# lucidrains/glom-pytorch

Hardware: AMD Instinct MI355X
Metric: images/sec (higher is better)
Workload: dtype bf16; 1 GPU; model=glom-512x6, global_batch=64, image_size=224, patch_size=14, iters=12, objective=denoising-mse fwd+bwd+adamw, decode_step=7, impl=native, parallelism=dp1

## Files before the change

### glom_pytorch_amd/ops/__init__.py

```python

from __future__ import annotations

import glob
import importlib
import os

import torch

_EXT = None
_EXT_ERR: Exception | None = None


def _load_extension():
    global _EXT, _EXT_ERR
    if _EXT is not None:
        return _EXT
    if _EXT_ERR is not None:
        raise _EXT_ERR
    try:
        from glom_pytorch_amd.ops import _glom_hip
        _EXT = _glom_hip
        return _EXT
    except ImportError as e:
        here = os.path.dirname(__file__)
        sos = glob.glob(os.path.join(here, "_glom_hip*.so"))
        _EXT_ERR = ImportError(
            f"glom_pytorch_amd HIP extension not importable ({e}). "
            f"Found candidate .so files: {sos or 'none'}. Build it in-tree with "
            f"`PYTORCH_ROCM_ARCH=gfx950 python setup.py build_ext --inplace` "
            f"from the repo root. The GPU path never falls back to eager.")
        raise _EXT_ERR


def available() -> bool:
    try:
        _load_extension()
        return True
    except ImportError:
        return False


def native_forward(model, img, iters, levels=None, return_all=False,
                   grad_iters=None, overlap_tail=False, loss_level_min=None):
    from glom_pytorch_amd.ops.functional import glom_forward
    return glom_forward(model, img, iters=iters, levels=levels,
                        return_all=return_all, grad_iters=grad_iters,
                        overlap_tail=overlap_tail,
                        loss_level_min=loss_level_min)


def set_token_hoist(on: bool) -> None:
    from glom_pytorch_amd.ops import functional
    functional.set_token_hoist(on)


def set_mix_fusion(on: bool) -> None:
    from glom_pytorch_amd.ops import functional
    functional.set_mix_fusion(on)


def set_check_level_cone(on: bool) -> None:
    from glom_pytorch_amd.ops import functional
    functional.set_check_level_cone(on)
```

### glom_pytorch_amd/ops/csrc/aux_kernels.h

```cpp
#pragma once
#include <hip/hip_runtime.h>

void launch_add_pos(const void* levels, const void* pos, void* out,
                    long total, int N, int L, int d, hipStream_t s);
void launch_rnorm(const void* levels, float* out, int B, int N, int L, int d,
                  hipStream_t s);
void launch_softmax_fwd(const void* scores, void* probs, const bool* mask,
                        int nprob, int N, int self_mask, hipStream_t s);
void launch_softmax_bwd(const void* P, const void* dP, const float* rnorm,
                        void* dS, void* dSr, const bool* mask, int nprob,
                        int N, int self_mask, float alpha, hipStream_t s,
                        int L = 1, int l_lo = 0);
void launch_knorm_combine(const void* dkhat, const void* lev,
                          const float* rnorm, const void* dv, const void* dq,
                          void* out, int B, int N, int L, int d,
                          hipStream_t s, int l_lo = 0);
void launch_mix_fwd(const void* prev, const void* bu, const void* td,
                    const void* cons, void* out, long total, int L, int d,
                    hipStream_t s, const void* bu0 = nullptr,
                    long bu0_ld = 0, const void* pos = nullptr,
                    void* td_next = nullptr, float* rn_next = nullptr,
                    int N = 1);
bool mix_fwd_can_emit_next(int L, int d);
void launch_mix_bwd(const void* dout, void* dmix, void* dtd, long total,
                    int L, int d, hipStream_t s);
void launch_add4(const void* a, const void* b, const void* c, const void* d,
                 void* out, long total, hipStream_t s);
void launch_gelu(const void* in, void* out, long total, hipStream_t s);
```

### glom_pytorch_amd/ops/csrc/aux_kernels.hip

```cpp

#include "common.h"
#include "aux_kernels.h"

#define NTHREADS 256
#define WPB (NTHREADS / WAVE)

__global__ __launch_bounds__(NTHREADS) void k_rnorm(
        const ushort_t* __restrict__ levels, float* __restrict__ out,
        int B, int N, int L, int d) {
    long row = (long)blockIdx.x * WPB + threadIdx.x / WAVE;
    long total = (long)B * N * L;
    if (row >= total) return;
    int lane = threadIdx.x % WAVE;
    int l = row % L;
    long n = (row / L) % N;
    long b = row / ((long)N * L);
    const ushort_t* x = levels + row * d;
    float ss = 0.f;
    if (d % 8 == 0) {
        for (int q0 = lane * 8; q0 < d; q0 += WAVE * 8) {
            union { uint4v v; ushort_t u[8]; } t;
            t.v = *(const uint4v*)(x + q0);
#pragma unroll
            for (int e = 0; e < 8; e++) {
                float v = bf2f(t.u[e]);
                ss += v * v;
            }
        }
    } else {
        for (int q = lane; q < d; q += WAVE) {
            float v = bf2f(x[q]);
            ss += v * v;
        }
    }
    ss = wave_reduce_sum(ss);
    if (lane == 0)
        out[(b * L + l) * N + n] = 1.0f / fmaxf(sqrtf(ss), 1e-12f);
}

__global__ __launch_bounds__(NTHREADS) void k_softmax_fwd(
        const ushort_t* __restrict__ scores, ushort_t* __restrict__ probs,
        const bool* __restrict__ nonlocal_mask, int nprob, int N,
        int self_mask) {
    long row = (long)blockIdx.x * WPB + threadIdx.x / WAVE;
    if (row >= (long)nprob * N) return;
    int lane = threadIdx.x % WAVE;
    int i = row % N;
    const ushort_t* s = scores + row * N;
    ushort_t* o = probs + row * N;
    const bool* m = nonlocal_mask ? nonlocal_mask + (long)i * N : nullptr;
    const float SELF = bf2f(f2bf(-5e-4f));
    const float NEG = -3.3895314e38f;

    if (N % 8 == 0) {
        float mx = -INFINITY, sum = 0.f;
#pragma unroll 1
        for (int j0 = lane * 8; j0 < N; j0 += WAVE * 8) {
            union { uint4v v; ushort_t u[8]; } t;
            t.v = *(const uint4v*)(s + j0);
#pragma unroll
            for (int e = 0; e < 8; e++) {
                float v = bf2f(t.u[e]);
                if (self_mask && j0 + e == i) v = SELF;
                if (m && m[j0 + e]) v = NEG;
                mx = fmaxf(mx, v);
            }
        }
        mx = wave_reduce_max(mx);
        mx = __shfl(mx, 0, WAVE);
#pragma unroll 1
        for (int j0 = lane * 8; j0 < N; j0 += WAVE * 8) {
            union { uint4v v; ushort_t u[8]; } t, ov;
            t.v = *(const uint4v*)(s + j0);
#pragma unroll
            for (int e = 0; e < 8; e++) {
                float v = bf2f(t.u[e]);
                if (self_mask && j0 + e == i) v = SELF;
                if (m && m[j0 + e]) v = NEG;
                float ex = __expf(v - mx);
                sum += ex;
                ov.u[e] = f2bf(ex);
            }
            *(uint4v*)(o + j0) = ov.v;
        }
        sum = wave_reduce_sum(sum);
        sum = __shfl(sum, 0, WAVE);
        float inv = 1.0f / sum;
#pragma unroll 1
        for (int j0 = lane * 8; j0 < N; j0 += WAVE * 8) {
            union { uint4v v; ushort_t u[8]; } t;
            t.v = *(const uint4v*)(o + j0);
#pragma unroll
            for (int e = 0; e < 8; e++) t.u[e] = f2bf(bf2f(t.u[e]) * inv);
            *(uint4v*)(o + j0) = t.v;
        }
        return;
    }
    float mx = -INFINITY;
    for (int j = lane; j < N; j += WAVE) {
        float v = bf2f(s[j]);
        if (self_mask && j == i) v = SELF;
        if (m && m[j]) v = NEG;
        mx = fmaxf(mx, v);
    }
    mx = wave_reduce_max(mx);
    mx = __shfl(mx, 0, WAVE);
    float sum = 0.f;
    for (int j = lane; j < N; j += WAVE) {
        float v = bf2f(s[j]);
        if (self_mask && j == i) v = SELF;
        if (m && m[j]) v = NEG;
        sum += expf(v - mx);
    }
    sum = wave_reduce_sum(sum);
    sum = __shfl(sum, 0, WAVE);
    float inv = 1.0f / sum;
    for (int j = lane; j < N; j += WAVE) {
        float v = bf2f(s[j]);
        if (self_mask && j == i) v = SELF;
        if (m && m[j]) v = NEG;
        o[j] = f2bf(expf(v - mx) * inv);
    }
}

__global__ __launch_bounds__(NTHREADS) void k_softmax_bwd(
        const ushort_t* __restrict__ P, const ushort_t* __restrict__ dP,
        const float* __restrict__ rnorm, ushort_t* __restrict__ dS,
        ushort_t* __restrict__ dSr, const bool* __restrict__ nonlocal_mask,
        int nprob, int N, int self_mask, float alpha, int L, int l_lo) {
    long row = (long)blockIdx.x * WPB + threadIdx.x / WAVE;
    if (row >= (long)nprob * N) return;
    int lane = threadIdx.x % WAVE;
    int i = row % N;
    long p = row / N;
    p = (p / (L - l_lo)) * L + l_lo + p % (L - l_lo);
    row = p * N + i;
    const ushort_t* pr = P + row * N;
    const ushort_t* dpr = dP + row * N;
    const float* rn = rnorm + p * N;
    const bool* m = nonlocal_mask ? nonlocal_mask + (long)i * N : nullptr;

    float t = 0.f;
    if (N % 8 == 0) {
#pragma unroll 1
        for (int j0 = lane * 8; j0 < N; j0 += WAVE * 8) {
            union { uint4v v; ushort_t u[8]; } a, bb;
            a.v = *(const uint4v*)(pr + j0);
            bb.v = *(const uint4v*)(dpr + j0);
#pragma unroll
            for (int e = 0; e < 8; e++) t += bf2f(a.u[e]) * bf2f(bb.u[e]);
        }
        t = wave_reduce_sum(t);
        t = __shfl(t, 0, WAVE);
#pragma unroll 1
        for (int j0 = lane * 8; j0 < N; j0 += WAVE * 8) {
            union { uint4v v; ushort_t u[8]; } a, bb, o1, o2;
            a.v = *(const uint4v*)(pr + j0);
            bb.v = *(const uint4v*)(dpr + j0);
#pragma unroll
            for (int e = 0; e < 8; e++) {
                float v = alpha * bf2f(a.u[e]) * (bf2f(bb.u[e]) - t);
                if (self_mask && j0 + e == i) v = 0.f;
                if (m && m[j0 + e]) v = 0.f;
                o1.u[e] = f2bf(v);
                o2.u[e] = f2bf(v * rn[j0 + e]);
            }
            *(uint4v*)(dS + row * N + j0) = o1.v;
            *(uint4v*)(dSr + row * N + j0) = o2.v;
        }
        return;
    }
    for (int j = lane; j < N; j += WAVE) t += bf2f(pr[j]) * bf2f(dpr[j]);
    t = wave_reduce_sum(t);
    t = __shfl(t, 0, WAVE);
    for (int j = lane; j < N; j += WAVE) {
        float v = alpha * bf2f(pr[j]) * (bf2f(dpr[j]) - t);
        if (self_mask && j == i) v = 0.f;
        if (m && m[j]) v = 0.f;
        dS[row * N + j] = f2bf(v);
        dSr[row * N + j] = f2bf(v * rn[j]);
    }
}

__global__ __launch_bounds__(NTHREADS) void k_knorm_combine(
        const ushort_t* __restrict__ dkhat, const ushort_t* __restrict__ lev,
        const float* __restrict__ rnorm, const ushort_t* __restrict__ dv,
        const ushort_t* __restrict__ dq, ushort_t* __restrict__ out,
        int B, int N, int L, int d, int l_lo) {
    long row = (long)blockIdx.x * WPB + threadIdx.x / WAVE;
    const int Ll = L - l_lo;
    long total = (long)B * N * Ll;
    if (row >= total) return;
    int lane = threadIdx.x % WAVE;
    int l = l_lo + row % Ll;
    long n = (row / Ll) % N;
    long b = row / ((long)N * Ll);
    row = (b * N + n) * L + l;
    const ushort_t* dkh = dkhat + ((b * L + l) * N + n) * (long)d;
    const ushort_t* x = lev + row * d;
    float r = rnorm[(b * L + l) * N + n];
    bool clamped = r >= 0.999e12f;

    const bool vec = (d % 8 == 0);
    float dot = 0.f;
    if (!clamped) {
        if (vec) {
            for (int q0 = lane * 8; q0 < d; q0 += WAVE * 8) {
                union { uint4v v; ushort_t u[8]; } a, b;
                a.v = *(const uint4v*)(dkh + q0);
                b.v = *(const uint4v*)(x + q0);
#pragma unroll
                for (int e = 0; e < 8; e++)
                    dot += bf2f(a.u[e]) * bf2f(b.u[e]);
            }
        } else {
            for (int q = lane; q < d; q += WAVE)
                dot += bf2f(dkh[q]) * bf2f(x[q]);
        }
        dot = wave_reduce_sum(dot);
        dot = __shfl(dot, 0, WAVE);
    }
    float c = clamped ? 0.f : r * r * dot;
    if (vec) {
        for (int q0 = lane * 8; q0 < d; q0 += WAVE * 8) {
            union { uint4v v; ushort_t u[8]; } a, b, dvv, dqv, o;
            a.v = *(const uint4v*)(dkh + q0);
            b.v = *(const uint4v*)(x + q0);
            dvv.v = *(const uint4v*)(dv + row * d + q0);
            dqv.v = *(const uint4v*)(dq + row * d + q0);
#pragma unroll
            for (int e = 0; e < 8; e++) {
                float dk = r * (bf2f(a.u[e]) - bf2f(b.u[e]) * c);
                o.u[e] = f2bf(dk + bf2f(dvv.u[e]) + bf2f(dqv.u[e]));
            }
            *(uint4v*)(out + row * d + q0) = o.v;
        }
    } else {
        for (int q = lane; q < d; q += WAVE) {
            float dk = r * (bf2f(dkh[q]) - bf2f(x[q]) * c);
            out[row * d + q] =
                f2bf(dk + bf2f(dv[row * d + q]) + bf2f(dq[row * d + q]));
        }
    }
}

template <bool NEXT>
__global__ __launch_bounds__(NTHREADS) void k_mix_fwd(
        const ushort_t* __restrict__ prev, const ushort_t* __restrict__ bu,
        const ushort_t* __restrict__ td, const ushort_t* __restrict__ cons,
        ushort_t* __restrict__ out, long total, int L, int d,
        const ushort_t* __restrict__ bu0, long bu0_ld,
        const ushort_t* __restrict__ pos, ushort_t* __restrict__ td_next,
        float* __restrict__ rn_next, int N) {
    long idx = ((long)blockIdx.x * NTHREADS + threadIdx.x) * 8;
    if (idx >= total) return;
    int q = idx % d;
    int l = (idx / d) % L;
    long bn = idx / ((long)d * L);
    union { uint4v v; ushort_t u[8]; } a, b, c4, t, o;
    a.v = *(const uint4v*)(prev + idx);
    b.v = *(const uint4v*)((bu0 && l == 0) ? bu0 + bn * bu0_ld + q
                                           : bu + idx);
    c4.v = *(const uint4v*)(cons + idx);
    bool has_td = l < L - 1;
    if (has_td) t.v = *(const uint4v*)(td + (bn * (L - 1) + l) * (long)d + q);
    float c = has_td ? 4.0f : 3.0f;
#pragma unroll
    for (int e = 0; e < 8; e++) {
        float v = bf2f(a.u[e]) + bf2f(b.u[e]) + bf2f(c4.u[e]);
        if (has_td) v += bf2f(t.u[e]);
        o.u[e] = f2bf(v / c);
    }
    *(uint4v*)(out + idx) = o.v;
    if (NEXT) {
        long n = bn % N;
        long bb = bn / N;
        float ss = 0.f;
#pragma unroll
        for (int e = 0; e < 8; e++) {
            float v = bf2f(o.u[e]);
            ss += v * v;
        }
        ss = wave_reduce_sum(ss);
        if (threadIdx.x % WAVE == 0)
            rn_next[(bb * L + l) * N + n] = 1.0f / fmaxf(sqrtf(ss), 1e-12f);
        if (l >= 1) {
            union { uint4v v; ushort_t u[8]; } p;
            p.v = *(const uint4v*)(pos + n * (long)d + q);
#pragma unroll
            for (int e = 0; e < 8; e++)
                p.u[e] = f2bf(bf2f(o.u[e]) + bf2f(p.u[e]));
            *(uint4v*)(td_next + (bn * (L - 1) + l - 1) * (long)d + q) = p.v;
        }
    }
}

__global__ __launch_bounds__(NTHREADS) void k_mix_bwd(
        const ushort_t* __restrict__ dout, ushort_t* __restrict__ dmix,
        ushort_t* __restrict__ dtd, long total, int L, int d) {
    long idx = ((long)blockIdx.x * NTHREADS + threadIdx.x) * 8;
    if (idx >= total) return;
    int q = idx % d;
    int l = (idx / d) % L;
    long bn = idx / ((long)d * L);
    union { uint4v v; ushort_t u[8]; } g, o;
    g.v = *(const uint4v*)(dout + idx);
    bool has_td = l < L - 1;
    float c = has_td ? 4.0f : 3.0f;
#pragma unroll
    for (int e = 0; e < 8; e++) o.u[e] = f2bf(bf2f(g.u[e]) / c);
    *(uint4v*)(dmix + idx) = o.v;
    if (has_td) *(uint4v*)(dtd + (bn * (L - 1) + l) * (long)d + q) = o.v;
}

__global__ __launch_bounds__(NTHREADS) void k_add_pos(
        const ushort_t* __restrict__ levels, const ushort_t* __restrict__ pos,
        ushort_t* __restrict__ out, long total, int N, int L, int d) {
    long i8 = ((long)blockIdx.x * NTHREADS + threadIdx.x) * 8;
    if (i8 >= total) return;
    int G = L - 1;
    int q = i8 % d;
    int g = (i8 / d) % G;
    long bn = i8 / ((long)d * G);
    long n = bn % N;
    const ushort_t* lv = levels + (bn * L + g + 1) * (long)d + q;
    const ushort_t* pp = pos + n * (long)d + q;
    union { uint4v v; ushort_t u[8]; } a, b;
    a.v = *(const uint4v*)lv;
    b.v = *(const uint4v*)pp;
#pragma unroll
    for (int e = 0; e < 8; e++) a.u[e] = f2bf(bf2f(a.u[e]) + bf2f(b.u[e]));
    *(uint4v*)(out + i8) = a.v;
}


static inline long cdiv(long a, long b) { return (a + b - 1) / b; }

void launch_add_pos(const void* levels, const void* pos, void* out,
                    long total, int N, int L, int d, hipStream_t s) {
    hipLaunchKernelGGL(k_add_pos, dim3(cdiv(total / 8, NTHREADS)),
                       dim3(NTHREADS), 0, s, (const ushort_t*)levels,
                       (const ushort_t*)pos, (ushort_t*)out, total, N, L, d);
}

void launch_rnorm(const void* levels, float* out, int B, int N, int L, int d,
                  hipStream_t s) {
    long rows = (long)B * N * L;
    hipLaunchKernelGGL(k_rnorm, dim3(cdiv(rows, WPB)), dim3(NTHREADS), 0, s,
                       (const ushort_t*)levels, out, B, N, L, d);
}

void launch_softmax_fwd(const void* scores, void* probs, const bool* mask,
                        int nprob, int N, int self_mask, hipStream_t s) {
    long rows = (long)nprob * N;
    hipLaunchKernelGGL(k_softmax_fwd, dim3(cdiv(rows, WPB)), dim3(NTHREADS),
                       0, s, (const ushort_t*)scores, (ushort_t*)probs, mask,
                       nprob, N, self_mask);
}

void launch_softmax_bwd(const void* P, const void* dP, const float* rnorm,
                        void* dS, void* dSr, const bool* mask, int nprob,
                        int N, int self_mask, float alpha, hipStream_t s,
                        int L, int l_lo) {
    long rows = (long)nprob * N;
    hipLaunchKernelGGL(k_softmax_bwd, dim3(cdiv(rows, WPB)), dim3(NTHREADS),
                       0, s, (const ushort_t*)P, (const ushort_t*)dP, rnorm,
                       (ushort_t*)dS, (ushort_t*)dSr, mask, nprob, N,
                       self_mask, alpha, L, l_lo);
}

void launch_knorm_combine(const void* dkhat, const void* lev,
                          const float* rnorm, const void* dv, const void* dq,
                          void* out, int B, int N, int L, int d,
                          hipStream_t s, int l_lo) {
    long rows = (long)B * N * (L - l_lo);
    if (rows <= 0) return;
    hipLaunchKernelGGL(k_knorm_combine, dim3(cdiv(rows, WPB)), dim3(NTHREADS),
                       0, s, (const ushort_t*)dkhat, (const ushort_t*)lev,
                       rnorm, (const ushort_t*)dv, (const ushort_t*)dq,
                       (ushort_t*)out, B, N, L, d, l_lo);
}

void launch_mix_fwd(const void* prev, const void* bu, const void* td,
                    const void* cons, void* out, long total, int L, int d,
                    hipStream_t s, const void* bu0, long bu0_ld,
                    const void* pos, void* td_next, float* rn_next, int N) {
    dim3 grid(cdiv(total / 8, NTHREADS)), block(NTHREADS);
    if (td_next)
        hipLaunchKernelGGL(k_mix_fwd<true>, grid, block, 0, s,
                           (const ushort_t*)prev, (const ushort_t*)bu,
                           (const ushort_t*)td, (const ushort_t*)cons,
                           (ushort_t*)out, total, L, d, (const ushort_t*)bu0,
                           bu0_ld, (const ushort_t*)pos, (ushort_t*)td_next,
                           rn_next, N);
    else
        hipLaunchKernelGGL(k_mix_fwd<false>, grid, block, 0, s,
                           (const ushort_t*)prev, (const ushort_t*)bu,
                           (const ushort_t*)td, (const ushort_t*)cons,
                           (ushort_t*)out, total, L, d, (const ushort_t*)bu0,
                           bu0_ld, (const ushort_t*)nullptr,
                           (ushort_t*)nullptr, (float*)nullptr, N);
}

bool mix_fwd_can_emit_next(int L, int d) { return d == WAVE * 8 && L >= 2; }

void launch_mix_bwd(const void* dout, void* dmix, void* dtd, long total,
                    int L, int d, hipStream_t s) {
    hipLaunchKernelGGL(k_mix_bwd, dim3(cdiv(total / 8, NTHREADS)), dim3(NTHREADS),
                       0, s, (const ushort_t*)dout, (ushort_t*)dmix,
                       (ushort_t*)dtd, total, L, d);
}

__global__ __launch_bounds__(NTHREADS) void k_add4(
        const ushort_t* __restrict__ a, const ushort_t* __restrict__ b,
        const ushort_t* __restrict__ c, const ushort_t* __restrict__ d,
        ushort_t* __restrict__ out, long total) {
    long i8 = ((long)blockIdx.x * NTHREADS + threadIdx.x) * 8;
    if (i8 >= total) return;
    union { uint4v v; ushort_t u[8]; } va, vb, vc, vd, o;
    va.v = *(const uint4v*)(a + i8);
    vb.v = *(const uint4v*)(b + i8);
    vc.v = *(const uint4v*)(c + i8);
    vd.v = *(const uint4v*)(d + i8);
#pragma unroll
    for (int e = 0; e < 8; e++)
        o.u[e] = f2bf(bf2f(va.u[e]) + bf2f(vb.u[e]) + bf2f(vc.u[e])
                      + bf2f(vd.u[e]));
    *(uint4v*)(out + i8) = o.v;
}

void launch_add4(const void* a, const void* b, const void* c, const void* d,
                 void* out, long total, hipStream_t s) {
    hipLaunchKernelGGL(k_add4, dim3(cdiv(total / 8, NTHREADS)),
                       dim3(NTHREADS), 0, s, (const ushort_t*)a,
                       (const ushort_t*)b, (const ushort_t*)c,
                       (const ushort_t*)d, (ushort_t*)out, total);
}

__global__ __launch_bounds__(NTHREADS) void k_gelu(
        const ushort_t* __restrict__ in, ushort_t* __restrict__ out,
        long total) {
    long i8 = ((long)blockIdx.x * NTHREADS + threadIdx.x) * 8;
    if (i8 >= total) return;
    union { uint4v v; ushort_t u[8]; } x, o;
    x.v = *(const uint4v*)(in + i8);
    float xin[8], yv[8];
#pragma unroll
    for (int e = 0; e < 8; e++) xin[e] = bf2f(x.u[e]);
    gelu_f_vec<8>(xin, yv);
#pragma unroll
    for (int e = 0; e < 8; e++) o.u[e] = f2bf(yv[e]);
    *(uint4v*)(out + i8) = o.v;
}

void launch_gelu(const void* in, void* out, long total, hipStream_t s) {
    hipLaunchKernelGGL(k_gelu, dim3(cdiv(total / 8, NTHREADS)),
                       dim3(NTHREADS), 0, s, (const ushort_t*)in,
                       (ushort_t*)out, total);
}
```

### glom_pytorch_amd/ops/csrc/bindings.cpp

```cpp

#include <torch/extension.h>
#include <c10/hip/HIPStream.h>
#include <hip/hip_runtime.h>

#include <cmath>
#include <cstring>
#include <vector>

#include "gemm.h"
#include "aux_kernels.h"
#include "native_ops.h"
#include "island_kernels.h"
#include "parse_kernels.h"
#include "contrast_kernels.h"

namespace {

torch::Tensor alias_slab_slice(const torch::Tensor& slab, int64_t idx,
                               c10::IntArrayRef sizes) {
    int64_t n = 1;
    for (auto s : sizes) n *= s;
    void* ptr = (char*)slab.data_ptr() + idx * n * slab.element_size();
    auto keep = slab;
    return torch::from_blob(
        ptr, sizes, [keep](void*) mutable {}, slab.options());
}

#define CHECK_IN(x)                                                        \
    TORCH_CHECK(x.is_cuda(), #x " must be on GPU");                        \
    TORCH_CHECK(x.is_contiguous(), #x " must be contiguous");              \
    TORCH_CHECK(x.scalar_type() == at::kBFloat16, #x " must be bf16")

hipStream_t cur_stream() {
    return c10::hip::getCurrentHIPStream().stream();
}

int g_nt8p_mode = []() {
    const char* e = getenv("GLOM_NT8P");
    return (e && e[0] == '0') ? 0 : 1;
}();

void set_nt8p(bool on) { g_nt8p_mode = on ? 1 : 0; }

int g_tn_tr = []() {
    const char* e = getenv("GLOM_TN_TR");
    return (e && e[0] >= '0' && e[0] <= '2') ? e[0] - '0' : 1;
}();
int g_tn_tr_variant = []() {
    const char* e = getenv("GLOM_TN_TR_VARIANT");
    return (e && e[0] >= '1' && e[0] <= '3') ? e[0] - '0' : 1;
}();
void set_tn_tr(bool on) { g_tn_tr = on ? 2 : 0; }
void set_tn_tr_mode(int64_t m) {
    TORCH_CHECK(m >= 0 && m <= 2, "tn_tr mode is 0..2");
    g_tn_tr = (int)m;
}
int64_t get_tn_tr_mode() { return g_tn_tr; }
void set_tn_tr_variant(int64_t v) {
    TORCH_CHECK(v >= 1 && v <= 3, "tn_tr variant is 1..3");
    g_tn_tr_variant = (int)v;
}
int64_t get_tn_tr_variant() { return g_tn_tr_variant; }
static bool tn_tr_auto(const GemmParams& p) {
    return p.splitk > 1 || p.K >= 4096;
}
int g_finish_wide = []() {
    const char* e = getenv("GLOM_FINISH_WIDE");
    return (e && e[0] == '0') ? 0 : 1;
}();
void set_finish_wide(bool on) { g_finish_wide = on ? 1 : 0; }

int g_gelu_pair = []() {
    const char* e = getenv("GLOM_GELU_PAIR");
    return (e && e[0] == '0') ? 0 : 1;
}();
void set_gelu_pair(bool on) { g_gelu_pair = on ? 1 : 0; }

int g_wide_epi = []() {
    const char* e = getenv("GLOM_WIDE_EPI");
    return (e && e[0] >= '0' && e[0] <= '3') ? e[0] - '0' : 1;
}();
int g_wide_epi_nt8p = []() {
    const char* e = getenv("GLOM_WIDE_EPI_NT8P");
    return (e && e[0] == '1') ? 1 : 0;
}();
void set_wide_epilogue(bool on) { g_wide_epi = on ? 2 : 0; }
void set_wide_epilogue_mode(int64_t m) {
    TORCH_CHECK(m >= 0 && m <= 3, "wide epilogue mode is 0..3");
    g_wide_epi = (int)m;
}
int64_t get_wide_epilogue_mode() { return g_wide_epi; }
static int wide_epi_auto(int epilogue) {
    return epilogue == EPI_GELUGRAD ? 3 : epilogue == EPI_GELU ? 1 : 0;
}
static int nt5p_wide_bits(int epilogue) {
    switch (g_wide_epi) {
    case 0: return 0;
    case 2: return 3;
    case 3: return 2;
    default: return wide_epi_auto(epilogue);
    }
}
void set_wide_epilogue_nt8p(bool on) { g_wide_epi_nt8p = on ? 1 : 0; }

static bool wide_epi_ok(const GemmParams& p) {
    auto al = [](const void* q) { return ((uintptr_t)q & 15) == 0; };
    bool ok = al(p.Cbase) && p.Cld % 8 == 0 && p.Csin % 8 == 0
              && p.Csout % 8 == 0;
    if (p.epilogue == EPI_GELU_PAIR)
        ok = ok && al(p.out2) && p.out2_ld % 8 == 0 && p.out2_sin % 8 == 0
             && p.out2_sout % 8 == 0;
    if (p.epilogue == EPI_GELUGRAD)
        ok = ok && al(p.aux_base) && p.aux_ld % 8 == 0 && p.aux_sin % 8 == 0
             && p.aux_sout % 8 == 0;
    return ok;
}

static bool nt5p_enabled() {
    static const bool on = []() {
        const char* e = getenv("GLOM_NT5P");
        return !e || e[0] != '0';
    }();
    return on;
}
static long nt5p_min_grid() {
    static const long g = []() {
        const char* e = getenv("GLOM_NT5P_MING");
        return e ? atol(e) : 96;
    }();
    return g;
}
static bool nt5p_takes_up_proj(int64_t M, int64_t N, int64_t K, int64_t G) {
    return nt5p_enabled() && M % 512 == 0 && N % 256 == 0 && N >= 1024
           && K % 64 == 0 && K >= 64
           && (N / 256) * (M / 512) * G >= nt5p_min_grid();
}

void check_launch() {
    hipError_t e = hipGetLastError();
    TORCH_CHECK(e == hipSuccess, "HIP launch failed: ", hipGetErrorString(e));
}

int64_t g_nce_launches[2] = {0, 0};
std::vector<int64_t> nce_launch_counts() {
    return {g_nce_launches[0], g_nce_launches[1]};
}
int g_nce_fast = []() {
    const char* e = getenv("GLOM_NCE_FAST");
    return (e && e[0] == '0') ? 0 : 1;
}();
void set_nce_fast(bool on) { g_nce_fast = on ? 1 : 0; }

void run_gemm(GemmParams& p, hipStream_t s, const torch::TensorOptions& opts,
              bool lds_ok, long gate_problems = 0) {
    const long gate_np = gate_problems > 0 ? gate_problems : p.nproblems;
    const bool no_xform = !(p.A.flags & (OP_GELU | OP_POS))
                          && !(p.B.flags & (OP_GELU | OP_POS));
    const bool nce_generic = !g_nce_fast && (p.epilogue == EPI_NCE_FWD
                                             || p.epilogue == EPI_NCE_BWD);
    const bool nt_fast = p.layout == LAYOUT_NT && lds_ok && no_xform
                         && p.M % 128 == 0 && p.N % 128 == 0
                         && p.K % 64 == 0 && p.K >= 64 && !nce_generic;
    const bool tn_fast = p.layout == LAYOUT_TN && lds_ok && no_xform
                         && p.M % 128 == 0 && p.N % 128 == 0 && p.K % 8 == 0;
    const bool nn_fast = p.layout == LAYOUT_NN && lds_ok && no_xform
                         && p.M % 128 == 0 && p.N % 128 == 0 && p.K % 8 == 0;

    p.splitk = 1;
    p.ws = nullptr;
    torch::Tensor ws;
    long blocks = ((p.N + 127) / 128) * ((p.M + 127) / 128) * gate_np;
    if (p.layout == LAYOUT_TN && p.epilogue == EPI_NONE && !p.has_bias
        && !p.has_colscale && blocks < 1024 && p.K >= 4096) {
        long sk = std::min<long>(16, std::max<long>(1, 2048 / blocks));
        sk = std::min<long>(sk, p.K / 64);
        if (sk > 1) {
            ws = torch::empty({sk * p.nproblems * (long)p.M * p.N},
                              opts.dtype(at::kFloat));
            p.splitk = (int)sk;
            p.ws = ws.data_ptr<float>();
        }
    }
    const bool nce = p.epilogue == EPI_NCE_FWD || p.epilogue == EPI_NCE_BWD;
    if (nce) {
        auto al = [](const void* q) { return ((uintptr_t)q & 15) == 0; };
        TORCH_CHECK(p.layout == LAYOUT_NT && p.nproblems == 1
                    && !((p.A.flags | p.B.flags | p.Cflags) & OP_TABLE)
                    && !p.has_bias && !p.has_colscale,
                    "EPI_NCE_* needs one plain NT problem");
        const NceArgs q = nce_get(p);
        TORCH_CHECK(q.rrow && q.rcol && q.part && q.group > 0,
                    "EPI_NCE_* parameters not set (nce_set)");
        TORCH_CHECK(p.epilogue == EPI_NCE_FWD ? q.pos != nullptr
                                              : (q.lse && p.Cbase),
                    "EPI_NCE_* outputs not set");
        TORCH_CHECK(!nt_fast
                    || (al(p.A.base) && al(p.B.base)
                        && (p.epilogue == EPI_NCE_FWD
                            || (al(p.Cbase) && p.Cld % 8 == 0))),
                    "EPI_NCE_* full-tile path needs 16-byte aligned operands");
    }
    const bool nt3 = nt_fast && p.N % 256 == 0 && p.N >= 1024 && !nce;
    const bool nt5p_on = nt5p_enabled();
    const bool nt5p = nt5p_on && nt3 && p.M % 512 == 0
                      && (long)(p.N / 256) * (p.M / 512) * gate_np
                         >= nt5p_min_grid()
                      && !(p.Cflags & OP_TABLE)
                      && (p.epilogue == EPI_NONE
                          || p.epilogue == EPI_GELUGRAD
                          || p.epilogue == EPI_GELU_PAIR
                          || p.epilogue == EPI_GELU);
    TORCH_CHECK(p.epilogue != EPI_GELU || nt5p,
                "EPI_GELU needs an nt5p-eligible shape");
    static const bool disp_dbg = []() {
        const char* e = getenv("GLOM_DISPATCH_DEBUG");
        return e && e[0] == '1';
    }();
    const bool nt8p_on = g_nt8p_mode == 1;
    static const long nt8p_mink = []() {
        const char* e = getenv("GLOM_NT8P_MINK");
        return e ? atol(e) : 2048;
    }();
    const bool nt8p = nt8p_on && p.layout == LAYOUT_NT && lds_ok && no_xform
                      && p.M % 256 == 0 && p.N % 256 == 0 && p.K % 64 == 0
                      && p.K >= nt8p_mink
                      && !(p.Cflags & OP_TABLE)
                      && (p.epilogue == EPI_NONE
                          || p.epilogue == EPI_GELUGRAD)
                      && (long)(p.N / 256) * (p.M / 256) * gate_np >= 256;
    auto al16 = [](const void* q) { return ((uintptr_t)q & 15) == 0; };
    bool tn_al = al16(p.A.base) && al16(p.B.base);
    if (p.A.flags & OP_TABLE)
        for (int g = 0; g < p.nproblems; g++) tn_al = tn_al && al16(p.Atab[g]);
    if (p.B.flags & OP_TABLE)
        for (int g = 0; g < p.nproblems; g++) tn_al = tn_al && al16(p.Btab[g]);
    const bool tn_tr = (g_tn_tr == 2 || (g_tn_tr == 1 && tn_tr_auto(p)))
                       && tn_fast && p.K % 64 == 0 && p.K >= 64
                       && tn_al && p.A.sin % 8 == 0 && p.A.sout % 8 == 0
                       && p.B.sin % 8 == 0 && p.B.sout % 8 == 0;
    p.wide_epi = !wide_epi_ok(p) ? 0
                 : nt8p ? g_wide_epi_nt8p : nt5p_wide_bits(p.epilogue);
    if (disp_dbg)
        fprintf(stderr,
                "[dispatch] L%d M%ld N%ld K%ld epi%d nt3=%d nt5p=%d on=%d "
                "nt8p=%d ctabflag=%d m512=%d tn_tr=%d sk=%d finw=%d "
                "kern=%s\n",
                p.layout, (long)p.M, (long)p.N, (long)p.K, p.epilogue,
                (int)nt3, (int)nt5p, (int)nt5p_on, (int)nt8p,
                (int)(p.Cflags & OP_TABLE), (int)(p.M % 512 == 0),
                tn_tr ? (p.splitk > 1 ? g_tn_tr_variant : 1) : 0,
                p.splitk, g_finish_wide,
                nt8p ? "nt8p" : nt5p ? "nt5p" : nt3 ? "nt4"
                : nt_fast ? "nt_fast" : tn_tr ? "tn_tr"
                : tn_fast ? (p.splitk > 1 ? "tn_sk" : "tn_fast")
                : nn_fast ? "nn_fast" : "generic");
    if (nt8p)
        launch_gemm_nt_fast8p(p, s);
    else if (nt5p)
        launch_gemm_nt_fast5p(p, s);
    else if (nt3)
        launch_gemm_nt_fast4(p, s);
    else if (nt_fast) {
        launch_gemm_nt_fast(p, s);
        if (nce) g_nce_launches[0]++;
    }
    else if (tn_tr)
        launch_gemm_tn_tr(p, g_tn_tr_variant, s);
    else if (tn_fast && p.splitk > 1)
        launch_gemm_tn_sk(p, s);
    else if (tn_fast)
        launch_gemm_tn_fast(p, s);
    else if (nn_fast)
        launch_gemm_nn_fast(p, s);
    else {
        launch_gemm(p, s);
        if (nce) g_nce_launches[1]++;
    }
    check_launch();
    if (p.splitk > 1) {
        launch_gemm_finish(p, s, g_finish_wide == 1);
        check_launch();
    }
}

GemmParams base_params(int64_t M, int64_t N, int64_t K, int layout,
                       int64_t nproblems, int64_t nInner, float alpha) {
    GemmParams p;
    std::memset(&p, 0, sizeof(p));
    p.M = (int)M; p.N = (int)N; p.K = (int)K;
    p.layout = layout;
    p.nproblems = (int)nproblems;
    p.nInner = (int)nInner;
    p.alpha = alpha;
    p.epilogue = EPI_NONE;
    return p;
}


void* u16_at(const torch::Tensor& t, int64_t off) {
    return (void*)((uint16_t*)t.data_ptr() + off);
}

void zero_fill(void* ptr, int64_t bytes, hipStream_t s) {
    if (bytes <= 0) return;
    hipError_t e = hipMemsetAsync(ptr, 0, (size_t)bytes, s);
    TORCH_CHECK(e == hipSuccess, "zero fill failed: ", hipGetErrorString(e));
}

void zero_unwritten_dx(void* dLevels, int64_t BN, int64_t L, int64_t d,
                       int64_t mode, int64_t g_lo, hipStream_t s) {
    if (mode == 0) {
        launch_zero_slices(dLevels, BN, (int)L, (int)d, 0,
                           (int)std::max<int64_t>(g_lo, 1) - 1, s);
        check_launch();
        launch_zero_slice(dLevels, BN, (int)L, (int)d, (int)L - 1, s);
        check_launch();
    } else {
        launch_zero_slices(dLevels, BN, (int)L, (int)d, 0,
                           (int)std::min<int64_t>(g_lo + 1, L), s);
        check_launch();
    }
}


std::vector<torch::Tensor> grouped_ff_fwd(
        c10::optional<torch::Tensor> tokens_opt, torch::Tensor levels,
        c10::optional<torch::Tensor> pos_opt, torch::Tensor w1,
        torch::Tensor b1, torch::Tensor w2, torch::Tensor b2, int64_t mode,
        bool save_for_bwd = true, bool group0_done = false,
        c10::optional<torch::Tensor> td_in_ready = c10::nullopt) {
    CHECK_IN(levels); CHECK_IN(w1); CHECK_IN(b1); CHECK_IN(w2); CHECK_IN(b2);
    const int64_t B = levels.size(0), N = levels.size(1),
                  L = levels.size(2), d = levels.size(3);
    const int64_t G = (mode == 0) ? L : L - 1;
    TORCH_CHECK(G <= GEMM_MAX_TABLE, "levels > 16 unsupported by table mode");
    TORCH_CHECK(!group0_done || (mode == 0 && G >= 2),
                "group0_done needs the bottom-up mode and levels >= 2");
    const int64_t g0 = group0_done ? 1 : 0;
    const int64_t Ga = G - g0;
    const int64_t m4 = w1.size(0) / G;
    const int64_t M = B * N;
    TORCH_CHECK(d % 8 == 0 && m4 % 8 == 0, "dim and mult*dim must be /8");
    TORCH_CHECK(w1.size(0) == G * m4 && w1.size(1) == d);
    TORCH_CHECK(w2.size(0) == G * d && w2.size(1) == m4);

    auto opts = levels.options();
    const bool pair = g_gelu_pair
                      && (M % 512 == 0) && (m4 % 256 == 0)
                      && m4 >= 1024;
    const bool gelu_only = !save_for_bwd && pair
                           && nt5p_takes_up_proj(M, m4, d, G);
    auto Hpre = gelu_only ? torch::empty({0}, opts)
                          : torch::empty({G, M, m4}, opts);
    auto Hact = torch::empty({G, M, m4}, opts);
    auto Y = torch::empty({B, N, G, d}, opts);
    hipStream_t s = cur_stream();

    torch::Tensor td_in;
    if (mode == 1) {
        TORCH_CHECK(pos_opt.has_value(), "top-down needs pos");
        auto pos = pos_opt.value();
        CHECK_IN(pos);
        if (td_in_ready.has_value()) {
            td_in = td_in_ready.value();
            CHECK_IN(td_in);
            TORCH_CHECK(td_in.dim() == 4 && td_in.size(0) == B
                        && td_in.size(1) == N && td_in.size(2) == G
                        && td_in.size(3) == d, "td_in must be (B,N,L-1,d)");
        } else {
            td_in = torch::empty({B, N, G, d}, opts);
            launch_add_pos(levels.data_ptr(), pos.data_ptr(),
                           td_in.data_ptr(), td_in.numel(), (int)N, (int)L,
                           (int)d, s);
            check_launch();
        }
    }

    {
        GemmParams p = base_params(M, m4, d, LAYOUT_NT, Ga, Ga, 1.0f);
        if (mode == 0) {
            TORCH_CHECK(tokens_opt.has_value(), "bottom-up needs tokens");
            auto tokens = tokens_opt.value();
            CHECK_IN(tokens);
            TORCH_CHECK(tokens.numel() == M * d, "tokens must be (B,N,d)");
            p.A.flags = OP_TABLE;
            if (g0 == 0) {
                p.Atab[0] = tokens.data_ptr();
                p.Atabld[0] = d;
            }
            for (int64_t g = 1; g < G; g++) {
                p.Atab[g - g0] = (const char*)levels.data_ptr()
                                 + (g - 1) * d * 2;
                p.Atabld[g - g0] = L * d;
            }
        } else {
            p.A.base = td_in.data_ptr();
            p.A.sin = d; p.A.ld = G * d;
        }
        p.B.base = u16_at(w1, g0 * m4 * d); p.B.sin = m4 * d; p.B.ld = d;
        p.Csin = M * m4; p.Cld = m4;
        p.bias_base = u16_at(b1, g0 * m4); p.bias_sin = m4; p.has_bias = 1;
        if (gelu_only) {
            p.epilogue = EPI_GELU;
            p.Cbase = u16_at(Hact, g0 * M * m4);
        } else {
            p.Cbase = u16_at(Hpre, g0 * M * m4);
            if (pair) {
                p.epilogue = EPI_GELU_PAIR;
                p.out2 = u16_at(Hact, g0 * M * m4);
                p.out2_sin = M * m4; p.out2_ld = m4;
            }
        }
        run_gemm(p, s, opts, true, G);
        if (!pair) {
            launch_gelu(u16_at(Hpre, g0 * M * m4), u16_at(Hact, g0 * M * m4),
                        Ga * M * m4, s);
            check_launch();
        }
    }
    {
        GemmParams p = base_params(M, d, m4, LAYOUT_NT, Ga, Ga, 1.0f);
        p.A.base = u16_at(Hact, g0 * M * m4); p.A.sin = M * m4; p.A.ld = m4;
        p.B.base = u16_at(w2, g0 * d * m4); p.B.sin = d * m4; p.B.ld = m4;
        p.Cbase = u16_at(Y, g0 * d); p.Csin = d; p.Cld = G * d;
        p.bias_base = u16_at(b2, g0 * d); p.bias_sin = d; p.has_bias = 1;
        run_gemm(p, s, opts, true, G);
    }
    if (mode != 1) td_in = torch::empty({0}, opts);
    if (!save_for_bwd) Hpre = torch::empty({0}, opts);
    return {Y, Hpre, Hact, td_in};
}

std::vector<torch::Tensor> grouped_ff_bwd(
        torch::Tensor dY, c10::optional<torch::Tensor> tokens_opt,
        torch::Tensor levels, c10::optional<torch::Tensor> pos_opt,
        torch::Tensor w1, torch::Tensor w2, torch::Tensor Hpre,
        torch::Tensor Hact, int64_t mode,
        c10::optional<torch::Tensor> w1t_opt = c10::nullopt,
        c10::optional<torch::Tensor> w2t_opt = c10::nullopt,
        c10::optional<torch::Tensor> td_in_opt = c10::nullopt,
        int64_t g_lo = 0) {
    CHECK_IN(dY); CHECK_IN(levels); CHECK_IN(w1); CHECK_IN(w2); CHECK_IN(Hpre);
    CHECK_IN(Hact);
    const int64_t B = levels.size(0), N = levels.size(1),
                  L = levels.size(2), d = levels.size(3);
    const int64_t G = (mode == 0) ? L : L - 1;
    const int64_t m4 = w1.size(0) / G;
    const int64_t M = B * N;
    TORCH_CHECK(g_lo >= 0 && g_lo <= G, "g_lo out of range");
    const int64_t Ga = G - g_lo;
    auto opts = levels.options();
    hipStream_t s = cur_stream();

    auto dLevels = torch::empty({B, N, L, d}, opts);
    zero_unwritten_dx(dLevels.data_ptr(), B * N, L, d, mode, g_lo, s);
    torch::Tensor dTokens;
    auto dW1 = torch::empty({G * m4, d}, opts);
    auto dW2 = torch::empty({G * d, m4}, opts);
    auto dB1 = torch::empty({G * m4}, opts);
    auto dB2 = torch::empty({G * d}, opts);
    zero_fill(dW1.data_ptr(), g_lo * m4 * d * 2, s);
    zero_fill(dW2.data_ptr(), g_lo * d * m4 * 2, s);
    zero_fill(dB1.data_ptr(), g_lo * m4 * 2, s);
    if (mode == 0) {
        dTokens = torch::empty({B, N, d}, opts);
        if (g_lo > 0) zero_fill(dTokens.data_ptr(), M * d * 2, s);
    } else {
        dTokens = torch::empty({0}, opts);
    }
    if (Ga == 0) {
        zero_fill(dB2.data_ptr(), G * d * 2, s);
        return {dTokens, dLevels, dW1, dB1, dW2, dB2};
    }
    TORCH_CHECK(Hpre.numel() == G * M * m4 && Hact.numel() == G * M * m4,
                "Hpre / Hact must be (G, M, m4)");
    auto dHpre = torch::empty({G, M, m4}, opts);

    auto w1t = w1t_opt.has_value()
        ? w1t_opt.value()
        : w1.view({G, m4, d}).transpose(1, 2).contiguous();
    auto w2t = w2t_opt.has_value()
        ? w2t_opt.value()
        : w2.view({G, d, m4}).transpose(1, 2).contiguous();

    torch::Tensor td_in;
    if (mode == 1) {
        if (td_in_opt.has_value() && td_in_opt->numel() > 0) {
            td_in = td_in_opt.value();
        } else {
            auto pos = pos_opt.value();
            CHECK_IN(pos);
            td_in = torch::empty({B, N, G, d}, opts);
            launch_add_pos(levels.data_ptr(), pos.data_ptr(),
                           td_in.data_ptr(), td_in.numel(), (int)N, (int)L,
                           (int)d, s);
            check_launch();
        }
    }

    const bool dh_nt3 = (M % 128 == 0) && (m4 % 256 == 0) && (m4 >= 1024)
                        && (d % 64 == 0);
    torch::Tensor db1f;
    {
        GemmParams p = base_params(M, m4, d, LAYOUT_NT, Ga, Ga, 1.0f);
        p.A.base = u16_at(dY, g_lo * d); p.A.sin = d; p.A.ld = G * d;
        p.B.base = u16_at(w2t, g_lo * m4 * d); p.B.sin = m4 * d; p.B.ld = d;
        p.Cbase = u16_at(dHpre, g_lo * M * m4); p.Csin = M * m4; p.Cld = m4;
        p.epilogue = EPI_GELUGRAD;
        p.aux_base = u16_at(Hpre, g_lo * M * m4);
        p.aux_sin = M * m4; p.aux_ld = m4;
        if (dh_nt3) {
            db1f = torch::empty({Ga, M / 64, m4}, opts.dtype(at::kFloat));
            p.colsum_out = db1f.data_ptr<float>();
            p.colsum_sin = (M / 64) * m4;
        }
        run_gemm(p, s, opts, true, G);
    }
    {
        GemmParams p = base_params(M, d, m4, LAYOUT_NT, Ga, Ga, 1.0f);
        p.A.base = u16_at(dHpre, g_lo * M * m4); p.A.sin = M * m4; p.A.ld = m4;
        p.B.base = u16_at(w1t, g_lo * d * m4); p.B.sin = d * m4; p.B.ld = m4;
        if (mode == 0) {
            p.Cflags = OP_TABLE;
            for (int64_t g = g_lo; g < G; g++) {
                p.Ctab[g - g_lo] = g == 0 ? dTokens.data_ptr()
                                          : u16_at(dLevels, (g - 1) * d);
                p.Ctabld[g - g_lo] = g == 0 ? d : L * d;
            }
        } else {
            p.Cbase = u16_at(dLevels, (g_lo + 1) * d);
            p.Csin = d; p.Cld = L * d;
        }
        run_gemm(p, s, opts, true, G);
    }
    {
        GemmParams p = base_params(m4, d, M, LAYOUT_TN, Ga, Ga, 1.0f);
        p.A.base = u16_at(dHpre, g_lo * M * m4); p.A.sin = M * m4; p.A.ld = m4;
        if (mode == 0) {
            auto tokens = tokens_opt.value();
            CHECK_IN(tokens);
            p.B.flags = OP_TABLE;
            for (int64_t g = g_lo; g < G; g++) {
                p.Btab[g - g_lo] = g == 0 ? tokens.data_ptr()
                                          : u16_at(levels, (g - 1) * d);
                p.Btabld[g - g_lo] = g == 0 ? d : L * d;
            }
        } else {
            p.B.base = u16_at(td_in, g_lo * d);
            p.B.sin = d; p.B.ld = G * d;
        }
        p.Cbase = u16_at(dW1, g_lo * m4 * d); p.Csin = m4 * d; p.Cld = d;
        run_gemm(p, s, opts, true, G);
    }
    {
        GemmParams p = base_params(d, m4, M, LAYOUT_TN, Ga, Ga, 1.0f);
        p.A.base = u16_at(dY, g_lo * d); p.A.sin = d; p.A.ld = G * d;
        p.B.base = u16_at(Hact, g_lo * M * m4); p.B.sin = M * m4; p.B.ld = m4;
        p.Cbase = u16_at(dW2, g_lo * d * m4); p.Csin = d * m4; p.Cld = m4;
        run_gemm(p, s, opts, true, G);
    }
    if (dh_nt3) {
        launch_colsum_fin(db1f.data_ptr<float>(), u16_at(dB1, g_lo * m4),
                          (int)Ga, m4, (int)(M / 64), s);
        check_launch();
    } else {
        auto ws = torch::empty({(long)Ga * colsum_rb(M) * m4},
                               opts.dtype(at::kFloat));
        launch_colsum(u16_at(dHpre, g_lo * M * m4), ws.data_ptr<float>(),
                      u16_at(dB1, g_lo * m4), (int)Ga, M, m4, s);
        check_launch();
    }
    {
        auto ws = torch::empty({(long)colsum_rb(M) * G * d},
                               opts.dtype(at::kFloat));
        launch_colsum(dY.data_ptr(), ws.data_ptr<float>(), dB2.data_ptr(),
                      1, M, G * d, s);
        check_launch();
    }
    return {dTokens, dLevels, dW1, dB1, dW2, dB2};
}


std::vector<torch::Tensor> consensus_fwd(
        torch::Tensor levels, bool attend_self,
        c10::optional<torch::Tensor> mask_opt,
        c10::optional<torch::Tensor> rnorm_ready = c10::nullopt) {
    CHECK_IN(levels);
    const int64_t B = levels.size(0), N = levels.size(1),
                  L = levels.size(2), d = levels.size(3);
    const int64_t P = B * L;
    auto opts = levels.options();
    hipStream_t s = cur_stream();
    const bool* mask = nullptr;
    if (mask_opt.has_value()) {
        auto m = mask_opt.value();
        TORCH_CHECK(m.is_cuda() && m.is_contiguous()
                    && m.scalar_type() == at::kBool);
        mask = m.data_ptr<bool>();
    }

    const bool lds_ok = (N % 8 == 0) && (d % 8 == 0);
    torch::Tensor rnorm;
    if (rnorm_ready.has_value()) {
        rnorm = rnorm_ready.value();
        TORCH_CHECK(rnorm.is_cuda() && rnorm.is_contiguous()
                    && rnorm.scalar_type() == at::kFloat
                    && rnorm.dim() == 3 && rnorm.size(0) == B
                    && rnorm.size(1) == L && rnorm.size(2) == N,
                    "rnorm must be f32 (B,L,N)");
    } else {
        rnorm = torch::empty({B, L, N}, opts.dtype(at::kFloat));
        launch_rnorm(levels.data_ptr(), rnorm.data_ptr<float>(),
                     (int)B, (int)N, (int)L, (int)d, s);
        check_launch();
    }

    auto probs = torch::empty({B, L, N, N}, opts);
    const bool fused_sm = (N == 256) && (d % 64 == 0) && lds_ok;
    const bool fuse_av = fused_sm && !getenv("GLOM_NO_FUSE_AV");
    torch::Tensor out_av;
    if (fuse_av) out_av = torch::empty({B, N, L, d}, opts);
    {
        GemmParams p = base_params(N, N, d, LAYOUT_NT, P, L,
                                   (float)std::pow((double)d, -0.5));
        p.A.base = levels.data_ptr(); p.A.sin = d; p.A.sout = N * L * d;
        p.A.ld = L * d;
        p.B = p.A;
        p.Cbase = probs.data_ptr(); p.Csin = N * N; p.Csout = L * N * N;
        p.Cld = N;
        p.colscale_base = rnorm.data_ptr<float>();
        p.cs_sin = N; p.cs_sout = L * N; p.has_colscale = 1;
        if (fused_sm) {
            p.epilogue = EPI_SOFTMAX;
            p.self_mask = attend_self ? 0 : 1;
            p.nlmask = mask;
            p.splitk = 1;
            if (fuse_av) {
                p.out2 = out_av.data_ptr();
                p.out2_sin = d; p.out2_sout = N * L * d; p.out2_ld = L * d;
                p.aux_base = levels.data_ptr();
                p.aux_sin = d; p.aux_sout = N * L * d; p.aux_ld = L * d;
                p.npatch = (int)d;
            }
            launch_gemm_nt_fast4(p, s);
            check_launch();
        } else {
            run_gemm(p, s, opts, lds_ok);
            launch_softmax_fwd(probs.data_ptr(), probs.data_ptr(), mask,
                               (int)P, (int)N, attend_self ? 0 : 1, s);
            check_launch();
        }
    }
    if (fuse_av)
        return {out_av, probs, rnorm};
    auto out = torch::empty({B, N, L, d}, opts);
    {
        GemmParams p = base_params(N, d, N, LAYOUT_NN, P, L, 1.0f);
        p.A.base = probs.data_ptr(); p.A.sin = N * N; p.A.sout = L * N * N;
        p.A.ld = N;
        p.B.base = levels.data_ptr(); p.B.sin = d; p.B.sout = N * L * d;
        p.B.ld = L * d;
        p.Cbase = out.data_ptr(); p.Csin = d; p.Csout = N * L * d;
        p.Cld = L * d;
        run_gemm(p, s, opts, lds_ok);
    }
    return {out, probs, rnorm};
}

torch::Tensor consensus_bwd(torch::Tensor dOut, torch::Tensor levels,
                            torch::Tensor probs, torch::Tensor rnorm,
                            bool attend_self,
                            c10::optional<torch::Tensor> mask_opt,
                            int64_t l_lo = 0) {
    CHECK_IN(dOut); CHECK_IN(levels); CHECK_IN(probs);
    const int64_t B = levels.size(0), N = levels.size(1),
                  L = levels.size(2), d = levels.size(3);
    TORCH_CHECK(l_lo >= 0 && l_lo <= L, "l_lo out of range");
    const int64_t Ll = L - l_lo;
    const int64_t P = B * Ll;
    const int64_t Pfull = B * L;
    const bool lds_ok = (N % 8 == 0) && (d % 8 == 0);
    auto opts = levels.options();
    hipStream_t s = cur_stream();
    const bool* mask = nullptr;
    if (mask_opt.has_value()) mask = mask_opt.value().data_ptr<bool>();

    auto dLevels = torch::empty({B, N, L, d}, opts);
    launch_zero_slices(dLevels.data_ptr(), B * N, (int)L, (int)d, 0,
                       (int)l_lo, s);
    check_launch();
    if (Ll == 0) return dLevels;
    TORCH_CHECK(l_lo == 0 || d % 8 == 0, "l_lo needs dim % 8 == 0");
    const float* rn = rnorm.data_ptr<float>();
    auto lv = [&](const torch::Tensor& t) { return u16_at(t, l_lo * d); };
    auto nn = [&](const torch::Tensor& t) { return u16_at(t, l_lo * N * N); };

    const bool fused_sm = (N == 256) && (d % 64 == 0) && lds_ok;
    auto dS = torch::empty({B, L, N, N}, opts);
    auto dSr = torch::empty({B, L, N, N}, opts);
    torch::Tensor dP;
    if (fused_sm) {
        GemmParams p = base_params(N, N, d, LAYOUT_NT, P, Ll, 1.0f);
        p.A.base = lv(dOut); p.A.sin = d; p.A.sout = N * L * d;
        p.A.ld = L * d;
        p.B.base = lv(levels); p.B.sin = d; p.B.sout = N * L * d;
        p.B.ld = L * d;
        p.Cbase = nn(dS); p.Csin = N * N; p.Csout = L * N * N;
        p.Cld = N;
        p.epilogue = EPI_SMBWD;
        p.aux_base = nn(probs);
        p.aux_sin = N * N; p.aux_sout = L * N * N; p.aux_ld = N;
        p.out2 = nn(dSr);
        p.out2_sin = N * N; p.out2_sout = L * N * N; p.out2_ld = N;
        p.colscale_base = rn + l_lo * N;
        p.cs_sin = N; p.cs_sout = L * N; p.has_colscale = 1;
        p.self_mask = attend_self ? 0 : 1;
        p.nlmask = mask;
        p.alpha2 = (float)std::pow((double)d, -0.5);
        p.splitk = 1;
        launch_gemm_nt_fast4(p, s);
        check_launch();
    } else {
        dP = torch::empty({B, L, N, N}, opts);
        GemmParams p = base_params(N, N, d, LAYOUT_NT, P, Ll, 1.0f);
        p.A.base = lv(dOut); p.A.sin = d; p.A.sout = N * L * d;
        p.A.ld = L * d;
        p.B.base = lv(levels); p.B.sin = d; p.B.sout = N * L * d;
        p.B.ld = L * d;
        p.Cbase = nn(dP); p.Csin = N * N; p.Csout = L * N * N;
        p.Cld = N;
        run_gemm(p, s, opts, lds_ok, Pfull);
        launch_softmax_bwd(probs.data_ptr(), dP.data_ptr(), rn,
                           dS.data_ptr(), dSr.data_ptr(), mask, (int)P,
                           (int)N, attend_self ? 0 : 1,
                           (float)std::pow((double)d, -0.5), s, (int)L,
                           (int)l_lo);
        check_launch();
    }

    auto dv = torch::empty({B, N, L, d}, opts);
    {
        GemmParams p = base_params(N, d, N, LAYOUT_TN, P, Ll, 1.0f);
        p.A.base = nn(probs); p.A.sin = N * N; p.A.sout = L * N * N;
        p.A.ld = N;
        p.B.base = lv(dOut); p.B.sin = d; p.B.sout = N * L * d;
        p.B.ld = L * d;
        p.Cbase = lv(dv); p.Csin = d; p.Csout = N * L * d;
        p.Cld = L * d;
        run_gemm(p, s, opts, lds_ok, Pfull);
    }
    auto dq = torch::empty({B, N, L, d}, opts);
    {
        GemmParams p = base_params(N, d, N, LAYOUT_NN, P, Ll, 1.0f);
        p.A.base = nn(dSr); p.A.sin = N * N; p.A.sout = L * N * N;
        p.A.ld = N;
        p.B.base = lv(levels); p.B.sin = d; p.B.sout = N * L * d;
        p.B.ld = L * d;
        p.Cbase = lv(dq); p.Csin = d; p.Csout = N * L * d;
        p.Cld = L * d;
        run_gemm(p, s, opts, lds_ok, Pfull);
    }
    auto dkhat = torch::empty({B, L, N, d}, opts);
    {
        GemmParams p = base_params(N, d, N, LAYOUT_TN, P, Ll, 1.0f);
        p.A.base = nn(dS); p.A.sin = N * N; p.A.sout = L * N * N;
        p.A.ld = N;
        p.B.base = lv(levels); p.B.sin = d; p.B.sout = N * L * d;
        p.B.ld = L * d;
        p.Cbase = u16_at(dkhat, l_lo * N * d);
        p.Csin = N * d; p.Csout = L * N * d;
        p.Cld = d;
        run_gemm(p, s, opts, lds_ok, Pfull);
    }
    launch_knorm_combine(dkhat.data_ptr(), levels.data_ptr(), rn,
                         dv.data_ptr(), dq.data_ptr(), dLevels.data_ptr(),
                         (int)B, (int)N, (int)L, (int)d, s, (int)l_lo);
    check_launch();
    return dLevels;
}


std::vector<torch::Tensor> level_mix_fwd_next(
        torch::Tensor levels, torch::Tensor bu, torch::Tensor td,
        torch::Tensor cons, c10::optional<torch::Tensor> slab = c10::nullopt,
        int64_t slab_idx = 0, c10::optional<torch::Tensor> bu0 = c10::nullopt,
        c10::optional<torch::Tensor> pos = c10::nullopt) {
    CHECK_IN(levels); CHECK_IN(bu); CHECK_IN(td); CHECK_IN(cons);
    const int64_t B = levels.size(0), N = levels.size(1),
                  L = levels.size(2), d = levels.size(3);
    TORCH_CHECK(d % 8 == 0, "dim must be a multiple of 8");
    TORCH_CHECK(bu.numel() == levels.numel() && cons.numel() == levels.numel()
                && td.numel() == B * N * (L - 1) * d,
                "level mix operands do not match levels");
    const void* bu0_ptr = nullptr;
    int64_t bu0_ld = 0;
    if (bu0.has_value()) {
        const auto& t = bu0.value();
        TORCH_CHECK(t.is_cuda() && t.scalar_type() == at::kBFloat16
                    && t.dim() == 3 && t.size(0) == B && t.size(1) == N
                    && t.size(2) == d && t.stride(2) == 1
                    && t.stride(1) >= d && t.stride(1) % 8 == 0
                    && t.stride(0) == N * t.stride(1)
                    && ((uintptr_t)t.data_ptr() & 15) == 0,
                    "bu0 must be an evenly strided (B,N,d) bf16 view");
        bu0_ptr = t.data_ptr();
        bu0_ld = t.stride(1);
    }
    const bool emit = pos.has_value() && mix_fwd_can_emit_next((int)L, (int)d);
    auto td_next = torch::empty({0}, levels.options());
    auto rn_next = torch::empty({0}, levels.options().dtype(at::kFloat));
    if (emit) {
        CHECK_IN(pos.value());
        TORCH_CHECK(pos->numel() == N * d, "pos must be (N,d)");
        td_next = torch::empty({B, N, L - 1, d}, levels.options());
        rn_next = torch::empty({B, L, N}, levels.options().dtype(at::kFloat));
    }
    torch::Tensor out;
    if (slab.has_value()) {
        TORCH_CHECK(slab->is_contiguous()
                    && slab->scalar_type() == at::kBFloat16
                    && slab->numel() >= (slab_idx + 1) * levels.numel(),
                    "bad trajectory slab");
        out = alias_slab_slice(slab.value(), slab_idx, levels.sizes());
    } else {
        out = torch::empty_like(levels);
    }
    launch_mix_fwd(levels.data_ptr(), bu.data_ptr(), td.data_ptr(),
                   cons.data_ptr(), out.data_ptr(), levels.numel(), (int)L,
                   (int)d, cur_stream(), bu0_ptr, bu0_ld,
                   emit ? pos->data_ptr() : nullptr,
                   emit ? td_next.data_ptr() : nullptr,
                   emit ? rn_next.data_ptr<float>() : nullptr, (int)N);
    check_launch();
    return {out, td_next, rn_next};
}

torch::Tensor level_mix_fwd(torch::Tensor levels, torch::Tensor bu,
                            torch::Tensor td, torch::Tensor cons,
                            c10::optional<torch::Tensor> slab = c10::nullopt,
                            int64_t slab_idx = 0,
                            c10::optional<torch::Tensor> bu0 = c10::nullopt) {
    return level_mix_fwd_next(levels, bu, td, cons, slab, slab_idx, bu0,
                              c10::nullopt)[0];
}

std::vector<torch::Tensor> level_mix_bwd(torch::Tensor dout) {
    CHECK_IN(dout);
    const int64_t B = dout.size(0), N = dout.size(1), L = dout.size(2),
                  d = dout.size(3);
    TORCH_CHECK(d % 8 == 0, "dim must be a multiple of 8");
    auto dmix = torch::empty_like(dout);
    auto dtd = torch::empty({B, N, L - 1, d}, dout.options());
    launch_mix_bwd(dout.data_ptr(), dmix.data_ptr(), dtd.data_ptr(),
                   dout.numel(), (int)L, (int)d, cur_stream());
    check_launch();
    return {dmix, dtd};
}




std::vector<torch::Tensor> glom_step_fwd(
        torch::Tensor tokens, torch::Tensor levels, torch::Tensor pos,
        torch::Tensor bw1, torch::Tensor bb1, torch::Tensor bw2,
        torch::Tensor bb2, torch::Tensor tw1, torch::Tensor tb1,
        torch::Tensor tw2, torch::Tensor tb2, bool attend_self,
        c10::optional<torch::Tensor> mask,
        c10::optional<torch::Tensor> slab = c10::nullopt,
        int64_t slab_idx = 0, bool save_for_bwd = true,
        c10::optional<torch::Tensor> bu0 = c10::nullopt,
        c10::optional<torch::Tensor> td_in_ready = c10::nullopt,
        c10::optional<torch::Tensor> rnorm_ready = c10::nullopt,
        bool emit_next = false) {
    auto bu = grouped_ff_fwd(tokens, levels, c10::nullopt, bw1, bb1, bw2,
                             bb2, 0, save_for_bwd, bu0.has_value());
    auto td = grouped_ff_fwd(c10::nullopt, levels, pos, tw1, tb1, tw2,
                             tb2, 1, save_for_bwd, false, td_in_ready);
    auto at = consensus_fwd(levels, attend_self, mask, rnorm_ready);
    auto mx = level_mix_fwd_next(
        levels, bu[0], td[0], at[0], slab, slab_idx, bu0,
        emit_next ? c10::optional<torch::Tensor>(pos) : c10::nullopt);
    std::vector<torch::Tensor> r = {mx[0], bu[1], bu[2], td[1], td[2],
                                    at[1], at[2], td[3]};
    if (emit_next) { r.push_back(mx[1]); r.push_back(mx[2]); }
    return r;
}

std::vector<torch::Tensor> glom_step_bwd(
        torch::Tensor dnew, torch::Tensor tokens, torch::Tensor levels,
        torch::Tensor pos, torch::Tensor bw1, torch::Tensor bw2,
        torch::Tensor tw1, torch::Tensor tw2, torch::Tensor buHpre,
        torch::Tensor buHact, torch::Tensor tdHpre, torch::Tensor tdHact,
        torch::Tensor probs, torch::Tensor rnorm, bool attend_self,
        c10::optional<torch::Tensor> mask,
        c10::optional<torch::Tensor> bw1t, c10::optional<torch::Tensor> bw2t,
        c10::optional<torch::Tensor> tw1t,
        c10::optional<torch::Tensor> tw2t,
        c10::optional<torch::Tensor> td_in = c10::nullopt,
        int64_t lo = 0) {
    const int64_t L = levels.size(2);
    TORCH_CHECK(lo >= 0 && lo < L, "lo out of range");
    auto mix = level_mix_bwd(dnew);
    auto bu = grouped_ff_bwd(mix[0], tokens, levels, c10::nullopt, bw1,
                             bw2, buHpre, buHact, 0, bw1t, bw2t,
                             c10::nullopt, lo);
    auto td = grouped_ff_bwd(mix[1], c10::nullopt, levels, pos, tw1, tw2,
                             tdHpre, tdHact, 1, tw1t, tw2t, td_in,
                             std::min<int64_t>(lo, L - 1));
    auto dAttn = consensus_bwd(mix[0], levels, probs, rnorm, attend_self,
                               mask, lo);
    auto dLevels = torch::empty_like(levels);
    launch_add4(mix[0].data_ptr(), bu[1].data_ptr(), td[1].data_ptr(),
                dAttn.data_ptr(), dLevels.data_ptr(), levels.numel(),
                cur_stream());
    check_launch();
    const int64_t B = levels.size(0), N = levels.size(1),
                  d = levels.size(3);
    auto dPos = torch::empty({N, d}, levels.options());
    const int BCH = (int)std::min<int64_t>(B, 8);
    auto ws = torch::empty({BCH * N * d}, levels.options().dtype(at::kFloat));
    launch_dpos(td[1].data_ptr(), dPos.data_ptr(), ws.data_ptr<float>(),
                BCH, (int)B, (int)N, (int)L, (int)d, cur_stream());
    check_launch();
    return {bu[0], dLevels, dPos, bu[2], bu[3], bu[4], bu[5],
            td[2], td[3], td[4], td[5]};
}

double bench_gemm(int64_t M, int64_t N, int64_t K, int64_t layout,
                  int64_t nproblems, int64_t epilogue, int64_t reps) {
    auto opts = torch::TensorOptions().dtype(at::kBFloat16)
                    .device(at::kCUDA);
    torch::Tensor A, Bt;
    if (layout == LAYOUT_TN)
        A = torch::randn({nproblems, K, M}, opts) * 0.05;
    else
        A = torch::randn({nproblems, M, K}, opts) * 0.05;
    if (layout == LAYOUT_NT)
        Bt = torch::randn({nproblems, N, K}, opts) * 0.05;
    else
        Bt = torch::randn({nproblems, K, N}, opts) * 0.05;
    auto C = torch::empty({nproblems, M, N}, opts);
    auto bias = torch::randn({nproblems, N}, opts);
    auto aux = torch::randn({nproblems, M, N}, opts);
    auto out2 = torch::empty({nproblems, M, N}, opts);
    hipStream_t s = cur_stream();

    auto run = [&]() {
        GemmParams p = base_params(M, N, K, (int)layout, nproblems,
                                   nproblems, 1.0f);
        p.A.base = A.data_ptr();
        p.A.sin = A.size(1) * A.size(2); p.A.ld = A.size(2);
        p.B.base = Bt.data_ptr();
        p.B.sin = Bt.size(1) * Bt.size(2); p.B.ld = Bt.size(2);
        p.Cbase = C.data_ptr(); p.Csin = M * N; p.Cld = N;
        p.epilogue = (int)epilogue;
        if (epilogue == EPI_GELUGRAD) {
            p.aux_base = aux.data_ptr(); p.aux_sin = M * N; p.aux_ld = N;
        }
        if (epilogue == EPI_GELU_PAIR || epilogue == EPI_GELU
            || epilogue == 10 || epilogue == 12) {
            p.bias_base = bias.data_ptr(); p.bias_sin = N; p.has_bias = 1;
            p.out2 = out2.data_ptr(); p.out2_sin = M * N; p.out2_ld = N;
        }
        run_gemm(p, s, opts, true);
    };
    for (int i = 0; i < 3; i++) run();
    hipEvent_t e0, e1;
    hipEventCreate(&e0); hipEventCreate(&e1);
    hipEventRecord(e0, s);
    for (int64_t i = 0; i < reps; i++) run();
    hipEventRecord(e1, s);
    hipEventSynchronize(e1);
    float ms = 0;
    hipEventElapsedTime(&ms, e0, e1);
    hipEventDestroy(e0); hipEventDestroy(e1);
    return ms / reps;
}

torch::Tensor gemm_tn(torch::Tensor A, torch::Tensor B) {
    CHECK_IN(A); CHECK_IN(B);
    TORCH_CHECK(A.dim() == 3 && B.dim() == 3 && A.size(0) == B.size(0)
                && A.size(1) == B.size(1), "A (G,K,M), B (G,K,N)");
    const int64_t G = A.size(0), K = A.size(1), M = A.size(2),
                  N = B.size(2);
    TORCH_CHECK(M % 8 == 0 && N % 8 == 0, "M and N must be /8");
    auto C = torch::empty({G, M, N}, A.options());
    GemmParams p = base_params(M, N, K, LAYOUT_TN, G, G, 1.0f);
    p.A.base = A.data_ptr(); p.A.sin = K * M; p.A.ld = M;
    p.B.base = B.data_ptr(); p.B.sin = K * N; p.B.ld = N;
    p.Cbase = C.data_ptr(); p.Csin = M * N; p.Cld = N;
    run_gemm(p, cur_stream(), A.options(), true);
    return C;
}

torch::Tensor gemm_nt(torch::Tensor A, torch::Tensor B,
                      c10::optional<torch::Tensor> bias_opt = c10::nullopt) {
    CHECK_IN(A); CHECK_IN(B);
    TORCH_CHECK(A.dim() == 3 && B.dim() == 3 && A.size(0) == B.size(0)
                && A.size(2) == B.size(2), "A (G,M,K), B (G,N,K)");
    const int64_t G = A.size(0), M = A.size(1), K = A.size(2),
                  N = B.size(1);
    TORCH_CHECK(K % 8 == 0 && N % 8 == 0, "K and N must be /8");
    auto C = torch::empty({G, M, N}, A.options());
    GemmParams p = base_params(M, N, K, LAYOUT_NT, G, G, 1.0f);
    p.A.base = A.data_ptr(); p.A.sin = M * K; p.A.ld = K;
    p.B.base = B.data_ptr(); p.B.sin = N * K; p.B.ld = K;
    p.Cbase = C.data_ptr(); p.Csin = M * N; p.Cld = N;
    if (bias_opt.has_value()) {
        auto bias = bias_opt.value();
        CHECK_IN(bias);
        TORCH_CHECK(bias.dim() == 2 && bias.size(0) == G
                    && bias.size(1) == N, "bias (G,N)");
        p.bias_base = bias.data_ptr(); p.bias_sin = N; p.has_bias = 1;
    }
    run_gemm(p, cur_stream(), A.options(), true);
    return C;
}

torch::Tensor gemm_nn(torch::Tensor A, torch::Tensor B) {
    CHECK_IN(A); CHECK_IN(B);
    TORCH_CHECK(A.dim() == 3 && B.dim() == 3 && A.size(0) == B.size(0)
                && A.size(2) == B.size(1), "A (G,M,K), B (G,K,N)");
    const int64_t G = A.size(0), M = A.size(1), K = A.size(2),
                  N = B.size(2);
    TORCH_CHECK(K % 8 == 0 && N % 8 == 0, "K and N must be /8");
    auto C = torch::empty({G, M, N}, A.options());
    GemmParams p = base_params(M, N, K, LAYOUT_NN, G, G, 1.0f);
    p.A.base = A.data_ptr(); p.A.sin = M * K; p.A.ld = K;
    p.B.base = B.data_ptr(); p.B.sin = K * N; p.B.ld = N;
    p.Cbase = C.data_ptr(); p.Csin = M * N; p.Cld = N;
    run_gemm(p, cur_stream(), A.options(), true);
    return C;
}

void add4_into(torch::Tensor a, torch::Tensor b, torch::Tensor c,
               torch::Tensor d, torch::Tensor out) {
    CHECK_IN(a); CHECK_IN(b); CHECK_IN(c); CHECK_IN(d); CHECK_IN(out);
    launch_add4(a.data_ptr(), b.data_ptr(), c.data_ptr(), d.data_ptr(),
                out.data_ptr(), out.numel(), cur_stream());
    check_launch();
}



std::vector<torch::Tensor> ff_bwd_dh(torch::Tensor dY, torch::Tensor w2t,
                                     torch::Tensor Hpre, int64_t g_lo = 0) {
    CHECK_IN(dY); CHECK_IN(w2t); CHECK_IN(Hpre);
    TORCH_CHECK(Hpre.dim() == 3, "Hpre must be (G, M, m4)");
    const int64_t G = Hpre.size(0), M = Hpre.size(1), m4 = Hpre.size(2);
    const int64_t d = dY.size(3);
    TORCH_CHECK(g_lo >= 0 && g_lo <= G, "g_lo out of range");
    const int64_t Ga = G - g_lo;
    auto opts = dY.options();
    hipStream_t s = cur_stream();
    auto dHpre = torch::empty({G, M, m4}, opts);
    auto dB1 = torch::empty({G * m4}, opts);
    zero_fill(dB1.data_ptr(), g_lo * m4 * 2, s);
    if (Ga == 0) return {dHpre, dB1};
    const bool fused = (M % 128 == 0) && (m4 % 256 == 0) && (m4 >= 1024)
                       && (d % 64 == 0);
    torch::Tensor db1f;
    GemmParams p = base_params(M, m4, d, LAYOUT_NT, Ga, Ga, 1.0f);
    p.A.base = u16_at(dY, g_lo * d); p.A.sin = d; p.A.ld = G * d;
    p.B.base = u16_at(w2t, g_lo * m4 * d); p.B.sin = m4 * d; p.B.ld = d;
    p.Cbase = u16_at(dHpre, g_lo * M * m4); p.Csin = M * m4; p.Cld = m4;
    p.epilogue = EPI_GELUGRAD;
    p.aux_base = u16_at(Hpre, g_lo * M * m4);
    p.aux_sin = M * m4; p.aux_ld = m4;
    if (fused) {
        db1f = torch::empty({Ga, M / 64, m4}, opts.dtype(at::kFloat));
        p.colsum_out = db1f.data_ptr<float>();
        p.colsum_sin = (M / 64) * m4;
    }
    run_gemm(p, s, opts, true, G);
    if (fused) {
        launch_colsum_fin(db1f.data_ptr<float>(), u16_at(dB1, g_lo * m4),
                          (int)Ga, m4, (int)(M / 64), s);
        check_launch();
    } else {
        auto cws = torch::empty({(long)Ga * colsum_rb(M) * m4},
                                opts.dtype(at::kFloat));
        launch_colsum(u16_at(dHpre, g_lo * M * m4), cws.data_ptr<float>(),
                      u16_at(dB1, g_lo * m4), (int)Ga, M, m4, s);
        check_launch();
    }
    return {dHpre, dB1};
}

std::vector<torch::Tensor> ff_bwd_dx(torch::Tensor dHpre, torch::Tensor w1t,
                                     c10::optional<torch::Tensor> tokens_opt,
                                     int64_t B, int64_t N, int64_t L,
                                     int64_t mode, int64_t g_lo = 0) {
    CHECK_IN(dHpre); CHECK_IN(w1t);
    const int64_t G = dHpre.size(0), M = dHpre.size(1), m4 = dHpre.size(2);
    const int64_t d = w1t.numel() / (G * m4);
    TORCH_CHECK(g_lo >= 0 && g_lo <= G, "g_lo out of range");
    TORCH_CHECK(G == (mode == 0 ? L : L - 1) && M == B * N,
                "dHpre does not match (B, N, L)");
    const int64_t Ga = G - g_lo;
    auto opts = dHpre.options();
    hipStream_t s = cur_stream();
    torch::Tensor dTokens;
    auto dLevels = torch::empty({B, N, L, d}, opts);
    zero_unwritten_dx(dLevels.data_ptr(), B * N, L, d, mode, g_lo, s);
    if (mode == 0) {
        auto tokens = tokens_opt.value();
        CHECK_IN(tokens);
        dTokens = torch::empty({B, N, d}, opts);
        if (g_lo > 0) zero_fill(dTokens.data_ptr(), M * d * 2, s);
    } else {
        dTokens = torch::empty({0}, opts);
    }
    if (Ga == 0) return {dTokens, dLevels};
    GemmParams p = base_params(M, d, m4, LAYOUT_NT, Ga, Ga, 1.0f);
    p.A.base = u16_at(dHpre, g_lo * M * m4); p.A.sin = M * m4; p.A.ld = m4;
    p.B.base = u16_at(w1t, g_lo * d * m4); p.B.sin = d * m4; p.B.ld = m4;
    if (mode == 0) {
        p.Cflags = OP_TABLE;
        for (int64_t g = g_lo; g < G; g++) {
            p.Ctab[g - g_lo] = g == 0 ? dTokens.data_ptr()
                                      : u16_at(dLevels, (g - 1) * d);
            p.Ctabld[g - g_lo] = g == 0 ? d : L * d;
        }
    } else {
        p.Cbase = u16_at(dLevels, (g_lo + 1) * d);
        p.Csin = d; p.Cld = L * d;
    }
    run_gemm(p, s, opts, true, G);
    return {dTokens, dLevels};
}

std::vector<torch::Tensor> ff_bwd_dw(
        torch::Tensor dY, torch::Tensor dHpre,
        c10::optional<torch::Tensor> tokens_opt, torch::Tensor levels,
        c10::optional<torch::Tensor> pos_opt, torch::Tensor Hact,
        int64_t mode,
        c10::optional<torch::Tensor> td_in_opt = c10::nullopt,
        int64_t g_lo = 0) {
    CHECK_IN(dY); CHECK_IN(dHpre); CHECK_IN(levels); CHECK_IN(Hact);
    const int64_t B = levels.size(0), N = levels.size(1),
                  L = levels.size(2), d = levels.size(3);
    const int64_t G = dHpre.size(0), M = dHpre.size(1), m4 = dHpre.size(2);
    TORCH_CHECK(g_lo >= 0 && g_lo <= G, "g_lo out of range");
    TORCH_CHECK(G == (mode == 0 ? L : L - 1) && M == B * N,
                "dHpre does not match levels");
    const int64_t Ga = G - g_lo;
    auto opts = levels.options();
    hipStream_t s = cur_stream();
    auto dW1 = torch::empty({G * m4, d}, opts);
    auto dW2 = torch::empty({G * d, m4}, opts);
    auto dB2 = torch::empty({G * d}, opts);
    zero_fill(dW1.data_ptr(), g_lo * m4 * d * 2, s);
    zero_fill(dW2.data_ptr(), g_lo * d * m4 * 2, s);
    if (Ga == 0) {
        zero_fill(dB2.data_ptr(), G * d * 2, s);
        return {dW1, dW2, dB2};
    }
    torch::Tensor td_in;
    if (mode == 1) {
        if (td_in_opt.has_value() && td_in_opt->numel() > 0) {
            td_in = td_in_opt.value();
        } else {
            auto pos = pos_opt.value();
            CHECK_IN(pos);
            td_in = torch::empty({B, N, G, d}, opts);
            launch_add_pos(levels.data_ptr(), pos.data_ptr(),
                           td_in.data_ptr(), td_in.numel(), (int)N, (int)L,
                           (int)d, s);
            check_launch();
        }
    }
    {
        GemmParams p = base_params(m4, d, M, LAYOUT_TN, Ga, Ga, 1.0f);
        p.A.base = u16_at(dHpre, g_lo * M * m4);
        p.A.sin = M * m4; p.A.ld = m4;
        if (mode == 0) {
            auto tokens = tokens_opt.value();
            CHECK_IN(tokens);
            p.B.flags = OP_TABLE;
            for (int64_t g = g_lo; g < G; g++) {
                p.Btab[g - g_lo] = g == 0 ? tokens.data_ptr()
                                          : u16_at(levels, (g - 1) * d);
                p.Btabld[g - g_lo] = g == 0 ? d : L * d;
            }
        } else {
            p.B.base = u16_at(td_in, g_lo * d);
            p.B.sin = d; p.B.ld = G * d;
        }
        p.Cbase = u16_at(dW1, g_lo * m4 * d); p.Csin = m4 * d; p.Cld = d;
        run_gemm(p, s, opts, true, G);
    }
    {
        GemmParams p = base_params(d, m4, M, LAYOUT_TN, Ga, Ga, 1.0f);
        p.A.base = u16_at(dY, g_lo * d); p.A.sin = d; p.A.ld = G * d;
        p.B.base = u16_at(Hact, g_lo * M * m4);
        p.B.sin = M * m4; p.B.ld = m4;
        p.Cbase = u16_at(dW2, g_lo * d * m4); p.Csin = d * m4; p.Cld = m4;
        run_gemm(p, s, opts, true, G);
    }
    {
        auto cws = torch::empty({(long)colsum_rb(M) * G * d},
                                opts.dtype(at::kFloat));
        launch_colsum(dY.data_ptr(), cws.data_ptr<float>(), dB2.data_ptr(),
                      1, M, G * d, s);
        check_launch();
    }
    return {dW1, dW2, dB2};
}


static int64_t pad_k(int64_t k) { return (k + 63) / 64 * 64; }

std::vector<torch::Tensor> patch_embed_fwd(torch::Tensor img,
                                           torch::Tensor w, torch::Tensor b,
                                           int64_t P) {
    CHECK_IN(img); CHECK_IN(w); CHECK_IN(b);
    const int64_t B = img.size(0), C = img.size(1), H = img.size(2),
                  W = img.size(3);
    const int64_t S = W / P, N = (H / P) * S;
    const int64_t K0 = P * P * C, Kp = pad_k(K0), dout = w.size(0);
    TORCH_CHECK(w.size(1) == K0, "embed weight/patch mismatch");
    auto opts = img.options();
    hipStream_t s = cur_stream();

    auto X = torch::empty({B, N, Kp}, opts);
    launch_patchify(img.data_ptr(), X.data_ptr(), (int)B, (int)C, (int)H,
                    (int)W, (int)P, (int)Kp, s);
    check_launch();
    auto Wp = torch::empty({dout, Kp}, opts);
    launch_pad_cols(w.data_ptr(), Wp.data_ptr(), dout, (int)K0, (int)Kp, s);
    check_launch();

    auto tokens = torch::empty({B, N, dout}, opts);
    GemmParams p = base_params(B * N, dout, Kp, LAYOUT_NT, 1, 1, 1.0f);
    p.A.base = X.data_ptr(); p.A.sin = 0; p.A.ld = Kp;
    p.B.base = Wp.data_ptr(); p.B.sin = 0; p.B.ld = Kp;
    p.Cbase = tokens.data_ptr(); p.Csin = 0; p.Cld = dout;
    p.bias_base = b.data_ptr(); p.bias_sin = 0; p.has_bias = 1;
    run_gemm(p, s, opts, true);
    return {tokens, X};
}

std::vector<torch::Tensor> patch_embed_bwd(torch::Tensor dTokens,
                                           torch::Tensor X, torch::Tensor w,
                                           int64_t P, int64_t imgH,
                                           int64_t imgW, bool need_dimg) {
    CHECK_IN(dTokens); CHECK_IN(X); CHECK_IN(w);
    const int64_t B = dTokens.size(0), N = dTokens.size(1),
                  dout = dTokens.size(2);
    const int64_t Kp = X.size(2), K0 = w.size(1), C = K0 / (P * P);
    const int64_t M = B * N;
    auto opts = dTokens.options();
    hipStream_t s = cur_stream();

    auto dWp = torch::empty({dout, Kp}, opts);
    {
        GemmParams p = base_params(dout, Kp, M, LAYOUT_TN, 1, 1, 1.0f);
        p.A.base = dTokens.data_ptr(); p.A.sin = 0; p.A.ld = dout;
        p.B.base = X.data_ptr(); p.B.sin = 0; p.B.ld = Kp;
        p.Cbase = dWp.data_ptr(); p.Csin = 0; p.Cld = Kp;
        run_gemm(p, s, opts, true);
    }
    auto dW = torch::empty({dout, K0}, opts);
    launch_slice_cols(dWp.data_ptr(), dW.data_ptr(), dout, (int)Kp,
                      (int)K0, s);
    check_launch();

    auto dB = torch::empty({dout}, opts);
    {
        auto cws = torch::empty({(long)colsum_rb(M) * dout},
                                opts.dtype(at::kFloat));
        launch_colsum(dTokens.data_ptr(), cws.data_ptr<float>(),
                      dB.data_ptr(), 1, M, dout, s);
        check_launch();
    }

    torch::Tensor dImg = torch::empty({0}, opts);
    if (need_dimg) {
        auto Wp = torch::empty({dout, Kp}, opts);
        launch_pad_cols(w.data_ptr(), Wp.data_ptr(), dout, (int)K0,
                        (int)Kp, s);
        check_launch();
        auto dX = torch::empty({B, N, Kp}, opts);
        GemmParams p = base_params(M, Kp, dout, LAYOUT_NN, 1, 1, 1.0f);
        p.A.base = dTokens.data_ptr(); p.A.sin = 0; p.A.ld = dout;
        p.B.base = Wp.data_ptr(); p.B.sin = 0; p.B.ld = Kp;
        p.Cbase = dX.data_ptr(); p.Csin = 0; p.Cld = Kp;
        run_gemm(p, s, opts, true);
        dImg = torch::empty({B, C, imgH, imgW}, opts);
        launch_unpatchify(dX.data_ptr(), dImg.data_ptr(), (int)B, (int)C,
                          (int)imgH, (int)imgW, (int)P, (int)Kp, s);
        check_launch();
    }
    return {dW, dB, dImg};
}

torch::Tensor dpos(torch::Tensor dLevels) {
    CHECK_IN(dLevels);
    const int64_t B = dLevels.size(0), N = dLevels.size(1),
                  L = dLevels.size(2), d = dLevels.size(3);
    auto out = torch::empty({N, d}, dLevels.options());
    const int BCH = (int)std::min<int64_t>(B, 8);
    auto ws = torch::empty({BCH * N * d},
                           dLevels.options().dtype(at::kFloat));
    launch_dpos(dLevels.data_ptr(), out.data_ptr(),
                d % 8 == 0 ? ws.data_ptr<float>() : nullptr, BCH,
                (int)B, (int)N, (int)L, (int)d, cur_stream());
    check_launch();
    return out;
}

torch::Tensor colsum(torch::Tensor x) {
    CHECK_IN(x);
    TORCH_CHECK(x.dim() == 2, "colsum expects (M, C)");
    const int64_t M = x.size(0), C = x.size(1);
    auto out = torch::empty({C}, x.options());
    auto ws = torch::empty({(long)colsum_rb(M) * C},
                           x.options().dtype(at::kFloat));
    launch_colsum(x.data_ptr(), ws.data_ptr<float>(), out.data_ptr(), 1, M,
                  C, cur_stream());
    check_launch();
    return out;
}


static OptTable opt_table(const std::vector<torch::Tensor>& grads,
                          const std::vector<torch::Tensor>& masters,
                          const std::vector<torch::Tensor>& m1s,
                          const std::vector<torch::Tensor>& m2s,
                          const std::vector<torch::Tensor>& params,
                          const torch::Tensor& partials,
                          const torch::Tensor& norm,
                          const torch::Tensor& step_dev) {
    const size_t nt = grads.size();
    TORCH_CHECK(nt > 0 && nt <= OPT_MAX_T, "fused_adamw: 1..", OPT_MAX_T,
                " tensors supported, got ", nt);
    TORCH_CHECK(masters.size() == nt && m1s.size() == nt
                && m2s.size() == nt && params.size() == nt);
    TORCH_CHECK(partials.numel() >= OPT_NPART
                && partials.scalar_type() == at::kFloat);
    TORCH_CHECK(norm.numel() >= 1 && norm.scalar_type() == at::kFloat);
    TORCH_CHECK(step_dev.numel() >= 1
                && step_dev.scalar_type() == at::kFloat);
    OptTable t;
    std::memset(&t, 0, sizeof(t));
    t.nt = (int)nt;
    long cum = 0;
    for (size_t i = 0; i < nt; i++) {
        CHECK_IN(grads[i]); CHECK_IN(params[i]);
        TORCH_CHECK(masters[i].is_contiguous()
                    && masters[i].scalar_type() == at::kFloat);
        TORCH_CHECK(m1s[i].is_contiguous() && m2s[i].is_contiguous());
        const long n = grads[i].numel();
        TORCH_CHECK(masters[i].numel() == n && m1s[i].numel() == n
                    && m2s[i].numel() == n && params[i].numel() == n);
        t.g[i] = (const unsigned short*)grads[i].data_ptr();
        t.mw[i] = masters[i].data_ptr<float>();
        t.m1[i] = m1s[i].data_ptr<float>();
        t.m2[i] = m2s[i].data_ptr<float>();
        t.pw[i] = (unsigned short*)params[i].data_ptr();
        t.cum[i] = cum;
        cum += n;
    }
    t.cum[nt] = cum;
    return t;
}

void fused_adamw(std::vector<torch::Tensor> grads,
                 std::vector<torch::Tensor> masters,
                 std::vector<torch::Tensor> m1s,
                 std::vector<torch::Tensor> m2s,
                 std::vector<torch::Tensor> params,
                 double lr, double b1, double b2, double eps, double wd,
                 double max_norm, torch::Tensor partials, torch::Tensor norm,
                 torch::Tensor step_dev) {
    OptTable t = opt_table(grads, masters, m1s, m2s, params, partials, norm,
                           step_dev);
    hipStream_t s = cur_stream();
    launch_grad_norm(t, partials.data_ptr<float>(), norm.data_ptr<float>(),
                     step_dev.data_ptr<float>(), s);
    check_launch();
    launch_adamw(t, (float)lr, (float)b1, (float)b2, (float)eps, (float)wd,
                 (float)max_norm, norm.data_ptr<float>(),
                 step_dev.data_ptr<float>(), s);
    check_launch();
}

void fused_adamw_sched(std::vector<torch::Tensor> grads,
                       std::vector<torch::Tensor> masters,
                       std::vector<torch::Tensor> m1s,
                       std::vector<torch::Tensor> m2s,
                       std::vector<torch::Tensor> params,
                       std::vector<double> lr_scales,
                       std::vector<double> wds, double b1, double b2,
                       double eps, double max_norm, torch::Tensor partials,
                       torch::Tensor norm, torch::Tensor step_dev,
                       torch::Tensor hyper) {
    OptTable t = opt_table(grads, masters, m1s, m2s, params, partials, norm,
                           step_dev);
    const size_t nt = grads.size();
    TORCH_CHECK(lr_scales.size() == nt && wds.size() == nt,
                "fused_adamw_sched: one lr_scale and weight_decay per tensor");
    TORCH_CHECK(hyper.is_cuda() && hyper.is_contiguous()
                && hyper.numel() >= OPT_H_SIZE
                && hyper.scalar_type() == at::kFloat
                && hyper.device() == step_dev.device(),
                "fused_adamw_sched: hyper must be ", OPT_H_SIZE,
                " contiguous fp32 values on the optimizer's device");
    OptGroups h;
    std::memset(&h, 0, sizeof(h));
    for (size_t i = 0; i < nt; i++) {
        h.lr_scale[i] = (float)lr_scales[i];
        h.wd[i] = (float)wds[i];
    }
    hipStream_t s = cur_stream();
    launch_grad_norm_sched(t, partials.data_ptr<float>(),
                           norm.data_ptr<float>(),
                           step_dev.data_ptr<float>(),
                           hyper.data_ptr<float>(), s);
    check_launch();
    launch_adamw_sched(t, h, (float)b1, (float)b2, (float)eps,
                       (float)max_norm, norm.data_ptr<float>(),
                       step_dev.data_ptr<float>(), hyper.data_ptr<float>(),
                       s);
    check_launch();
}


torch::Tensor island_agreement(torch::Tensor levels, int64_t H, int64_t W,
                               int64_t connectivity) {
    CHECK_IN(levels);
    TORCH_CHECK(levels.dim() >= 3, "levels must be (*lead, N, L, D)");
    TORCH_CHECK(connectivity == 4 || connectivity == 8,
                "connectivity must be 4 or 8");
    const int64_t nd = levels.dim();
    const int64_t N = levels.size(nd - 3), L = levels.size(nd - 2),
                  D = levels.size(nd - 1);
    TORCH_CHECK(H > 0 && W > 0 && H * W == N, "grid does not match N");
    TORCH_CHECK(D % 8 == 0, "dim must be a multiple of 8");
    const int64_t C = connectivity == 4 ? 2 : 4;
    TORCH_CHECK(N * L * C < (1LL << 30), "grid too large (32-bit indices)");
    const int64_t P = N * L * D ? levels.numel() / (N * L * D) : 0;
    TORCH_CHECK((P * N * L + 3) / 4 <= INT32_MAX
                && (P * L * C * N + 255) / 256 <= INT32_MAX,
                "too many rows for one launch");
    std::vector<int64_t> shape(levels.sizes().begin(),
                               levels.sizes().end() - 3);
    shape.insert(shape.end(), {L, C, H, W});
    auto fopts = levels.options().dtype(at::kFloat);
    auto out = torch::empty(shape, fopts);
    auto norm = torch::empty({P * L, N}, fopts);
    hipStream_t s = cur_stream();
    launch_island_dots(levels.data_ptr(), norm.data_ptr<float>(),
                       out.data_ptr<float>(), P, (int)H, (int)W, (int)L,
                       (int)D, (int)C, s);
    check_launch();
    launch_island_finish(norm.data_ptr<float>(), out.data_ptr<float>(),
                         P * L, (int)H, (int)W, (int)C, s);
    check_launch();
    return out;
}

torch::Tensor island_labels(torch::Tensor agreement, double threshold) {
    TORCH_CHECK(agreement.is_cuda() && agreement.is_contiguous()
                && agreement.scalar_type() == at::kFloat,
                "agreement must be a contiguous f32 GPU tensor");
    TORCH_CHECK(agreement.dim() >= 4,
                "agreement must be (*lead, L, C, H, W)");
    const int64_t nd = agreement.dim();
    const int64_t C = agreement.size(nd - 3), H = agreement.size(nd - 2),
                  W = agreement.size(nd - 1);
    TORCH_CHECK(C == 2 || C == 4, "agreement must have 2 or 4 channels");
    TORCH_CHECK(H * W <= ISLAND_MAX_CELLS, "native labelling needs N <= ",
                ISLAND_MAX_CELLS);
    const int64_t cell = C * H * W;
    const int64_t PL = cell ? agreement.numel() / cell : 0;
    TORCH_CHECK(PL <= INT32_MAX, "too many (lead, level) problems");
    std::vector<int64_t> shape(agreement.sizes().begin(),
                               agreement.sizes().end() - 3);
    shape.insert(shape.end(), {H, W});
    auto labels = torch::empty(shape, agreement.options().dtype(at::kInt));
    launch_island_labels(agreement.data_ptr<float>(),
                         labels.data_ptr<int>(), PL, (int)H, (int)W, (int)C,
                         (float)threshold, cur_stream());
    check_launch();
    return labels;
}

std::vector<torch::Tensor> island_sizes(torch::Tensor labels,
                                        bool want_sizes, bool want_count) {
    TORCH_CHECK(labels.is_cuda() && labels.is_contiguous()
                && labels.scalar_type() == at::kInt,
                "labels must be a contiguous i32 GPU tensor");
    TORCH_CHECK(labels.dim() >= 2, "labels must be (*lead, H, W)");
    const int64_t nd = labels.dim();
    const int64_t N = labels.size(nd - 2) * labels.size(nd - 1);
    TORCH_CHECK(N <= ISLAND_MAX_CELLS, "native island sizes need N <= ",
                ISLAND_MAX_CELLS);
    TORCH_CHECK(N > 0, "empty grid");
    const int64_t PL = labels.numel() / N;
    TORCH_CHECK(PL <= INT32_MAX, "too many (lead, level) problems");
    std::vector<int64_t> cshape(labels.sizes().begin(),
                                labels.sizes().end() - 2);
    auto sizes = want_sizes ? torch::empty_like(labels)
                            : torch::empty({0}, labels.options());
    auto count = want_count ? torch::empty(cshape, labels.options())
                            : torch::empty({0}, labels.options());
    if (want_sizes || want_count) {
        launch_island_sizes(labels.data_ptr<int>(),
                            want_sizes ? sizes.data_ptr<int>() : nullptr,
                            want_count ? count.data_ptr<int>() : nullptr,
                            PL, (int)N, cur_stream());
        check_launch();
    }
    return {sizes, count};
}


std::vector<torch::Tensor> island_parents(torch::Tensor labels) {
    TORCH_CHECK(labels.is_cuda() && labels.is_contiguous()
                && labels.scalar_type() == at::kInt,
                "labels must be a contiguous i32 GPU tensor");
    TORCH_CHECK(labels.dim() >= 3, "labels must be (*lead, L, H, W)");
    const int64_t nd = labels.dim();
    const int64_t L = labels.size(nd - 3);
    const int64_t N = labels.size(nd - 2) * labels.size(nd - 1);
    TORCH_CHECK(N <= PARSE_MAX_CELLS, "native island parents need N <= ",
                PARSE_MAX_CELLS);
    TORCH_CHECK(N > 0 && L > 0, "empty grid");
    const int64_t PL = labels.numel() / N;
    TORCH_CHECK(PL <= INT32_MAX && L <= INT32_MAX,
                "too many (lead, level) problems");
    auto parents = torch::empty_like(labels);
    auto overlap = torch::empty_like(labels);
    launch_island_parents(labels.data_ptr<int>(), parents.data_ptr<int>(),
                          overlap.data_ptr<int>(), PL, (int)L, (int)N,
                          cur_stream());
    check_launch();
    return {parents, overlap};
}

torch::Tensor island_means(torch::Tensor levels, torch::Tensor labels,
                           bool broadcast, bool out_bf16) {
    CHECK_IN(levels);
    TORCH_CHECK(labels.is_cuda() && labels.is_contiguous()
                && labels.scalar_type() == at::kInt,
                "labels must be a contiguous i32 GPU tensor");
    TORCH_CHECK(labels.device() == levels.device(),
                "levels and labels must be on the same device");
    TORCH_CHECK(levels.dim() >= 3, "levels must be (*lead, N, L, D)");
    TORCH_CHECK(labels.dim() == levels.dim(),
                "labels must be (*lead, L, H, W) with the lead of levels");
    const int64_t nd = levels.dim();
    const int64_t N = levels.size(nd - 3), L = levels.size(nd - 2),
                  D = levels.size(nd - 1);
    for (int64_t i = 0; i < nd - 3; i++)
        TORCH_CHECK(labels.size(i) == levels.size(i),
                    "levels and labels must have equal lead dimensions");
    TORCH_CHECK(labels.size(nd - 3) == L
                && labels.size(nd - 2) * labels.size(nd - 1) == N,
                "labels do not match the N and L of levels");
    TORCH_CHECK(N > 0 && L > 0 && D > 0, "empty levels");
    TORCH_CHECK(N <= PARSE_MAX_CELLS, "native island means need N <= ",
                PARSE_MAX_CELLS);
    TORCH_CHECK(D % 8 == 0, "dim must be a multiple of 8");
    TORCH_CHECK((uintptr_t)levels.data_ptr() % 16 == 0,
                "levels must be 16-byte aligned");
    const int64_t P = levels.numel() / (N * L * D);
    TORCH_CHECK(P * L <= INT32_MAX && L * D <= INT32_MAX,
                "too many (lead, level) problems");
    auto out = torch::empty(
        levels.sizes(),
        levels.options().dtype(out_bf16 ? at::kBFloat16 : at::kFloat));
    launch_island_means(levels.data_ptr(), labels.data_ptr<int>(),
                        out.data_ptr(), P, (int)N, (int)L, (int)D, broadcast,
                        out_bf16, cur_stream());
    check_launch();
    return out;
}


static void check_nce_in(const torch::Tensor& x, const char* name) {
    TORCH_CHECK(x.is_cuda() && x.scalar_type() == at::kBFloat16
                && x.dim() == 2, name, " must be a 2-D bf16 GPU tensor");
    TORCH_CHECK(x.stride(1) == 1 && x.stride(0) % 8 == 0
                && x.size(1) % 8 == 0
                && ((uintptr_t)x.data_ptr() & 15) == 0,
                name, " needs unit column stride, dim and row stride "
                "multiples of 8 and a 16-byte aligned base");
}

static float* fptr(const torch::Tensor& t) { return t.data_ptr<float>(); }

static NceArgs nce_common(int64_t group, double temperature, bool all,
                          int64_t M) {
    NceArgs q;
    std::memset(&q, 0, sizeof(q));
    q.invt = (float)(1.0 / temperature);
    q.invm = (float)(1.0 / (double)M);
    q.group = (int)group;
    q.all = all ? 1 : 0;
    return q;
}

std::vector<torch::Tensor> nce_fwd(torch::Tensor a, torch::Tensor b,
                                   int64_t group, double temperature,
                                   bool all) {
    check_nce_in(a, "a"); check_nce_in(b, "b");
    TORCH_CHECK(a.sizes() == b.sizes(), "a and b must have equal shapes");
    const int64_t M = a.size(0), D = a.size(1);
    TORCH_CHECK(M > 0 && group > 0 && M % group == 0, "bad group size");
    TORCH_CHECK(temperature >= 0.03, "native path needs temperature >= 0.03");
    TORCH_CHECK(M <= (1LL << 30), "too many rows");
    auto fo = a.options().dtype(at::kFloat);
    hipStream_t s = cur_stream();
    const int64_t ntn = (M + 127) / 128;
    auto ra = torch::empty({M}, fo), rb = torch::empty({M}, fo);
    auto lse = torch::empty({M}, fo), pos = torch::empty({M}, fo);
    auto part = torch::empty({M, ntn}, fo);
    auto bpart = torch::empty({NCE_MAX_PARTS}, fo);
    auto loss = torch::empty({}, fo);
    launch_nce_rnorm(a.data_ptr(), a.stride(0), fptr(ra), M, (int)D, s);
    check_launch();
    launch_nce_rnorm(b.data_ptr(), b.stride(0), fptr(rb), M, (int)D, s);
    check_launch();
    GemmParams p = base_params(M, M, D, LAYOUT_NT, 1, 1, 1.0f);
    p.A.base = a.data_ptr(); p.A.ld = a.stride(0);
    p.B.base = b.data_ptr(); p.B.ld = b.stride(0);
    p.epilogue = EPI_NCE_FWD;
    NceArgs q = nce_common(group, temperature, all, M);
    q.rrow = fptr(ra); q.rcol = fptr(rb);
    q.part = fptr(part); q.pos = fptr(pos);
    nce_set(p, q);
    run_gemm(p, s, a.options(), true);
    launch_nce_loss(fptr(part), fptr(pos), fptr(lse), fptr(bpart),
                    fptr(loss), M, (int)ntn, q.invt, s);
    check_launch();
    return {loss, lse, ra, rb};
}

static torch::Tensor nce_bwd_side(const torch::Tensor& go,
                                  const torch::Tensor& x,
                                  const torch::Tensor& y,
                                  const torch::Tensor& rx,
                                  const torch::Tensor& ry,
                                  const torch::Tensor& lse, bool lse_by_col,
                                  int64_t group, double temperature, bool all,
                                  hipStream_t s) {
    const int64_t M = x.size(0), D = x.size(1);
    const int64_t ntn = (M + 127) / 128;
    int64_t Rc = (32LL << 20) / M;
    if (Rc >= 128) Rc -= Rc % 128;
    Rc = std::max<int64_t>(1, std::min(Rc, M));
    auto opts = x.options();
    auto ws = torch::empty({Rc, M}, opts);
    auto part = torch::empty({Rc, ntn}, opts.dtype(at::kFloat));
    auto dx = torch::empty({M, D}, opts);
    const int64_t tiles = ((Rc + 127) / 128) * ((D + 127) / 128);
    const int64_t sk = std::max<int64_t>(
        2, std::min<int64_t>({16, (512 + tiles - 1) / tiles, (M + 63) / 64}));
    auto acc = torch::empty({sk, Rc, D}, opts.dtype(at::kFloat));
    for (int64_t r0 = 0; r0 < M; r0 += Rc) {
        const int64_t rows = std::min(Rc, M - r0);
        {
            GemmParams p = base_params(rows, M, D, LAYOUT_NT, 1, 1, 1.0f);
            p.A.base = (const uint16_t*)x.data_ptr() + r0 * x.stride(0);
            p.A.ld = x.stride(0);
            p.B.base = y.data_ptr(); p.B.ld = y.stride(0);
            p.Cbase = ws.data_ptr(); p.Cld = M;
            p.epilogue = EPI_NCE_BWD;
            NceArgs q = nce_common(group, temperature, all, M);
            q.rrow = fptr(rx); q.rcol = fptr(ry);
            q.lse = fptr(lse); q.lse_col = lse_by_col ? 1 : 0;
            q.part = fptr(part);
            q.row0 = (int)r0;
            nce_set(p, q);
            run_gemm(p, s, opts, true);
        }
        {
            GemmParams p = base_params(rows, D, M, LAYOUT_NN, 1, 1, 1.0f);
            p.A.base = ws.data_ptr(); p.A.ld = M;
            p.B.base = y.data_ptr(); p.B.ld = y.stride(0);
            p.splitk = (int)sk; p.ws = fptr(acc);
            if (rows % 128 == 0 && D % 128 == 0 && M % 8 == 0)
                launch_gemm_nn_sk(p, s);
            else
                launch_gemm(p, s);
            check_launch();
        }
        launch_nce_grad_rows((uint16_t*)dx.data_ptr() + r0 * D, fptr(acc),
                             (int)sk,
                             (const uint16_t*)x.data_ptr() + r0 * x.stride(0),
                             x.stride(0), fptr(part), (int)ntn,
                             fptr(rx) + r0, fptr(go), rows, (int)D, s);
        check_launch();
    }
    return dx;
}

std::vector<torch::Tensor> nce_bwd(torch::Tensor go, torch::Tensor a,
                                   torch::Tensor b, torch::Tensor lse,
                                   torch::Tensor ra, torch::Tensor rb,
                                   int64_t group, double temperature,
                                   bool all, bool need_a, bool need_b) {
    check_nce_in(a, "a"); check_nce_in(b, "b");
    TORCH_CHECK(a.sizes() == b.sizes(), "a and b must have equal shapes");
    const int64_t M = a.size(0);
    TORCH_CHECK(M > 0 && group > 0 && M % group == 0, "bad group size");
    TORCH_CHECK(temperature >= 0.03, "native path needs temperature >= 0.03");
    auto isf = [&](const torch::Tensor& t, int64_t n) {
        return t.is_cuda() && t.is_contiguous()
               && t.scalar_type() == at::kFloat && t.numel() == n;
    };
    TORCH_CHECK(isf(go, 1) && isf(lse, M) && isf(ra, M) && isf(rb, M),
                "go / lse / ra / rb must be contiguous f32 GPU tensors");
    hipStream_t s = cur_stream();
    auto none = torch::empty({0}, a.options());
    auto dA = need_a ? nce_bwd_side(go, a, b, ra, rb, lse, false, group,
                                    temperature, all, s) : none;
    auto dB = need_b ? nce_bwd_side(go, b, a, rb, ra, lse, true, group,
                                    temperature, all, s) : none;
    return {dA, dB};
}

std::string build_info() {
    return "glom_pytorch_amd HIP extension (gfx950, bf16 MFMA 16x16x32)";
}

}

PYBIND11_MODULE(TORCH_EXTENSION_NAME, m) {
    m.def("grouped_ff_fwd", &grouped_ff_fwd, "grouped FF forward",
          py::arg("tokens"), py::arg("levels"), py::arg("pos"),
          py::arg("w1"), py::arg("b1"), py::arg("w2"), py::arg("b2"),
          py::arg("mode"), py::arg("save_for_bwd") = true,
          py::arg("group0_done") = false,
          py::arg("td_in") = c10::nullopt);
    m.def("grouped_ff_bwd", &grouped_ff_bwd, "grouped FF backward",
          py::arg("dY"), py::arg("tokens"), py::arg("levels"),
          py::arg("pos"), py::arg("w1"), py::arg("w2"),
          py::arg("Hpre"), py::arg("Hact"), py::arg("mode"),
          py::arg("w1t") = c10::nullopt,
          py::arg("w2t") = c10::nullopt,
          py::arg("td_in") = c10::nullopt, py::arg("g_lo") = 0);
    m.def("consensus_fwd", &consensus_fwd, "consensus attention forward",
          py::arg("levels"), py::arg("attend_self"), py::arg("mask"),
          py::arg("rnorm") = c10::nullopt);
    m.def("consensus_bwd", &consensus_bwd, "consensus attention backward",
          py::arg("dOut"), py::arg("levels"), py::arg("probs"),
          py::arg("rnorm"), py::arg("attend_self"), py::arg("mask"),
          py::arg("l_lo") = 0);
    m.def("level_mix_fwd", &level_mix_fwd, "level mix forward",
          py::arg("levels"), py::arg("bu"), py::arg("td"), py::arg("cons"),
          py::arg("slab") = c10::nullopt, py::arg("slab_idx") = 0,
          py::arg("bu0") = c10::nullopt);
    m.def("level_mix_fwd_next", &level_mix_fwd_next,
          "level mix forward, also emitting the next td_in / rnorm",
          py::arg("levels"), py::arg("bu"), py::arg("td"), py::arg("cons"),
          py::arg("slab") = c10::nullopt, py::arg("slab_idx") = 0,
          py::arg("bu0") = c10::nullopt, py::arg("pos") = c10::nullopt);
    m.def("level_mix_bwd", &level_mix_bwd, "level mix backward");
    m.def("glom_step_fwd", &glom_step_fwd, "full GLOM iteration forward",
          py::arg("tokens"), py::arg("levels"), py::arg("pos"),
          py::arg("bw1"), py::arg("bb1"), py::arg("bw2"), py::arg("bb2"),
          py::arg("tw1"), py::arg("tb1"), py::arg("tw2"), py::arg("tb2"),
          py::arg("attend_self"), py::arg("mask"),
          py::arg("slab") = c10::nullopt, py::arg("slab_idx") = 0,
          py::arg("save_for_bwd") = true, py::arg("bu0") = c10::nullopt,
          py::arg("td_in") = c10::nullopt, py::arg("rnorm") = c10::nullopt,
          py::arg("emit_next") = false);
    m.def("glom_step_bwd", &glom_step_bwd, "full GLOM iteration backward",
          py::arg("dnew"), py::arg("tokens"), py::arg("levels"),
          py::arg("pos"), py::arg("bw1"), py::arg("bw2"), py::arg("tw1"),
          py::arg("tw2"), py::arg("buHpre"), py::arg("buHact"),
          py::arg("tdHpre"), py::arg("tdHact"), py::arg("probs"),
          py::arg("rnorm"), py::arg("attend_self"), py::arg("mask"),
          py::arg("bw1t") = c10::nullopt, py::arg("bw2t") = c10::nullopt,
          py::arg("tw1t") = c10::nullopt, py::arg("tw2t") = c10::nullopt,
          py::arg("td_in") = c10::nullopt, py::arg("lo") = 0);
    m.def("patch_embed_fwd", &patch_embed_fwd,
          "patchify + embed GEMM (K1)");
    m.def("patch_embed_bwd", &patch_embed_bwd, "patch embed backward");
    m.def("dpos", &dpos, "positional embedding gradient reduction");
    m.def("colsum", &colsum, "fixed-order column sum (M,C) -> (C,)");
    m.def("fused_adamw", &fused_adamw,
          "fused AdamW + global-norm grad clip (torch semantics)");
    m.def("fused_adamw_sched", &fused_adamw_sched,
          "fused AdamW with device-resident lr schedule and per-tensor "
          "lr scale / weight decay");
    m.def("add4_into", &add4_into, "fused 4-way elementwise sum");
    m.def("ff_bwd_dh", &ff_bwd_dh, py::arg("dY"), py::arg("w2t"),
          py::arg("Hpre"), py::arg("g_lo") = 0);
    m.def("ff_bwd_dx", &ff_bwd_dx, py::arg("dHpre"), py::arg("w1t"),
          py::arg("tokens"), py::arg("B"), py::arg("N"), py::arg("L"),
          py::arg("mode"), py::arg("g_lo") = 0);
    m.def("ff_bwd_dw", &ff_bwd_dw, py::arg("dY"), py::arg("dHpre"),
          py::arg("tokens"), py::arg("levels"), py::arg("pos"),
          py::arg("Hact"), py::arg("mode"),
          py::arg("td_in") = c10::nullopt, py::arg("g_lo") = 0);
    m.def("set_nt8p", &set_nt8p, "toggle the 8-phase NT kernel (A/B)");
    m.def("set_tn_tr", &set_tn_tr,
          "toggle the transposed-read TN kernel (A/B, same bits)");
    m.def("set_tn_tr_mode", &set_tn_tr_mode,
          "0 never, 1 default policy, 2 every eligible TN call");
    m.def("get_tn_tr_mode", &get_tn_tr_mode);
    m.def("get_tn_tr_variant", &get_tn_tr_variant);
    m.def("set_tn_tr_variant", &set_tn_tr_variant,
          "split-K pipeline point of the transposed-read TN kernel (1..3)");
    m.def("set_finish_wide", &set_finish_wide,
          "toggle the re-blocked split-K finish (A/B, same bits)");
    m.def("gemm_tn", &gemm_tn, "C = A^T B per group (tests / tuning only)");
    m.def("gemm_nt", &gemm_nt, "C = A B^T + bias per group (tests only)",
          py::arg("A"), py::arg("B"), py::arg("bias") = c10::nullopt);
    m.def("gemm_nn", &gemm_nn, "C = A B per group (tests only)");
    m.def("set_wide_epilogue", &set_wide_epilogue,
          "toggle the 16-byte register epilogue of nt5p (A/B)");
    m.def("set_wide_epilogue_mode", &set_wide_epilogue_mode,
          "0 narrow, 1 per-epilogue default, 2 all wide, 3 wide aux only");
    m.def("get_wide_epilogue_mode", &get_wide_epilogue_mode);
    m.def("set_wide_epilogue_nt8p", &set_wide_epilogue_nt8p,
          "toggle the 16-byte register epilogue of nt8p (A/B)");
    m.def("set_gelu_pair", &set_gelu_pair,
          "toggle fused GELU-pair up-projection epilogue (A/B)");
    m.def("island_agreement", &island_agreement,
          "neighbour cosine agreement on the patch grid",
          py::arg("levels"), py::arg("H"), py::arg("W"),
          py::arg("connectivity"));
    m.def("island_labels", &island_labels,
          "connected components of the kept-edge graph (min-index labels)");
    m.def("island_sizes", &island_sizes,
          "island size at each root cell and/or island count",
          py::arg("labels"), py::arg("want_sizes") = true,
          py::arg("want_count") = true);
    m.def("island_parents", &island_parents,
          "parent label and overlap of every island one level up");
    m.def("island_means", &island_means,
          "mean level-state vector of every island",
          py::arg("levels"), py::arg("labels"), py::arg("broadcast"),
          py::arg("out_bf16"));
    m.def("nce_fwd", &nce_fwd,
          "column-contrastive loss forward: (M,D) bf16 a, b -> "
          "{loss, lse, ra, rb}");
    m.def("nce_bwd", &nce_bwd, "column-contrastive loss backward");
    m.def("set_nce_fast", &set_nce_fast,
          "A/B: host the EPI_NCE_* epilogues on gemm_nt_fast where eligible");
    m.def("nce_launch_counts", &nce_launch_counts,
          "EPI_NCE_* launches so far: {gemm_nt_fast, generic}");
    m.def("build_info", &build_info);
    m.def("bench_gemm", &bench_gemm, "raw GEMM microbench (tuning only)");
}
```

### glom_pytorch_amd/ops/csrc/native_ops.h

```cpp
#pragma once
#include <hip/hip_runtime.h>

void launch_patchify(const void* img, void* X, int B, int C, int H, int W,
                     int P, int Kp, hipStream_t s);
void launch_unpatchify(const void* dX, void* dImg, int B, int C, int H,
                       int W, int P, int Kp, hipStream_t s);
void launch_pad_cols(const void* src, void* dst, long rows, int Kin, int Kp,
                     hipStream_t s);
void launch_slice_cols(const void* src, void* dst, long rows, int Kp,
                       int Kin, hipStream_t s);
int colsum_rb(long M);
void launch_colsum(const void* in, float* partials, void* out, int nprob,
                   long M, long C, hipStream_t s);
void launch_colsum_fin(const float* partials, void* out, int nprob, long C,
                       int RB, hipStream_t s);
void launch_dpos(const void* dlev, void* out, float* partials, int BCH,
                 int B, int N, int L, int d, hipStream_t s);
void launch_zero_slice(void* out, long BN, int L, int d, int l0,
                       hipStream_t s);
void launch_zero_slices(void* out, long BN, int L, int d, int l0, int nl,
                        hipStream_t s);

#define OPT_MAX_T 24

struct OptTable {
    int nt;
    const unsigned short* g[OPT_MAX_T];
    float* mw[OPT_MAX_T];
    float* m1[OPT_MAX_T];
    float* m2[OPT_MAX_T];
    unsigned short* pw[OPT_MAX_T];
    long cum[OPT_MAX_T + 1];
};

#define OPT_NPART 1024

void launch_grad_norm(const OptTable& t, float* partials, float* norm,
                      float* step_dev, hipStream_t s);
void launch_adamw(const OptTable& t, float lr, float b1, float b2, float eps,
                  float wd, float max_norm, const float* norm,
                  const float* step_dev, hipStream_t s);

#define OPT_H_BASE_LR 0
#define OPT_H_KIND 1
#define OPT_H_WARMUP 2
#define OPT_H_TOTAL 3
#define OPT_H_MIN_RATIO 4
#define OPT_H_LR_T 5
#define OPT_H_SIZE 8

struct OptGroups {
    float lr_scale[OPT_MAX_T];
    float wd[OPT_MAX_T];
};

void launch_grad_norm_sched(const OptTable& t, float* partials, float* norm,
                            float* step_dev, float* hyper, hipStream_t s);
void launch_adamw_sched(const OptTable& t, const OptGroups& h, float b1,
                        float b2, float eps, float max_norm,
                        const float* norm, const float* step_dev,
                        const float* hyper, hipStream_t s);
```

### glom_pytorch_amd/ops/csrc/native_ops.hip

```cpp

#include "common.h"
#include "native_ops.h"

#define NT256 256

__host__ __device__ static inline long cdivl(long a, long b) {
    return (a + b - 1) / b;
}


__global__ __launch_bounds__(NT256) void k_patchify(
        const ushort_t* __restrict__ img, ushort_t* __restrict__ X,
        int B, int C, int H, int W, int P, int Kp) {
    const int S = W / P;
    const int K0 = P * P * C;
    long idx = (long)blockIdx.x * NT256 + threadIdx.x;
    long total = (long)B * (H / P) * S * Kp;
    if (idx >= total) return;
    int k = idx % Kp;
    long n = (idx / Kp) % ((long)(H / P) * S);
    long b = idx / ((long)Kp * (H / P) * S);
    ushort_t v = 0;
    if (k < K0) {
        int c = k % C;
        int p2 = (k / C) % P;
        int p1 = k / (C * P);
        int h = n / S, w = n % S;
        v = img[((b * C + c) * (long)H + h * P + p1) * W + w * P + p2];
    }
    X[idx] = v;
}

__global__ __launch_bounds__(NT256) void k_unpatchify(
        const ushort_t* __restrict__ dX, ushort_t* __restrict__ dImg,
        int B, int C, int H, int W, int P, int Kp) {
    const int S = W / P;
    long idx = (long)blockIdx.x * NT256 + threadIdx.x;
    long total = (long)B * C * H * W;
    if (idx >= total) return;
    int x = idx % W;
    int y = (idx / W) % H;
    int c = (idx / ((long)W * H)) % C;
    long b = idx / ((long)W * H * C);
    long n = (long)(y / P) * S + x / P;
    int k = ((y % P) * P + x % P) * C + c;
    dImg[idx] = dX[(b * ((long)(H / P) * S) + n) * Kp + k];
}

__global__ __launch_bounds__(NT256) void k_pad_cols(
        const ushort_t* __restrict__ src, ushort_t* __restrict__ dst,
        long rows, int Kin, int Kp) {
    long idx = (long)blockIdx.x * NT256 + threadIdx.x;
    if (idx >= rows * Kp) return;
    int k = idx % Kp;
    long r = idx / Kp;
    dst[idx] = (k < Kin) ? src[r * Kin + k] : (ushort_t)0;
}

__global__ __launch_bounds__(NT256) void k_slice_cols(
        const ushort_t* __restrict__ src, ushort_t* __restrict__ dst,
        long rows, int Kp, int Kin) {
    long idx = (long)blockIdx.x * NT256 + threadIdx.x;
    if (idx >= rows * Kin) return;
    int k = idx % Kin;
    long r = idx / Kin;
    dst[idx] = src[r * Kp + k];
}

void launch_patchify(const void* img, void* X, int B, int C, int H, int W,
                     int P, int Kp, hipStream_t s) {
    long total = (long)B * (H / P) * (W / P) * Kp;
    hipLaunchKernelGGL(k_patchify, dim3(cdivl(total, NT256)), dim3(NT256),
                       0, s, (const ushort_t*)img, (ushort_t*)X, B, C, H, W,
                       P, Kp);
}

void launch_unpatchify(const void* dX, void* dImg, int B, int C, int H,
                       int W, int P, int Kp, hipStream_t s) {
    long total = (long)B * C * H * W;
    hipLaunchKernelGGL(k_unpatchify, dim3(cdivl(total, NT256)), dim3(NT256),
                       0, s, (const ushort_t*)dX, (ushort_t*)dImg, B, C, H,
                       W, P, Kp);
}

void launch_pad_cols(const void* src, void* dst, long rows, int Kin, int Kp,
                     hipStream_t s) {
    hipLaunchKernelGGL(k_pad_cols, dim3(cdivl(rows * Kp, NT256)),
                       dim3(NT256), 0, s, (const ushort_t*)src,
                       (ushort_t*)dst, rows, Kin, Kp);
}

void launch_slice_cols(const void* src, void* dst, long rows, int Kp,
                       int Kin, hipStream_t s) {
    hipLaunchKernelGGL(k_slice_cols, dim3(cdivl(rows * Kin, NT256)),
                       dim3(NT256), 0, s, (const ushort_t*)src,
                       (ushort_t*)dst, rows, Kp, Kin);
}


int colsum_rb(long M) {
    long rb = cdivl(M, 64);
    return (int)(rb < 256 ? rb : 256);
}

__global__ __launch_bounds__(NT256) void k_colsum_part(
        const ushort_t* __restrict__ in, float* __restrict__ partials,
        long M, long C, int RB) {
    int rc = blockIdx.y;
    int p = blockIdx.z;
    long chunk = cdivl(M, RB);
    long r0 = rc * chunk, r1 = min((long)M, r0 + chunk);
    const ushort_t* base = in + (long)p * M * C;
    float* pout = partials + ((long)p * RB + rc) * C;
    if (C % 8 == 0) {
        long c8 = ((long)blockIdx.x * NT256 + threadIdx.x) * 8;
        if (c8 >= C) return;
        float acc[8] = {};
        for (long r = r0; r < r1; r++) {
            union { uint4v v; ushort_t u[8]; } t;
            t.v = *(const uint4v*)(base + r * C + c8);
#pragma unroll
            for (int e = 0; e < 8; e++) acc[e] += bf2f(t.u[e]);
        }
#pragma unroll
        for (int e = 0; e < 8; e++) pout[c8 + e] = acc[e];
        return;
    }
    long c = (long)blockIdx.x * NT256 + threadIdx.x;
    if (c >= C) return;
    float acc = 0.f;
    for (long r = r0; r < r1; r++) acc += bf2f(base[r * C + c]);
    pout[c] = acc;
}

#define CSF_NT 64
#define CSF_UNROLL 16
__global__ __launch_bounds__(CSF_NT) void k_colsum_fin(
        const float* __restrict__ partials, ushort_t* __restrict__ out,
        long C, int RB) {
    long c = (long)blockIdx.x * CSF_NT + threadIdx.x;
    int p = blockIdx.y;
    if (c >= C) return;
    const float* base = partials + (long)p * RB * C + c;
    float acc = 0.f;
    int rc = 0;
    for (; rc + CSF_UNROLL <= RB; rc += CSF_UNROLL) {
        float v[CSF_UNROLL];
#pragma unroll
        for (int u = 0; u < CSF_UNROLL; u++) v[u] = base[(long)(rc + u) * C];
#pragma unroll
        for (int u = 0; u < CSF_UNROLL; u++) acc += v[u];
    }
    for (; rc < RB; rc++) acc += base[(long)rc * C];
    out[(long)p * C + c] = f2bf(acc);
}

void launch_colsum(const void* in, float* partials, void* out, int nprob,
                   long M, long C, hipStream_t s) {
    int RB = colsum_rb(M);
    long ctiles = (C % 8 == 0) ? cdivl(C / 8, NT256) : cdivl(C, NT256);
    hipLaunchKernelGGL(k_colsum_part,
                       dim3(ctiles, RB, nprob), dim3(NT256), 0, s,
                       (const ushort_t*)in, partials, M, C, RB);
    hipLaunchKernelGGL(k_colsum_fin, dim3(cdivl(C, CSF_NT), nprob),
                       dim3(CSF_NT), 0, s, partials, (ushort_t*)out, C, RB);
}

void launch_colsum_fin(const float* partials, void* out, int nprob, long C,
                       int RB, hipStream_t s) {
    hipLaunchKernelGGL(k_colsum_fin, dim3(cdivl(C, CSF_NT), nprob),
                       dim3(CSF_NT), 0, s, partials, (ushort_t*)out, C, RB);
}


__global__ __launch_bounds__(NT256) void k_dpos_part(
        const ushort_t* __restrict__ dlev, float* __restrict__ partials,
        int B, int N, int L, int d, int BCH) {
    long q8 = ((long)blockIdx.x * NT256 + threadIdx.x) * 8;
    int n = blockIdx.y;
    int bc = blockIdx.z;
    if (q8 >= d) return;
    int bchunk = (B + BCH - 1) / BCH;
    int b0 = bc * bchunk, b1 = min(B, b0 + bchunk);
    float acc[8] = {};
    const long bstride = (long)N * L * d;
    const ushort_t* base = dlev + ((long)n * L + 1) * d + q8;
    for (int b = b0; b < b1; b++) {
        const ushort_t* p = base + b * bstride;
        for (int l = 0; l < L - 1; l++) {
            union { uint4v v; ushort_t u[8]; } t;
            t.v = *(const uint4v*)(p + (long)l * d);
#pragma unroll
            for (int e = 0; e < 8; e++) acc[e] += bf2f(t.u[e]);
        }
    }
    float* pout = partials + ((long)bc * N + n) * d + q8;
#pragma unroll
    for (int e = 0; e < 8; e++) pout[e] = acc[e];
}

__global__ __launch_bounds__(NT256) void k_dpos_fin(
        const float* __restrict__ partials, ushort_t* __restrict__ out,
        long Nd, int BCH) {
    long i = (long)blockIdx.x * NT256 + threadIdx.x;
    if (i >= Nd) return;
    float acc = 0.f;
    for (int bc = 0; bc < BCH; bc++) acc += partials[(long)bc * Nd + i];
    out[i] = f2bf(acc);
}

__global__ __launch_bounds__(NT256) void k_dpos(
        const ushort_t* __restrict__ dlev, ushort_t* __restrict__ out,
        int B, int N, int L, int d) {
    int q = blockIdx.x * NT256 + threadIdx.x;
    int n = blockIdx.y;
    if (q >= d) return;
    float acc = 0.f;
    const long bstride = (long)N * L * d;
    const ushort_t* base = dlev + ((long)n * L + 1) * d + q;
    for (int b = 0; b < B; b++) {
        const ushort_t* p = base + b * bstride;
        for (int l = 0; l < L - 1; l++) acc += bf2f(p[(long)l * d]);
    }
    out[(long)n * d + q] = f2bf(acc);
}

void launch_dpos(const void* dlev, void* out, float* partials, int BCH,
                 int B, int N, int L, int d, hipStream_t s) {
    if (d % 8 == 0 && partials != nullptr && BCH > 0) {
        hipLaunchKernelGGL(k_dpos_part,
                           dim3(cdivl(d / 8, NT256), N, BCH), dim3(NT256),
                           0, s, (const ushort_t*)dlev, partials, B, N, L,
                           d, BCH);
        hipLaunchKernelGGL(k_dpos_fin,
                           dim3(cdivl((long)N * d, NT256)), dim3(NT256), 0,
                           s, partials, (ushort_t*)out, (long)N * d, BCH);
        return;
    }
    hipLaunchKernelGGL(k_dpos, dim3(cdivl(d, NT256), N), dim3(NT256), 0, s,
                       (const ushort_t*)dlev, (ushort_t*)out, B, N, L, d);
}


__global__ __launch_bounds__(NT256) void k_zero_slice(
        ushort_t* __restrict__ out, long BN, int L, int d, int l0) {
    long i8 = ((long)blockIdx.x * NT256 + threadIdx.x) * 8;
    if (i8 >= BN * d) return;
    int q = i8 % d;
    long bn = i8 / d;
    uint4v z = {0, 0, 0, 0};
    *(uint4v*)(out + (bn * L + l0) * (long)d + q) = z;
}

void launch_zero_slice(void* out, long BN, int L, int d, int l0,
                       hipStream_t s) {
    hipLaunchKernelGGL(k_zero_slice, dim3(cdivl(BN * d / 8, NT256)),
                       dim3(NT256), 0, s, (ushort_t*)out, BN, L, d, l0);
}

__global__ __launch_bounds__(NT256) void k_zero_slices(
        ushort_t* __restrict__ out, long BN, long Ld, long w, long off) {
    long i8 = ((long)blockIdx.x * NT256 + threadIdx.x) * 8;
    if (i8 >= BN * w) return;
    long q = i8 % w;
    long bn = i8 / w;
    uint4v z = {0, 0, 0, 0};
    *(uint4v*)(out + bn * Ld + off + q) = z;
}

void launch_zero_slices(void* out, long BN, int L, int d, int l0, int nl,
                        hipStream_t s) {
    if (nl <= 0 || BN <= 0) return;
    const long w = (long)nl * d;
    hipLaunchKernelGGL(k_zero_slices, dim3(cdivl(BN * w / 8, NT256)),
                       dim3(NT256), 0, s, (ushort_t*)out, BN, (long)L * d, w,
                       (long)l0 * d);
}


__global__ __launch_bounds__(NT256) void k_grad_norm_part(
        OptTable t, float* __restrict__ partials) {
    long gid = (long)blockIdx.x * NT256 + threadIdx.x;
    const long gstride = (long)OPT_NPART * NT256;
    float acc = 0.f;
    for (int ti = 0; ti < t.nt; ti++) {
        const ushort_t* g = t.g[ti];
        long n = t.cum[ti + 1] - t.cum[ti];
        for (long i = gid; i < n; i += gstride) {
            float v = bf2f(g[i]);
            acc = fmaf(v, v, acc);
        }
    }
    __shared__ float red[NT256 / WAVE];
    acc = wave_reduce_sum(acc);
    if (threadIdx.x % WAVE == 0) red[threadIdx.x / WAVE] = acc;
    __syncthreads();
    if (threadIdx.x == 0) {
        float s = 0.f;
        for (int w = 0; w < NT256 / WAVE; w++) s += red[w];
        partials[blockIdx.x] = s;
    }
}

__global__ __launch_bounds__(NT256) void k_grad_norm_fin(
        const float* __restrict__ partials, float* __restrict__ norm,
        float* __restrict__ step_dev) {
    __shared__ float red[NT256 / WAVE];
    float acc = 0.f;
    for (int i = threadIdx.x; i < OPT_NPART; i += NT256) acc += partials[i];
    acc = wave_reduce_sum(acc);
    if (threadIdx.x % WAVE == 0) red[threadIdx.x / WAVE] = acc;
    __syncthreads();
    if (threadIdx.x == 0) {
        float s = 0.f;
        for (int w = 0; w < NT256 / WAVE; w++) s += red[w];
        norm[0] = sqrtf(s);
        step_dev[0] += 1.0f;
    }
}

__global__ __launch_bounds__(NT256) void k_adamw(
        OptTable t, float lr, float b1, float b2, float eps, float wd,
        float max_norm, const float* __restrict__ norm,
        const float* __restrict__ step_dev) {
    const float tstep = step_dev[0];
    float scale = 1.0f;
    if (max_norm > 0.f) {
        float c = max_norm / (norm[0] + 1e-6f);
        scale = fminf(1.0f, c);
    }
    const float bc1 = 1.0f - __powf(b1, tstep);
    const float bc2 = 1.0f - __powf(b2, tstep);
    const float step_size = lr / bc1;
    const float inv_bc2 = 1.0f / bc2;
    const float decay = 1.0f - lr * wd;

    long gid = (long)blockIdx.x * NT256 + threadIdx.x;
    const long gstride = (long)gridDim.x * NT256;
    for (int ti = 0; ti < t.nt; ti++) {
        const ushort_t* gp = t.g[ti];
        float* mw = t.mw[ti];
        float* m1 = t.m1[ti];
        float* m2 = t.m2[ti];
        ushort_t* pw = t.pw[ti];
        long n = t.cum[ti + 1] - t.cum[ti];
        for (long i = gid; i < n; i += gstride) {
            float g = bf2f(gp[i]) * scale;
            float m = fmaf(b1, m1[i], (1.0f - b1) * g);
            float v = fmaf(b2, m2[i], (1.0f - b2) * g * g);
            m1[i] = m;
            m2[i] = v;
            float p = mw[i] * decay;
            p -= step_size * m / (sqrtf(v * inv_bc2) + eps);
            mw[i] = p;
            pw[i] = f2bf(p);
        }
    }
}

__global__ __launch_bounds__(NT256) void k_grad_norm_fin_sched(
        const float* __restrict__ partials, float* __restrict__ norm,
        float* __restrict__ step_dev, float* __restrict__ hyper) {
    __shared__ float red[NT256 / WAVE];
    float acc = 0.f;
    for (int i = threadIdx.x; i < OPT_NPART; i += NT256) acc += partials[i];
    acc = wave_reduce_sum(acc);
    if (threadIdx.x % WAVE == 0) red[threadIdx.x / WAVE] = acc;
    __syncthreads();
    if (threadIdx.x == 0) {
        float s = 0.f;
        for (int w = 0; w < NT256 / WAVE; w++) s += red[w];
        norm[0] = sqrtf(s);
        const float tstep = step_dev[0] + 1.0f;
        step_dev[0] = tstep;

        const float si = tstep - 1.0f;
        const int kind = (int)hyper[OPT_H_KIND];
        const float W = hyper[OPT_H_WARMUP];
        const float T = hyper[OPT_H_TOTAL];
        const float mr = hyper[OPT_H_MIN_RATIO];
        float f;
        if (si < W) {
            f = (si + 1.0f) / W;
        } else if (kind == 0) {
            f = 1.0f;
        } else if (si >= T) {
            f = mr;
        } else {
            const float x = (si - W) / (T - W);
            const float shape = kind == 1
                ? 1.0f - x
                : 0.5f * (1.0f + cosf(3.14159265358979323846f * x));
            f = mr + (1.0f - mr) * shape;
        }
        hyper[OPT_H_LR_T] = hyper[OPT_H_BASE_LR] * f;
    }
}

__global__ __launch_bounds__(NT256) void k_adamw_sched(
        OptTable t, OptGroups h, float b1, float b2, float eps,
        float max_norm, const float* __restrict__ norm,
        const float* __restrict__ step_dev,
        const float* __restrict__ hyper) {
#pragma clang fp contract(off)
    const float tstep = step_dev[0];
    const float lr_t = hyper[OPT_H_LR_T];
    float scale = 1.0f;
    if (max_norm > 0.f) {
        float c = max_norm / (norm[0] + 1e-6f);
        scale = fminf(1.0f, c);
    }
    const float bc1 = 1.0f - __powf(b1, tstep);
    const float bc2 = 1.0f - __powf(b2, tstep);
    const float inv_bc2 = 1.0f / bc2;

    long gid = (long)blockIdx.x * NT256 + threadIdx.x;
    const long gstride = (long)gridDim.x * NT256;
    for (int ti = 0; ti < t.nt; ti++) {
        const float lr = lr_t * h.lr_scale[ti];
        const float wd = h.wd[ti];
        const float step_size = lr / bc1;
        const float decay = fmaf(-lr, wd, 1.0f);
        const ushort_t* gp = t.g[ti];
        float* mw = t.mw[ti];
        float* m1 = t.m1[ti];
        float* m2 = t.m2[ti];
        ushort_t* pw = t.pw[ti];
        long n = t.cum[ti + 1] - t.cum[ti];
        for (long i = gid; i < n; i += gstride) {
            float g = bf2f(gp[i]) * scale;
            float m = fmaf(b1, m1[i], (1.0f - b1) * g);
            float v = fmaf(b2, m2[i], (1.0f - b2) * g * g);
            m1[i] = m;
            m2[i] = v;
            float p = mw[i] * decay;
            p -= step_size * m / (sqrtf(v * inv_bc2) + eps);
            mw[i] = p;
            pw[i] = f2bf(p);
        }
    }
}

void launch_grad_norm_sched(const OptTable& t, float* partials, float* norm,
                            float* step_dev, float* hyper, hipStream_t s) {
    hipLaunchKernelGGL(k_grad_norm_part, dim3(OPT_NPART), dim3(NT256), 0, s,
                       t, partials);
    hipLaunchKernelGGL(k_grad_norm_fin_sched, dim3(1), dim3(NT256), 0, s,
                       partials, norm, step_dev, hyper);
}

void launch_adamw_sched(const OptTable& t, const OptGroups& h, float b1,
                        float b2, float eps, float max_norm,
                        const float* norm, const float* step_dev,
                        const float* hyper, hipStream_t s) {
    hipLaunchKernelGGL(k_adamw_sched, dim3(2048), dim3(NT256), 0, s, t, h,
                       b1, b2, eps, max_norm, norm, step_dev, hyper);
}

void launch_grad_norm(const OptTable& t, float* partials, float* norm,
                      float* step_dev, hipStream_t s) {
    hipLaunchKernelGGL(k_grad_norm_part, dim3(OPT_NPART), dim3(NT256), 0, s,
                       t, partials);
    hipLaunchKernelGGL(k_grad_norm_fin, dim3(1), dim3(NT256), 0, s,
                       partials, norm, step_dev);
}

void launch_adamw(const OptTable& t, float lr, float b1, float b2, float eps,
                  float wd, float max_norm, const float* norm,
                  const float* step_dev, hipStream_t s) {
    hipLaunchKernelGGL(k_adamw, dim3(2048), dim3(NT256), 0, s, t, lr, b1,
                       b2, eps, wd, max_norm, norm, step_dev);
}
```

### glom_pytorch_amd/ops/functional.py

```python

from __future__ import annotations

import os

import torch

from glom_pytorch_amd.ops import _load_extension


class PatchEmbedFn(torch.autograd.Function):

    @staticmethod
    def forward(ctx, img, w, b, patch_size):
        ext = _load_extension()
        tokens, X = ext.patch_embed_fwd(img.contiguous(), w, b, patch_size)
        ctx.save_for_backward(X, w)
        ctx.patch = patch_size
        ctx.img_hw = (img.shape[2], img.shape[3])
        return tokens

    @staticmethod
    def backward(ctx, dTokens):
        ext = _load_extension()
        X, w = ctx.saved_tensors
        need_dimg = ctx.needs_input_grad[0]
        dW, dB, dImg = ext.patch_embed_bwd(
            dTokens.contiguous(), X, w, ctx.patch, ctx.img_hw[0],
            ctx.img_hw[1], need_dimg)
        return (dImg if need_dimg else None), dW, dB, None


class LinearFixedBiasGradFn(torch.autograd.Function):

    @staticmethod
    def forward(ctx, x, w, b):
        ctx.save_for_backward(x, w)
        return torch.nn.functional.linear(x, w, b)

    @staticmethod
    def backward(ctx, g):
        ext = _load_extension()
        x, w = ctx.saved_tensors
        g2 = g.reshape(-1, g.shape[-1]).contiguous()
        x2 = x.reshape(-1, x.shape[-1])
        dx = g2.mm(w).view_as(x) if ctx.needs_input_grad[0] else None
        dw = g2.t().mm(x2) if ctx.needs_input_grad[1] else None
        db = ext.colsum(g2) if ctx.needs_input_grad[2] else None
        return dx, dw, db


class ContrastFn(torch.autograd.Function):

    @staticmethod
    def forward(ctx, a, b, group, temperature, all_negatives):
        ext = _load_extension()
        loss, lse, ra, rb = ext.nce_fwd(a, b, group, temperature,
                                        all_negatives)
        ctx.save_for_backward(a, b, lse, ra, rb)
        ctx.cfg = (group, temperature, all_negatives)
        return loss

    @staticmethod
    def backward(ctx, go):
        ext = _load_extension()
        a, b, lse, ra, rb = ctx.saved_tensors
        need_a, need_b = ctx.needs_input_grad[0], ctx.needs_input_grad[1]
        go = go.to(torch.float32).reshape(1).contiguous()
        dA, dB = ext.nce_bwd(go, a, b, lse, ra, rb, *ctx.cfg, need_a,
                             need_b)
        return (dA if need_a else None), (dB if need_b else None), \
            None, None, None


class TrajectoryFn(torch.autograd.Function):

    @staticmethod
    def forward(ctx, slab, *steps):
        return slab

    @staticmethod
    def backward(ctx, dtraj):
        return (None,) + tuple(dtraj[t] for t in range(dtraj.shape[0]))


class GroupedFFFn(torch.autograd.Function):

    @staticmethod
    def forward(ctx, tokens, levels, pos, w1, b1, w2, b2, mode):
        ext = _load_extension()
        Y, Hpre, Hact, td_in = ext.grouped_ff_fwd(tokens, levels, pos, w1,
                                                  b1, w2, b2, mode)
        ctx.save_for_backward(tokens, levels, pos, w1, w2, Hpre, Hact,
                              td_in)
        ctx.mode = mode
        return Y

    @staticmethod
    def backward(ctx, dY):
        ext = _load_extension()
        tokens, levels, pos, w1, w2, Hpre, Hact, td_in = ctx.saved_tensors
        dTokens, dLevels, dW1, dB1, dW2, dB2 = ext.grouped_ff_bwd(
            dY.contiguous(), tokens, levels, pos, w1, w2, Hpre, Hact,
            ctx.mode, None, None, td_in)
        dPos = None
        if ctx.mode == 1 and pos is not None and ctx.needs_input_grad[2]:
            dPos = ext.dpos(dLevels)
        if ctx.mode == 0:
            return dTokens, dLevels, None, dW1, dB1, dW2, dB2, None
        return None, dLevels, dPos, dW1, dB1, dW2, dB2, None


class ConsensusFn(torch.autograd.Function):

    @staticmethod
    def forward(ctx, levels, attend_self, mask):
        ext = _load_extension()
        out, probs, rnorm = ext.consensus_fwd(levels, attend_self, mask)
        ctx.save_for_backward(levels, probs, rnorm, mask)
        ctx.attend_self = attend_self
        return out

    @staticmethod
    def backward(ctx, dOut):
        ext = _load_extension()
        levels, probs, rnorm, mask = ctx.saved_tensors
        dLevels = ext.consensus_bwd(dOut.contiguous(), levels, probs, rnorm,
                                    ctx.attend_self, mask)
        return dLevels, None, None


class LevelMixFn(torch.autograd.Function):

    @staticmethod
    def forward(ctx, levels, bu, td, cons):
        ext = _load_extension()
        return ext.level_mix_fwd(levels, bu, td, cons)

    @staticmethod
    def backward(ctx, dout):
        ext = _load_extension()
        dmix, dtd = ext.level_mix_bwd(dout.contiguous())
        return dmix, dmix.view_as(dmix), dtd, dmix.view_as(dmix)


class GlomStepFn(torch.autograd.Function):

    _streams = None

    @staticmethod
    def _side_streams():
        if GlomStepFn._streams is None:
            GlomStepFn._streams = (torch.cuda.Stream(), torch.cuda.Stream(),
                                   torch.cuda.Stream())
        return GlomStepFn._streams

    @staticmethod
    def forward(ctx, tokens, levels, pos, bw1, bb1, bw2, bb2,
                tw1, tb1, tw2, tb2, attend_self, mask,
                bw1t, bw2t, tw1t, tw2t, slab_ref=None,
                save_for_bwd=True, cone=None, carry=None):
        ext = _load_extension()
        bu0 = carry.bu0 if carry is not None and carry.skip0 else None
        td_ready = carry.td_in if carry is not None else None
        rn_ready = carry.rnorm if carry is not None else None
        emit = carry is not None and carry.emit
        slab, sidx = slab_ref if slab_ref is not None else (None, 0)
        lo = cone[0] if cone is not None else 0
        save_td = save_for_bwd and (lo < levels.size(2) - 1
                                    or FORCE_SAVE_FOR_BWD)
        if (torch.is_grad_enabled()
                and os.environ.get("GLOM_FWD_STREAMS", "0") != "1"):
            (out, bhp, bha, thp, tha, probs, rnorm,
             tdin) = ext.glom_step_fwd(
                tokens, levels, pos, bw1, bb1, bw2, bb2, tw1, tb1, tw2,
                tb2, attend_self, mask, slab, sidx, save_for_bwd)
            if carry is not None:
                carry.set_next(None, None)
        else:
            cur = torch.cuda.current_stream()
            s_td, s_at, _ = GlomStepFn._side_streams()
            ev = torch.cuda.Event()
            ev.record(cur)
            buY, bhp, bha, _ = ext.grouped_ff_fwd(tokens, levels, None,
                                                  bw1, bb1, bw2, bb2, 0,
                                                  save_for_bwd,
                                                  bu0 is not None)
            with torch.cuda.stream(s_td):
                s_td.wait_event(ev)
                tdY, thp, tha, tdin = ext.grouped_ff_fwd(None, levels, pos,
                                                         tw1, tb1, tw2,
                                                         tb2, 1,
                                                         save_td, False,
                                                         td_ready)
            with torch.cuda.stream(s_at):
                s_at.wait_event(ev)
                cons, probs, rnorm = ext.consensus_fwd(levels, attend_self,
                                                       mask, rn_ready)
            cur.wait_stream(s_td)
            cur.wait_stream(s_at)
            for t in (tdY, thp, tha, tdin, cons, probs, rnorm):
                if t.numel():
                    t.record_stream(cur)
            if emit:
                out, td_next, rn_next = ext.level_mix_fwd_next(
                    levels, buY, tdY, cons, slab, sidx, bu0, pos)
                carry.set_next(td_next, rn_next)
            else:
                out = ext.level_mix_fwd(levels, buY, tdY, cons, slab, sidx,
                                        bu0)
                if carry is not None:
                    carry.set_next(None, None)
            if carry is not None and carry.hoist and carry.bu0 is None:
                carry.bu0 = buY[:, :, 0, :]
        ctx.save_for_backward(tokens, levels, pos, bw1, bw2, tw1, tw2,
                              bhp, bha, thp, tha, probs, rnorm, mask,
                              bw1t, bw2t, tw1t, tw2t, tdin)
        ctx.attend_self = attend_self
        ctx.cone = cone
        return out

    @staticmethod
    def backward(ctx, dnew):
        ext = _load_extension()
        (tokens, levels, pos, bw1, bw2, tw1, tw2, bhp, bha, thp, tha,
         probs, rnorm, mask, bw1t, bw2t, tw1t, tw2t,
         tdin) = ctx.saved_tensors
        L = levels.size(2)
        lo = ctx.cone[0] if ctx.cone is not None else 0
        if lo > 0 and CHECK_LEVEL_CONE:
            _check_cone(dnew, lo, ctx.cone[1])
        td_lo = min(lo, L - 1)
        td_live = td_lo < L - 1
        if os.environ.get("GLOM_NO_BWD_STREAMS", "0") == "1":
            (dTokens, dLevels, dPos, dbw1, dbb1, dbw2, dbb2,
             dtw1, dtb1, dtw2, dtb2) = ext.glom_step_bwd(
                dnew.contiguous(), tokens, levels, pos, bw1, bw2, tw1, tw2,
                bhp, bha, thp, tha, probs, rnorm, ctx.attend_self, mask,
                bw1t, bw2t, tw1t, tw2t, tdin, lo)
            return (dTokens, dLevels, dPos, dbw1, dbb1, dbw2, dbb2,
                    dtw1, dtb1, dtw2, dtb2, None, None, None, None, None,
                    None, None, None, None, None)
        if os.environ.get("GLOM_BWD_FORK", "3") == "3":
            cur = torch.cuda.current_stream()
            s_td, s_at, _ = GlomStepFn._side_streams()
            dmix, dtd = ext.level_mix_bwd(dnew.contiguous())
            ev = torch.cuda.Event()
            ev.record(cur)
            bu = ext.grouped_ff_bwd(dmix, tokens, levels, None, bw1, bw2,
                                    bhp, bha, 0, bw1t, bw2t, None, lo)
            if td_live:
                with torch.cuda.stream(s_td):
                    s_td.wait_event(ev)
                    td = ext.grouped_ff_bwd(dtd, None, levels, pos, tw1,
                                            tw2, thp, tha, 1, tw1t, tw2t,
                                            tdin, td_lo)
                dtd.record_stream(s_td)
            else:
                td = ext.grouped_ff_bwd(dtd, None, levels, pos, tw1, tw2,
                                        thp, tha, 1, tw1t, tw2t, tdin,
                                        td_lo)
            with torch.cuda.stream(s_at):
                s_at.wait_event(ev)
                dAttn = ext.consensus_bwd(dmix, levels, probs, rnorm,
                                          ctx.attend_self, mask, lo)
            dmix.record_stream(s_at)
            if td_live:
                cur.wait_stream(s_td)
            cur.wait_stream(s_at)
            for t in (list(td) if td_live else []) + [dAttn]:
                if t is not None and t.numel():
                    t.record_stream(cur)
            dLevels = torch.empty_like(levels)
            ext.add4_into(dmix, bu[1], td[1], dAttn, dLevels)
            dPos = ext.dpos(td[1])
            return (bu[0], dLevels, dPos, bu[2], bu[3], bu[4], bu[5],
                    td[2], td[3], td[4], td[5], None, None, None, None,
                    None, None, None, None, None, None)
        B, N = levels.size(0), levels.size(1)
        cur = torch.cuda.current_stream()
        s_td, s_at, s_w = GlomStepFn._side_streams()
        dmix, dtd = ext.level_mix_bwd(dnew.contiguous())
        ev0 = torch.cuda.Event()
        ev0.record(cur)
        bu_dh, bu_db1 = ext.ff_bwd_dh(dmix, bw2t, bhp, lo)
        ev_bu = torch.cuda.Event()
        ev_bu.record(cur)
        if td_live:
            with torch.cuda.stream(s_td):
                s_td.wait_event(ev0)
                td_dh, td_db1 = ext.ff_bwd_dh(dtd, tw2t, thp, td_lo)
                ev_td = torch.cuda.Event()
                ev_td.record(s_td)
        else:
            (_, td_dl, td_w1, td_db1, td_w2, td_b2) = ext.grouped_ff_bwd(
                dtd, None, levels, pos, tw1, tw2, thp, tha, 1, tw1t, tw2t,
                tdin, td_lo)
        with torch.cuda.stream(s_at):
            s_at.wait_event(ev0)
            dAttn = ext.consensus_bwd(dmix, levels, probs, rnorm,
                                      ctx.attend_self, mask, lo)
        with torch.cuda.stream(s_w):
            s_w.wait_event(ev_bu)
            bu_w1, bu_w2, bu_b2 = ext.ff_bwd_dw(dmix, bu_dh, tokens,
                                                levels, None, bha, 0, None,
                                                lo)
            if td_live:
                s_w.wait_event(ev_td)
                td_w1, td_w2, td_b2 = ext.ff_bwd_dw(dtd, td_dh, None,
                                                    levels, pos, tha, 1,
                                                    tdin, td_lo)
        bu_dt, bu_dl = ext.ff_bwd_dx(bu_dh, bw1t, tokens, B, N, L, 0, lo)
        if td_live:
            with torch.cuda.stream(s_td):
                _, td_dl = ext.ff_bwd_dx(td_dh, tw1t, None, B, N, L, 1,
                                         td_lo)
        pins = [(dmix, s_at), (dmix, s_w), (bu_dh, s_w)]
        if td_live:
            pins += [(dtd, s_td), (dtd, s_w), (td_dh, s_w)]
        for t, st in pins:
            t.record_stream(st)
        if td_live:
            cur.wait_stream(s_td)
        cur.wait_stream(s_at)
        cur.wait_stream(s_w)
        back = [dAttn, bu_w1, bu_w2, bu_b2]
        if td_live:
            back += [td_db1, td_dl, td_w1, td_w2, td_b2]
        for t in back:
            t.record_stream(cur)
        dLevels = torch.empty_like(levels)
        ext.add4_into(dmix, bu_dl, td_dl, dAttn, dLevels)
        dPos = ext.dpos(td_dl)
        return (bu_dt, dLevels, dPos, bu_w1, bu_db1, bu_w2, bu_b2,
                td_w1, td_db1, td_w2, td_b2, None, None, None, None, None,
                None, None, None, None, None)


def _transposed_weights(model):
    with torch.no_grad():
        L, d = model.levels, model.dim
        bw1 = model.bottom_up.net[1].weight[..., 0]
        bw2 = model.bottom_up.net[3].weight[..., 0]
        tw1 = model.top_down.net[1].weight[..., 0]
        tw2 = model.top_down.net[3].weight[..., 0]
        m4 = bw1.shape[0] // L
        return (
            bw1.view(L, m4, d).transpose(1, 2).contiguous(),
            bw2.view(L, d, m4).transpose(1, 2).contiguous(),
            tw1.view(L - 1, m4, d).transpose(1, 2).contiguous(),
            tw2.view(L - 1, d, m4).transpose(1, 2).contiguous(),
        )


FORCE_SAVE_FOR_BWD = os.environ.get("GLOM_SAVE_HPRE", "0") == "1"


CHECK_LEVEL_CONE = os.environ.get("GLOM_CHECK_LEVEL_CONE", "0") == "1"


def set_check_level_cone(on: bool) -> None:
    global CHECK_LEVEL_CONE
    CHECK_LEVEL_CONE = bool(on)


TOKEN_HOIST = True
MIX_FUSION = True


def set_token_hoist(on: bool) -> None:
    global TOKEN_HOIST
    TOKEN_HOIST = bool(on)


def set_mix_fusion(on: bool) -> None:
    global MIX_FUSION
    MIX_FUSION = bool(on)


class _LoopCarry:

    def __init__(self, levels):
        two = levels.size(2) >= 2
        self.hoist = (two and TOKEN_HOIST and
                      os.environ.get("GLOM_NO_TOKEN_HOIST", "0") != "1")
        self.fuse = (two and MIX_FUSION and
                     os.environ.get("GLOM_NO_MIX_FUSION", "0") != "1")
        self.bu0 = None
        self.skip0 = False
        self.td_in = None
        self.rnorm = None
        self.emit = False

    def set_next(self, td_in, rnorm):
        ok = td_in is not None and td_in.numel() > 0
        self.td_in = td_in if ok else None
        self.rnorm = rnorm if ok else None

    def tensors(self):
        return [t for t in (self.bu0, self.td_in, self.rnorm)
                if t is not None]


def level_cone_lo(loss_level_min: int, grad_iters: int, t: int) -> int:
    return max(0, loss_level_min - (grad_iters - 1 - t))


def _check_cone(dnew, lo, t):
    if torch.cuda.is_current_stream_capturing():
        raise RuntimeError(
            "the level-cone check synchronises with the host and cannot "
            "run under stream capture; turn it off (set_check_level_cone"
            "(False), GLOM_CHECK_LEVEL_CONE=0) or run the step uncaptured")
    bad = dnew[:, :, :lo].ne(0).any(dim=3).any(dim=1).any(dim=0).tolist()
    if any(bad):
        lvl = bad.index(True)
        raise RuntimeError(
            f"loss_level_min promise broken: the gradient arriving at "
            f"iteration {t} is non-zero in level {lvl}, below the first "
            f"level ({lo}) that loss_level_min allows there")


def _needs_bwd(*tensors):
    if FORCE_SAVE_FOR_BWD:
        return True
    return torch.is_grad_enabled() and any(
        t is not None and t.requires_grad for t in tensors)


def glom_step(model, tokens, levels, pos, mask, wts=None, slab_ref=None,
              cone=None, carry=None):
    bw = model.bottom_up.net
    tw = model.top_down.net
    if wts is None:
        wts = (None, None, None, None)
    args = (tokens, levels, pos,
            bw[1].weight[..., 0], bw[1].bias, bw[3].weight[..., 0],
            bw[3].bias,
            tw[1].weight[..., 0], tw[1].bias, tw[3].weight[..., 0],
            tw[3].bias)
    if carry is not None:
        records_bwd = torch.is_grad_enabled() and any(
            t is not None and t.requires_grad for t in args)
        carry.skip0 = carry.bu0 is not None and (
            not records_bwd or (cone is not None and cone[0] >= 1))
    return GlomStepFn.apply(
        *args, model.attention.attend_self, mask, *wts, slab_ref,
        _needs_bwd(*args), cone, carry)


_TAIL_STREAM = None
_TAIL_KEEP = []


def _tail_stream():
    global _TAIL_STREAM
    if _TAIL_STREAM is None:
        _TAIL_STREAM = torch.cuda.Stream()
    return _TAIL_STREAM


def join_tail_stream():
    if _TAIL_STREAM is not None:
        torch.cuda.current_stream().wait_stream(_TAIL_STREAM)
    del _TAIL_KEEP[:]


def glom_forward(model, img, iters, levels=None, return_all=False,
                 grad_iters=None, overlap_tail=False, loss_level_min=None):
    from glom_pytorch_amd.utils.profiling import trace_range
    if loss_level_min is not None:
        if grad_iters is None:
            raise ValueError("loss_level_min requires grad_iters")
        if not 0 <= loss_level_min < model.levels:
            raise ValueError("loss_level_min must be a level index")
    b = img.shape[0]
    with trace_range("glom/patch_embed"):
        emb = model.image_to_tokens[1]
        tokens = PatchEmbedFn.apply(img, emb.weight, emb.bias,
                                    model.patch_size)
    n = tokens.shape[1]
    pos = model.pos_emb.weight
    mask = (model.attention.non_local_mask
            if model.attention.local_consensus_radius > 0 else None)

    if levels is None:
        levels = model.init_levels.view(1, 1, model.levels, model.dim) \
            .expand(b, n, model.levels, model.dim).contiguous()
    else:
        levels = levels.contiguous()

    wts = _transposed_weights(model) if torch.is_grad_enabled() else None

    slab = None
    if return_all:
        slab = torch.empty((iters + 1,) + tuple(levels.shape),
                           device=levels.device, dtype=levels.dtype)
        with torch.no_grad():
            slab[0].copy_(levels)

    overlap = (overlap_tail and grad_iters is not None
               and grad_iters < iters and img.is_cuda
               and torch.is_grad_enabled())
    n_sync = grad_iters if overlap else iters

    carry = _LoopCarry(levels)

    steps = [levels]
    with trace_range(f"glom/iterate x{iters}"):
        for t in range(n_sync):
            sref = (slab, t + 1) if slab is not None else None
            carry.emit = carry.fuse and t < iters - 1
            with trace_range(f"glom/step{t}"):
                if grad_iters is not None and t >= grad_iters:
                    with torch.no_grad():
                        levels = glom_step(model, tokens, levels, pos,
                                           mask, wts, sref, None, carry)
                else:
                    cone = None
                    if loss_level_min is not None:
                        cone = (level_cone_lo(loss_level_min, grad_iters,
                                              t), t)
                    levels = glom_step(model, tokens, levels, pos, mask,
                                       wts, sref, cone, carry)
            if return_all:
                steps.append(levels)
        if overlap:
            ext = _load_extension()
            bw = model.bottom_up.net
            tw = model.top_down.net
            s_tail = _tail_stream()
            ev = torch.cuda.Event()
            ev.record(torch.cuda.current_stream())
            for kept in carry.tensors():
                kept.record_stream(s_tail)
            _TAIL_KEEP[:] = carry.tensors()
            with torch.no_grad(), torch.cuda.stream(s_tail):
                s_tail.wait_event(ev)
                for t in range(n_sync, iters):
                    emit = carry.fuse and t < iters - 1
                    outs = ext.glom_step_fwd(
                        tokens, levels, pos,
                        bw[1].weight[..., 0], bw[1].bias,
                        bw[3].weight[..., 0], bw[3].bias,
                        tw[1].weight[..., 0], tw[1].bias,
                        tw[3].weight[..., 0], tw[3].bias,
                        model.attention.attend_self, mask, slab, t + 1,
                        FORCE_SAVE_FOR_BWD, carry.bu0, carry.td_in,
                        carry.rnorm, emit)
                    levels = outs[0]
                    if emit:
                        carry.set_next(outs[8], outs[9])
                    else:
                        carry.set_next(None, None)
                    if return_all:
                        steps.append(levels)
                if slab is not None:
                    slab.record_stream(s_tail)

    if return_all:
        return TrajectoryFn.apply(slab, *steps)
    return levels
```

### glom_pytorch_amd/parallel/trainer.py

```python

from __future__ import annotations

import json
import os
import time
import warnings

import torch
import torch.distributed as dist
import torch.nn.functional as F
from einops.layers.torch import Rearrange
from torch import nn

from glom_pytorch_amd.parallel.ddp import BucketedDDP
from glom_pytorch_amd.parallel.failure import Heartbeat


class _DecoderLinear(nn.Linear):

    def forward(self, x):
        if (x.is_cuda and x.dtype == torch.bfloat16
                and self.bias is not None and torch.is_grad_enabled()):
            from glom_pytorch_amd.ops.functional import LinearFixedBiasGradFn
            return LinearFixedBiasGradFn.apply(x, self.weight, self.bias)
        return super().forward(x)


class DenoisingDecoder(nn.Sequential):

    def __init__(self, dim: int, image_size: int, patch_size: int):
        side = image_size // patch_size
        super().__init__(
            _DecoderLinear(dim, patch_size ** 2 * 3),
            Rearrange("b (h w) (p1 p2 c) -> b c (h p1) (w p2)",
                      h=side, w=side, p1=patch_size, p2=patch_size),
        )


class DenoisingTrainer:
    def __init__(self, model, *, lr=3e-4, noise_std=1.0, decode_step=7,
                 grad_clip=1.0, distributed=False, bucket_bytes=16 << 20,
                 process_group=None, graph_step=True, overlap_tail=True,
                 micro_batches=1, log_path=None, contrast_weight=0.0,
                 contrast_level=-1, contrast_temperature=0.1,
                 contrast_negatives="other_images", level_cone=True,
                 lr_schedule=None, no_decay=False):
        from glom_pytorch_amd.contrast import NEGATIVES
        from glom_pytorch_amd.ops.optim import LRSchedule
        if lr_schedule is not None and not isinstance(lr_schedule,
                                                      LRSchedule):
            raise ValueError("lr_schedule must be an LRSchedule or None")
        self.base_lr = float(lr)
        self.lr_schedule = lr_schedule
        self.no_decay = bool(no_decay)
        if contrast_weight < 0 or not contrast_temperature > 0:
            raise ValueError("contrast_weight must be >= 0 and "
                             "contrast_temperature > 0")
        if contrast_negatives not in NEGATIVES:
            raise ValueError(f"contrast_negatives must be one of {NEGATIVES}")
        self.contrast_weight = float(contrast_weight)
        self.contrast_level = int(contrast_level)
        self.contrast_temperature = float(contrast_temperature)
        self.contrast_negatives = contrast_negatives
        self.model = model
        self.dim = model.dim
        self.decode_step = decode_step
        self.noise_std = noise_std
        p = next(model.parameters())
        self.decoder = DenoisingDecoder(
            model.dim, model.image_size, model.patch_size
        ).to(p.device, p.dtype)
        self.distributed = distributed and dist.is_initialized()
        self.ddp_model = self.ddp_dec = self.heartbeat = None
        if self.distributed:
            self.ddp_model = BucketedDDP(model, bucket_bytes,
                                         process_group=process_group)
            self.ddp_dec = BucketedDDP(self.decoder, bucket_bytes,
                                       process_group=process_group)
            self.heartbeat = Heartbeat(every_steps=50)
        params = list(model.parameters()) + list(self.decoder.parameters())
        self._params = params
        names = ([n for n, _ in model.named_parameters()]
                 + ["decoder." + n
                    for n, _ in self.decoder.named_parameters()])
        wds = [0.0 if self.no_decay and (
                   q.ndim <= 1 or n in ("pos_emb.weight", "init_levels"))
               else 1e-2 for n, q in zip(names, params)]

        def torch_adamw(tensors):
            if not self.no_decay:
                return torch.optim.AdamW(tensors, lr=lr, foreach=True)
            groups: dict = {}
            for t, w in zip(tensors, wds):
                groups.setdefault(w, []).append(t)
            return torch.optim.AdamW(
                [{"params": ts, "weight_decay": w}
                 for w, ts in groups.items()], lr=lr, foreach=True)
        self.master = None
        self.fused_opt = None
        if p.dtype == torch.bfloat16:
            self.master = [q.detach().float().requires_grad_(False)
                           for q in params]
            if p.is_cuda and self._ops_available():
                from glom_pytorch_amd.ops.optim import FusedAdamW
                self.fused_opt = FusedAdamW(
                    params, self.master, lr=lr,
                    weight_decay=wds if self.no_decay else 1e-2,
                    max_grad_norm=grad_clip if grad_clip else 0.0,
                    schedule=lr_schedule)
                self.opt = self.fused_opt
            else:
                self.opt = torch_adamw(self.master)
        else:
            self.opt = torch_adamw(params)
        self.grad_clip = grad_clip
        self.step_idx = 0
        self.log_path = log_path
        self.graph_step = (graph_step
                           and os.environ.get("GLOM_NO_GRAPH_STEP", "0")
                           != "1")
        self.level_cone = (level_cone
                           and os.environ.get("GLOM_NO_LEVEL_CONE", "0")
                           != "1")
        self.overlap_tail = (overlap_tail
                             and os.environ.get("GLOM_NO_OVERLAP_TAIL",
                                                "0") != "1")
        self.micro_batches = int(os.environ.get("GLOM_MICRO_BATCHES",
                                                str(micro_batches)))
        self._micro_stream = None
        self._graphs: dict = {}

    def _loss_level_min(self, contrast: bool = False):
        if not self.level_cone:
            return None
        L = self.model.levels
        return min(L - 1, self.contrast_level % L) if contrast else L - 1

    @staticmethod
    def _ops_available():
        from glom_pytorch_amd import ops
        return ops.available()

    def _torch_opt_step(self):
        if self.lr_schedule is not None:
            lr = self.base_lr * self.lr_schedule.factor(self.step_idx)
            for g in self.opt.param_groups:
                g["lr"] = lr
        self.opt.step()

    def current_lr(self) -> float:
        if self.fused_opt is not None:
            return self.fused_opt.current_lr()
        return float(self.opt.param_groups[0]["lr"])


    def step(self, img: torch.Tensor, iters: int | None = None,
             sync_loss: bool = True):
        iters = iters if iters is not None else 2 * self.model.levels
        if self._graph_usable(img):
            loss = self._graphed_step(img, iters)
        else:
            loss = self._eager_step(img, iters)
        self.step_idx += 1
        if self.heartbeat is not None:
            self.heartbeat.tick()
        return loss.item() if sync_loss else loss.detach()

    def _graph_usable(self, img) -> bool:
        return (self.graph_step and self.micro_batches == 1
                and self.fused_opt is not None
                and not self.fused_opt._uses_device_lr()
                and img.is_cuda and img.dtype == torch.bfloat16
                and not getattr(self.model, "force_eager", False)
                and os.environ.get("GLOM_FORCE_EAGER", "0") != "1")

    def _eager_step(self, img: torch.Tensor, iters: int) -> torch.Tensor:
        if self.contrast_weight > 0:
            return self._contrast_step(img, iters)
        m = self.micro_batches
        if (m > 1 and img.is_cuda and img.shape[0] % m == 0
                and not getattr(self.model, "force_eager", False)):
            return self._micro_step(img, iters, m)
        t = min(self.decode_step, iters)
        self.opt.zero_grad(set_to_none=True)
        noised = img + torch.randn_like(img) * self.noise_std
        overlap = (self.overlap_tail and img.is_cuda
                   and not getattr(self.model, "force_eager", False))
        all_levels = self.model(noised, iters=iters, return_all=True,
                                grad_iters=t, overlap_tail=overlap,
                                loss_level_min=self._loss_level_min())
        top = all_levels[t, :, :, -1]
        recon = self.decoder(top)
        loss = F.mse_loss(recon.float(), img.float())
        loss.backward()
        if self.distributed:
            self.ddp_model.finalize()
            self.ddp_dec.finalize()
        if overlap:
            from glom_pytorch_amd.ops.functional import join_tail_stream
            join_tail_stream()
        if self.fused_opt is not None:
            self.fused_opt.step()
        elif self.master is not None:
            with torch.no_grad():
                for mw, q in zip(self.master, self._params):
                    mw.grad = q.grad.float() if q.grad is not None else None
                if self.grad_clip:
                    torch.nn.utils.clip_grad_norm_(self.master,
                                                   self.grad_clip)
                self._torch_opt_step()
                for mw, q in zip(self.master, self._params):
                    q.data.copy_(mw)
        else:
            if self.grad_clip:
                torch.nn.utils.clip_grad_norm_(
                    [q for g in self.opt.param_groups for q in g["params"]],
                    self.grad_clip)
            self._torch_opt_step()
        return loss.detach()

    def _contrast_step(self, img: torch.Tensor, iters: int) -> torch.Tensor:
        from glom_pytorch_amd.contrast import column_contrastive_loss
        if self.micro_batches > 1:
            raise NotImplementedError(
                "contrast_weight > 0 does not support micro_batches > 1")
        t = min(self.decode_step, iters)
        B = img.shape[0]
        self.opt.zero_grad(set_to_none=True)
        noised = torch.cat(
            (img + torch.randn_like(img) * self.noise_std,
             img + torch.randn_like(img) * self.noise_std))
        overlap = (self.overlap_tail and img.is_cuda
                   and not getattr(self.model, "force_eager", False))
        all_levels = self.model(noised, iters=iters, return_all=True,
                                grad_iters=t, overlap_tail=overlap,
                                loss_level_min=self._loss_level_min(True))
        recon = self.decoder(all_levels[t, :, :, -1])
        clean = torch.cat((img, img))
        loss = F.mse_loss(recon.float(), clean.float())
        lvl = all_levels[t, :, :, self.contrast_level]
        loss = loss + self.contrast_weight * column_contrastive_loss(
            lvl[:B], lvl[B:], temperature=self.contrast_temperature,
            negatives=self.contrast_negatives)
        loss.backward()
        if self.distributed:
            self.ddp_model.finalize()
            self.ddp_dec.finalize()
        if overlap:
            from glom_pytorch_amd.ops.functional import join_tail_stream
            join_tail_stream()
        if self.fused_opt is not None:
            self.fused_opt.step()
        elif self.master is not None:
            with torch.no_grad():
                for mw, q in zip(self.master, self._params):
                    mw.grad = q.grad.float() if q.grad is not None else None
                if self.grad_clip:
                    torch.nn.utils.clip_grad_norm_(self.master,
                                                   self.grad_clip)
                self._torch_opt_step()
                for mw, q in zip(self.master, self._params):
                    q.data.copy_(mw)
        else:
            if self.grad_clip:
                torch.nn.utils.clip_grad_norm_(
                    [q for g in self.opt.param_groups for q in g["params"]],
                    self.grad_clip)
            self._torch_opt_step()
        return loss.detach()

    def _micro_forward(self, half: torch.Tensor, iters: int, t: int,
                       scale: float) -> torch.Tensor:
        noised = half + torch.randn_like(half) * self.noise_std
        traj = self.model(noised, iters=iters, return_all=True,
                          grad_iters=t, overlap_tail=True,
                          loss_level_min=self._loss_level_min())
        recon = self.decoder(traj[t, :, :, -1])
        return F.mse_loss(recon.float(), half.float()) * scale

    def _micro_step(self, img: torch.Tensor, iters: int,
                    m: int) -> torch.Tensor:
        t = min(self.decode_step, iters)
        self.opt.zero_grad(set_to_none=True)
        if self._micro_stream is None:
            self._micro_stream = torch.cuda.Stream()
        s_f = self._micro_stream
        halves = img.chunk(m)
        if self.distributed:
            self.ddp_model.set_accumulate(True)
            self.ddp_dec.set_accumulate(True)
        cur = torch.cuda.current_stream()
        losses = []
        pending = self._micro_forward(halves[0], iters, t, 1.0 / m)
        for i in range(1, m):
            ev = torch.cuda.Event()
            ev.record(cur)
            with torch.cuda.stream(s_f):
                s_f.wait_event(ev)
                nxt = self._micro_forward(halves[i], iters, t, 1.0 / m)
            pending.backward()
            losses.append(pending.detach())
            if self.distributed and i == m - 1:
                self.ddp_model.set_accumulate(False)
                self.ddp_dec.set_accumulate(False)
                self.ddp_model._reset_counts()
                self.ddp_dec._reset_counts()
            pending = nxt
        pending.backward()
        losses.append(pending.detach())
        cur.wait_stream(s_f)
        if self.distributed:
            self.ddp_model.finalize()
            self.ddp_dec.finalize()
        from glom_pytorch_amd.ops.functional import join_tail_stream
        join_tail_stream()
        loss = losses[0]
        for l in losses[1:]:
            loss = loss + l
        if self.fused_opt is not None:
            self.fused_opt.step()
        elif self.master is not None:
            with torch.no_grad():
                for mw, q in zip(self.master, self._params):
                    mw.grad = (q.grad.float() if q.grad is not None
                               else None)
                if self.grad_clip:
                    torch.nn.utils.clip_grad_norm_(self.master,
                                                   self.grad_clip)
                self._torch_opt_step()
                for mw, q in zip(self.master, self._params):
                    q.data.copy_(mw)
        else:
            self._torch_opt_step()
        return loss.detach()


    def _graphed_step(self, img: torch.Tensor, iters: int) -> torch.Tensor:
        key = (tuple(img.shape), iters)
        entry = self._graphs.get(key)
        if entry is None:
            entry = self._capture(img, iters)
            self._graphs[key] = entry
        if entry is False:
            return self._eager_step(img, iters)
        entry["img"].copy_(img)
        entry["graph"].replay()
        self.fused_opt.note_replays(1)
        return entry["loss"]

    def _capture(self, img: torch.Tensor, iters: int):
        if self.distributed and os.environ.get("GLOM_GRAPH_DIST",
                                               "1") == "0":
            return False
        try:
            static_img = img.clone()
            fo = self.fused_opt
            with torch.no_grad():
                snap = ([m.clone() for m in self.master]
                        + [t.clone() for t in fo.exp_avg]
                        + [t.clone() for t in fo.exp_avg_sq]
                        + [q.detach().clone() for q in self._params]
                        + [fo._step_dev.clone()])
            s = torch.cuda.Stream()
            s.wait_stream(torch.cuda.current_stream())
            with torch.cuda.stream(s):
                for _ in range(2):
                    self._eager_step(static_img, iters)
            torch.cuda.current_stream().wait_stream(s)
            with torch.no_grad():
                live = (self.master + fo.exp_avg + fo.exp_avg_sq
                        + [q.data for q in self._params] + [fo._step_dev])
                for dst, src in zip(live, snap):
                    dst.copy_(src)
                fo._step_host = max(0, fo._step_host - 2)
            for q in self._params:
                q.grad = None
            graph = torch.cuda.CUDAGraph()
            import gc
            gc.collect()
            gc_was_enabled = gc.isenabled()
            gc.disable()
            try:
                with torch.cuda.graph(graph,
                                      capture_error_mode="thread_local"):
                    loss = self._eager_step(static_img, iters)
            finally:
                if gc_was_enabled:
                    gc.enable()
            fo._step_host = max(0, fo._step_host - 1)
            return {"graph": graph, "img": static_img, "loss": loss}
        except Exception as e:
            warnings.warn(f"training-step hipGraph capture failed "
                          f"({type(e).__name__}: {e}); using eager "
                          f"launches")
            return False

    def log(self, **metrics):
        if self.log_path:
            with open(self.log_path, "a") as f:
                f.write(json.dumps({"step": self.step_idx,
                                    "time": time.time(), **metrics}) + "\n")


    def save_checkpoint(self, path: str):
        if self.distributed and dist.get_rank() != 0:
            return
        tmp = path + ".tmp"
        torch.save({
            "model": self.model.state_dict(),
            "decoder": self.decoder.state_dict(),
            "optimizer": self.opt.state_dict(),
            "master": self.master,
            "step": self.step_idx,
            "lr_schedule": (self.lr_schedule.to_dict()
                            if self.lr_schedule is not None else None),
            "base_lr": (self.fused_opt.lr if self.fused_opt is not None
                        else self.base_lr),
            "no_decay": self.no_decay,
            "rng": torch.get_rng_state(),
            "cuda_rng": (torch.cuda.get_rng_state()
                         if torch.cuda.is_available() else None),
        }, tmp)
        os.replace(tmp, path)

    def load_checkpoint(self, path: str):
        ckpt = torch.load(path, map_location="cpu", weights_only=False)
        if bool(ckpt.get("no_decay", False)) != self.no_decay:
            raise ValueError(
                f"checkpoint was written with no_decay="
                f"{bool(ckpt.get('no_decay', False))}, this trainer has "
                f"no_decay={self.no_decay}")
        self.model.load_state_dict(ckpt["model"])
        self.decoder.load_state_dict(ckpt["decoder"])
        self.opt.load_state_dict(ckpt["optimizer"])
        if "lr_schedule" in ckpt:
            from glom_pytorch_amd.ops.optim import LRSchedule
            d = ckpt["lr_schedule"]
            self.lr_schedule = (LRSchedule.from_dict(d) if d is not None
                                else None)
            self.base_lr = float(ckpt["base_lr"])
            if self.fused_opt is not None:
                self.fused_opt._lr = self.base_lr
                self.fused_opt.schedule = self.lr_schedule
        if ckpt.get("master") is not None and self.master is not None:
            for mw, saved in zip(self.master, ckpt["master"]):
                mw.data.copy_(saved.to(mw.device))
        self.step_idx = ckpt["step"]
        if self.master is not None:
            with torch.no_grad():
                for mw, q in zip(self.master, self._params):
                    q.data.copy_(mw.to(q.dtype))
        torch.set_rng_state(ckpt["rng"])
        if ckpt.get("cuda_rng") is not None and torch.cuda.is_available():
            torch.cuda.set_rng_state(ckpt["cuda_rng"])
        self._graphs.clear()
        return self
```

Before: 1968 images/sec.

## Merge per-step backward gradient sums and carry next-step level-mix gradient

Adds a merged backward path for GLOM steps. A single grad_merge kernel sums the four per-level gradient contributions and also emits the next step's level-mix gradient, replacing separate add4 and mix_bwd launches. Zero fills are skipped, bias gradients come from a cone-limited column sum, and the trajectory gradient is routed straight to step t instead of materialising a full trajectory gradient. This cuts kernel launches and memory passes in backward, at the cost of more intricate cone-range bookkeeping and a carry object whose correctness relies on pointer matching between steps.

```diff
diff --git a/glom_pytorch_amd/ops/__init__.py b/glom_pytorch_amd/ops/__init__.py
--- a/glom_pytorch_amd/ops/__init__.py
+++ b/glom_pytorch_amd/ops/__init__.py
@@ -59,6 +59,16 @@
     functional.set_mix_fusion(on)
 
 
+def set_bwd_merge(on: bool) -> None:
+    from glom_pytorch_amd.ops import functional
+    functional.set_bwd_merge(on)
+
+
+def trajectory_at(all_levels, t):
+    from glom_pytorch_amd.ops import functional
+    return functional.trajectory_at(all_levels, t)
+
+
 def set_check_level_cone(on: bool) -> None:
     from glom_pytorch_amd.ops import functional
     functional.set_check_level_cone(on)
diff --git a/glom_pytorch_amd/ops/csrc/aux_kernels.h b/glom_pytorch_amd/ops/csrc/aux_kernels.h
--- a/glom_pytorch_amd/ops/csrc/aux_kernels.h
+++ b/glom_pytorch_amd/ops/csrc/aux_kernels.h
@@ -24,6 +24,15 @@
 bool mix_fwd_can_emit_next(int L, int d);
 void launch_mix_bwd(const void* dout, void* dmix, void* dtd, long total,
                     int L, int d, hipStream_t s);
+void launch_mix_bwd_lo(const void* dout, void* dmix, long BN, int L, int d,
+                       int lo, hipStream_t s);
+struct MergeRanges {
+    int a_lo, a_hi, b_lo, b_hi, c_lo, c_hi, d_lo, d_hi, dead;
+};
+void launch_grad_merge(const void* a, const void* b, const void* c,
+                       const void* dd, void* out, void* dmix_next,
+                       long total, int L, int d, const MergeRanges& r,
+                       bool posz, hipStream_t s);
 void launch_add4(const void* a, const void* b, const void* c, const void* d,
                  void* out, long total, hipStream_t s);
 void launch_gelu(const void* in, void* out, long total, hipStream_t s);
diff --git a/glom_pytorch_amd/ops/csrc/aux_kernels.hip b/glom_pytorch_amd/ops/csrc/aux_kernels.hip
--- a/glom_pytorch_amd/ops/csrc/aux_kernels.hip
+++ b/glom_pytorch_amd/ops/csrc/aux_kernels.hip
@@ -313,6 +313,59 @@
     if (has_td) *(uint4v*)(dtd + (bn * (L - 1) + l) * (long)d + q) = o.v;
 }
 
+__global__ __launch_bounds__(NTHREADS) void k_mix_bwd_lo(
+        const ushort_t* __restrict__ dout, ushort_t* __restrict__ dmix,
+        long live, int L, int d, int lo) {
+    long i8 = ((long)blockIdx.x * NTHREADS + threadIdx.x) * 8;
+    if (i8 >= live) return;
+    const long w = (long)(L - lo) * d;
+    long bn = i8 / w;
+    long r = i8 % w;
+    int l = lo + (int)(r / d);
+    long idx = bn * (long)L * d + (long)lo * d + r;
+    union { uint4v v; ushort_t u[8]; } g, o;
+    g.v = *(const uint4v*)(dout + idx);
+    float c = (l < L - 1) ? 4.0f : 3.0f;
+#pragma unroll
+    for (int e = 0; e < 8; e++) o.u[e] = f2bf(bf2f(g.u[e]) / c);
+    *(uint4v*)(dmix + idx) = o.v;
+}
+
+template <bool NEXT>
+__global__ __launch_bounds__(NTHREADS) void k_grad_merge(
+        const ushort_t* __restrict__ a, const ushort_t* __restrict__ b,
+        const ushort_t* __restrict__ c, const ushort_t* __restrict__ dd,
+        ushort_t* __restrict__ out, ushort_t* __restrict__ dmix_next,
+        long total, int L, int d, MergeRanges r, int posz) {
+    long idx = ((long)blockIdx.x * NTHREADS + threadIdx.x) * 8;
+    if (idx >= total) return;
+    int l = (idx / d) % L;
+    union { uint4v v; ushort_t u[8]; } va, vb, vc, vd, o;
+    const uint4v z = {0, 0, 0, 0};
+    if (l < r.dead) {
+        *(uint4v*)(out + idx) = z;
+        return;
+    }
+    va.v = (l >= r.a_lo && l < r.a_hi) ? *(const uint4v*)(a + idx) : z;
+    vb.v = (l >= r.b_lo && l < r.b_hi) ? *(const uint4v*)(b + idx) : z;
+    vc.v = (l >= r.c_lo && l < r.c_hi) ? *(const uint4v*)(c + idx) : z;
+    vd.v = (l >= r.d_lo && l < r.d_hi) ? *(const uint4v*)(dd + idx) : z;
+#pragma unroll
+    for (int e = 0; e < 8; e++) {
+        ushort_t v = f2bf(bf2f(va.u[e]) + bf2f(vb.u[e]) + bf2f(vc.u[e])
+                          + bf2f(vd.u[e]));
+        if (posz && v == 0x8000) v = 0;
+        o.u[e] = v;
+    }
+    *(uint4v*)(out + idx) = o.v;
+    if (NEXT) {
+        float cl = (l < L - 1) ? 4.0f : 3.0f;
+#pragma unroll
+        for (int e = 0; e < 8; e++) o.u[e] = f2bf(bf2f(o.u[e]) / cl);
+        *(uint4v*)(dmix_next + idx) = o.v;
+    }
+}
+
 __global__ __launch_bounds__(NTHREADS) void k_add_pos(
         const ushort_t* __restrict__ levels, const ushort_t* __restrict__ pos,
         ushort_t* __restrict__ out, long total, int N, int L, int d) {
@@ -411,6 +464,35 @@
                        (ushort_t*)dtd, total, L, d);
 }
 
+void launch_mix_bwd_lo(const void* dout, void* dmix, long BN, int L, int d,
+                       int lo, hipStream_t s) {
+    const long live = BN * (long)(L - lo) * d;
+    if (live <= 0) return;
+    hipLaunchKernelGGL(k_mix_bwd_lo, dim3(cdiv(live / 8, NTHREADS)),
+                       dim3(NTHREADS), 0, s, (const ushort_t*)dout,
+                       (ushort_t*)dmix, live, L, d, lo);
+}
+
+void launch_grad_merge(const void* a, const void* b, const void* c,
+                       const void* dd, void* out, void* dmix_next,
+                       long total, int L, int d, const MergeRanges& r,
+                       bool posz, hipStream_t s) {
+    if (total <= 0) return;
+    dim3 grid(cdiv(total / 8, NTHREADS)), block(NTHREADS);
+    if (dmix_next)
+        hipLaunchKernelGGL(k_grad_merge<true>, grid, block, 0, s,
+                           (const ushort_t*)a, (const ushort_t*)b,
+                           (const ushort_t*)c, (const ushort_t*)dd,
+                           (ushort_t*)out, (ushort_t*)dmix_next, total, L, d,
+                           r, posz ? 1 : 0);
+    else
+        hipLaunchKernelGGL(k_grad_merge<false>, grid, block, 0, s,
+                           (const ushort_t*)a, (const ushort_t*)b,
+                           (const ushort_t*)c, (const ushort_t*)dd,
+                           (ushort_t*)out, (ushort_t*)nullptr, total, L, d,
+                           r, posz ? 1 : 0);
+}
+
 __global__ __launch_bounds__(NTHREADS) void k_add4(
         const ushort_t* __restrict__ a, const ushort_t* __restrict__ b,
         const ushort_t* __restrict__ c, const ushort_t* __restrict__ d,
diff --git a/glom_pytorch_amd/ops/csrc/bindings.cpp b/glom_pytorch_amd/ops/csrc/bindings.cpp
--- a/glom_pytorch_amd/ops/csrc/bindings.cpp
+++ b/glom_pytorch_amd/ops/csrc/bindings.cpp
@@ -439,7 +439,9 @@
         c10::optional<torch::Tensor> w1t_opt = c10::nullopt,
         c10::optional<torch::Tensor> w2t_opt = c10::nullopt,
         c10::optional<torch::Tensor> td_in_opt = c10::nullopt,
-        int64_t g_lo = 0) {
+        int64_t g_lo = 0, int64_t dy_ld = 0,
+        c10::optional<torch::Tensor> dB2_ready = c10::nullopt,
+        bool no_fill = false) {
     CHECK_IN(dY); CHECK_IN(levels); CHECK_IN(w1); CHECK_IN(w2); CHECK_IN(Hpre);
     CHECK_IN(Hact);
     const int64_t B = levels.size(0), N = levels.size(1),
@@ -448,17 +450,28 @@
     const int64_t m4 = w1.size(0) / G;
     const int64_t M = B * N;
     TORCH_CHECK(g_lo >= 0 && g_lo <= G, "g_lo out of range");
+    const int64_t ldY = dy_ld > 0 ? dy_ld : G * d;
+    TORCH_CHECK(ldY >= G * d && (dy_ld == 0 || ldY % 8 == 0),
+                "dy_ld must be a multiple of 8 and at least G * d");
+    TORCH_CHECK(M == 0 || dY.numel() >= (M - 1) * ldY + G * d,
+                "dY is smaller than (M, G*d) at row stride dy_ld");
+    if (dB2_ready.has_value()) {
+        CHECK_IN((*dB2_ready));
+        TORCH_CHECK(dB2_ready->numel() == G * d, "dB2_ready must be (G*d,)");
+    }
     const int64_t Ga = G - g_lo;
     auto opts = levels.options();
     hipStream_t s = cur_stream();
 
     auto dLevels = torch::empty({B, N, L, d}, opts);
-    zero_unwritten_dx(dLevels.data_ptr(), B * N, L, d, mode, g_lo, s);
+    if (!no_fill)
+        zero_unwritten_dx(dLevels.data_ptr(), B * N, L, d, mode, g_lo, s);
     torch::Tensor dTokens;
     auto dW1 = torch::empty({G * m4, d}, opts);
     auto dW2 = torch::empty({G * d, m4}, opts);
     auto dB1 = torch::empty({G * m4}, opts);
-    auto dB2 = torch::empty({G * d}, opts);
+    auto dB2 = dB2_ready.has_value() ? *dB2_ready
+                                     : torch::empty({G * d}, opts);
     zero_fill(dW1.data_ptr(), g_lo * m4 * d * 2, s);
     zero_fill(dW2.data_ptr(), g_lo * d * m4 * 2, s);
     zero_fill(dB1.data_ptr(), g_lo * m4 * 2, s);
@@ -469,7 +482,7 @@
         dTokens = torch::empty({0}, opts);
     }
     if (Ga == 0) {
-        zero_fill(dB2.data_ptr(), G * d * 2, s);
+        if (!dB2_ready.has_value()) zero_fill(dB2.data_ptr(), G * d * 2, s);
         return {dTokens, dLevels, dW1, dB1, dW2, dB2};
     }
     TORCH_CHECK(Hpre.numel() == G * M * m4 && Hact.numel() == G * M * m4,
@@ -503,7 +516,7 @@
     torch::Tensor db1f;
     {
         GemmParams p = base_params(M, m4, d, LAYOUT_NT, Ga, Ga, 1.0f);
-        p.A.base = u16_at(dY, g_lo * d); p.A.sin = d; p.A.ld = G * d;
+        p.A.base = u16_at(dY, g_lo * d); p.A.sin = d; p.A.ld = ldY;
         p.B.base = u16_at(w2t, g_lo * m4 * d); p.B.sin = m4 * d; p.B.ld = d;
         p.Cbase = u16_at(dHpre, g_lo * M * m4); p.Csin = M * m4; p.Cld = m4;
         p.epilogue = EPI_GELUGRAD;
@@ -554,7 +567,7 @@
     }
     {
         GemmParams p = base_params(d, m4, M, LAYOUT_TN, Ga, Ga, 1.0f);
-        p.A.base = u16_at(dY, g_lo * d); p.A.sin = d; p.A.ld = G * d;
+        p.A.base = u16_at(dY, g_lo * d); p.A.sin = d; p.A.ld = ldY;
         p.B.base = u16_at(Hact, g_lo * M * m4); p.B.sin = M * m4; p.B.ld = m4;
         p.Cbase = u16_at(dW2, g_lo * d * m4); p.Csin = d * m4; p.Cld = m4;
         run_gemm(p, s, opts, true, G);
@@ -570,11 +583,16 @@
                       u16_at(dB1, g_lo * m4), (int)Ga, M, m4, s);
         check_launch();
     }
-    {
+    if (!dB2_ready.has_value()) {
         auto ws = torch::empty({(long)colsum_rb(M) * G * d},
                                opts.dtype(at::kFloat));
-        launch_colsum(dY.data_ptr(), ws.data_ptr<float>(), dB2.data_ptr(),
-                      1, M, G * d, s);
+        if (ldY == G * d)
+            launch_colsum(dY.data_ptr(), ws.data_ptr<float>(),
+                          dB2.data_ptr(), 1, M, G * d, s);
+        else
+            launch_colsum_cone(dY.data_ptr(), ws.data_ptr<float>(),
+                               dB2.data_ptr(), nullptr, M, G * d, 0, ldY, 0,
+                               s);
         check_launch();
     }
     return {dTokens, dLevels, dW1, dB1, dW2, dB2};
@@ -671,7 +689,7 @@
                             torch::Tensor probs, torch::Tensor rnorm,
                             bool attend_self,
                             c10::optional<torch::Tensor> mask_opt,
-                            int64_t l_lo = 0) {
+                            int64_t l_lo = 0, bool no_fill = false) {
     CHECK_IN(dOut); CHECK_IN(levels); CHECK_IN(probs);
     const int64_t B = levels.size(0), N = levels.size(1),
                   L = levels.size(2), d = levels.size(3);
@@ -686,9 +704,11 @@
     if (mask_opt.has_value()) mask = mask_opt.value().data_ptr<bool>();
 
     auto dLevels = torch::empty({B, N, L, d}, opts);
-    launch_zero_slices(dLevels.data_ptr(), B * N, (int)L, (int)d, 0,
-                       (int)l_lo, s);
-    check_launch();
+    if (!no_fill) {
+        launch_zero_slices(dLevels.data_ptr(), B * N, (int)L, (int)d, 0,
+                           (int)l_lo, s);
+        check_launch();
+    }
     if (Ll == 0) return dLevels;
     TORCH_CHECK(l_lo == 0 || d % 8 == 0, "l_lo needs dim % 8 == 0");
     const float* rn = rnorm.data_ptr<float>();
@@ -844,12 +864,21 @@
                               c10::nullopt)[0];
 }
 
-std::vector<torch::Tensor> level_mix_bwd(torch::Tensor dout) {
+std::vector<torch::Tensor> level_mix_bwd(torch::Tensor dout, int64_t lo = 0,
+                                         bool want_dtd = true) {
     CHECK_IN(dout);
     const int64_t B = dout.size(0), N = dout.size(1), L = dout.size(2),
                   d = dout.size(3);
     TORCH_CHECK(d % 8 == 0, "dim must be a multiple of 8");
+    TORCH_CHECK(lo >= 0 && lo <= L && (want_dtd ? lo == 0 : true),
+                "lo out of range (and needs want_dtd = false)");
     auto dmix = torch::empty_like(dout);
+    if (!want_dtd) {
+        launch_mix_bwd_lo(dout.data_ptr(), dmix.data_ptr(), B * N, (int)L,
+                          (int)d, (int)lo, cur_stream());
+        check_launch();
+        return {dmix, torch::empty({0}, dout.options())};
+    }
     auto dtd = torch::empty({B, N, L - 1, d}, dout.options());
     launch_mix_bwd(dout.data_ptr(), dmix.data_ptr(), dtd.data_ptr(),
                    dout.numel(), (int)L, (int)d, cur_stream());
@@ -1042,6 +1071,53 @@
 }
 
 
+std::vector<torch::Tensor> grad_merge(torch::Tensor dmix, torch::Tensor bu_dl,
+                                      torch::Tensor td_dl,
+                                      torch::Tensor dattn, int64_t lo,
+                                      bool posz, bool next) {
+    CHECK_IN(dmix); CHECK_IN(bu_dl); CHECK_IN(td_dl); CHECK_IN(dattn);
+    TORCH_CHECK(dmix.dim() == 4, "grad_merge expects (B,N,L,d)");
+    const int64_t L = dmix.size(2), d = dmix.size(3);
+    TORCH_CHECK(d % 8 == 0, "dim must be a multiple of 8");
+    TORCH_CHECK(lo >= 0 && lo <= L, "lo out of range");
+    TORCH_CHECK(bu_dl.sizes() == dmix.sizes() && td_dl.sizes() == dmix.sizes()
+                && dattn.sizes() == dmix.sizes(),
+                "grad_merge: the four contributions must share one shape");
+    MergeRanges r;
+    r.a_lo = (int)lo; r.a_hi = (int)L;
+    r.b_lo = (int)std::max<int64_t>(lo, 1) - 1; r.b_hi = (int)L - 1;
+    r.c_lo = (int)lo + 1; r.c_hi = (int)L;
+    r.d_lo = (int)lo; r.d_hi = (int)L;
+    r.dead = (int)std::max<int64_t>(lo - 1, 0);
+    auto out = torch::empty_like(dmix);
+    auto nxt = next ? torch::empty_like(dmix)
+                    : torch::empty({0}, dmix.options());
+    launch_grad_merge(dmix.data_ptr(), bu_dl.data_ptr(), td_dl.data_ptr(),
+                      dattn.data_ptr(), out.data_ptr(),
+                      next ? nxt.data_ptr() : nullptr, out.numel(), (int)L,
+                      (int)d, r, posz, cur_stream());
+    check_launch();
+    return {out, nxt};
+}
+
+std::vector<torch::Tensor> db2_cone(torch::Tensor dmix, int64_t lo) {
+    CHECK_IN(dmix);
+    TORCH_CHECK(dmix.dim() == 4, "db2_cone expects (B,N,L,d)");
+    const int64_t M = dmix.size(0) * dmix.size(1), L = dmix.size(2),
+                  d = dmix.size(3);
+    TORCH_CHECK(d % 8 == 0, "dim must be a multiple of 8");
+    TORCH_CHECK(lo >= 0 && lo <= L && M > 0, "lo out of range");
+    auto bu = torch::empty({L * d}, dmix.options());
+    auto td = torch::empty({(L - 1) * d}, dmix.options());
+    auto ws = torch::empty({(long)colsum_rb(M) * L * d},
+                           dmix.options().dtype(at::kFloat));
+    launch_colsum_cone(dmix.data_ptr(), ws.data_ptr<float>(), bu.data_ptr(),
+                       L > 1 ? td.data_ptr() : nullptr, M, L * d,
+                       (L - 1) * d, L * d, lo * d, cur_stream());
+    check_launch();
+    return {bu, td};
+}
+
 
 std::vector<torch::Tensor> ff_bwd_dh(torch::Tensor dY, torch::Tensor w2t,
                                      torch::Tensor Hpre, int64_t g_lo = 0) {
@@ -1295,17 +1371,22 @@
     return {dW, dB, dImg};
 }
 
-torch::Tensor dpos(torch::Tensor dLevels) {
+torch::Tensor dpos(torch::Tensor dLevels, int64_t l0 = 1) {
     CHECK_IN(dLevels);
     const int64_t B = dLevels.size(0), N = dLevels.size(1),
                   L = dLevels.size(2), d = dLevels.size(3);
+    TORCH_CHECK(l0 >= 1, "l0 must be at least 1");
     auto out = torch::empty({N, d}, dLevels.options());
+    if (l0 >= L) {
+        zero_fill(out.data_ptr(), N * d * 2, cur_stream());
+        return out;
+    }
     const int BCH = (int)std::min<int64_t>(B, 8);
     auto ws = torch::empty({BCH * N * d},
                            dLevels.options().dtype(at::kFloat));
     launch_dpos(dLevels.data_ptr(), out.data_ptr(),
                 d % 8 == 0 ? ws.data_ptr<float>() : nullptr, BCH,
-                (int)B, (int)N, (int)L, (int)d, cur_stream());
+                (int)B, (int)N, (int)L, (int)d, cur_stream(), (int)l0);
     check_launch();
     return out;
 }
@@ -1742,14 +1823,16 @@
           py::arg("Hpre"), py::arg("Hact"), py::arg("mode"),
           py::arg("w1t") = c10::nullopt,
           py::arg("w2t") = c10::nullopt,
-          py::arg("td_in") = c10::nullopt, py::arg("g_lo") = 0);
+          py::arg("td_in") = c10::nullopt, py::arg("g_lo") = 0,
+          py::arg("dy_ld") = 0, py::arg("dB2_ready") = c10::nullopt,
+          py::arg("no_fill") = false);
     m.def("consensus_fwd", &consensus_fwd, "consensus attention forward",
           py::arg("levels"), py::arg("attend_self"), py::arg("mask"),
           py::arg("rnorm") = c10::nullopt);
     m.def("consensus_bwd", &consensus_bwd, "consensus attention backward",
           py::arg("dOut"), py::arg("levels"), py::arg("probs"),
           py::arg("rnorm"), py::arg("attend_self"), py::arg("mask"),
-          py::arg("l_lo") = 0);
+          py::arg("l_lo") = 0, py::arg("no_fill") = false);
     m.def("level_mix_fwd", &level_mix_fwd, "level mix forward",
           py::arg("levels"), py::arg("bu"), py::arg("td"), py::arg("cons"),
           py::arg("slab") = c10::nullopt, py::arg("slab_idx") = 0,
@@ -1759,7 +1842,15 @@
           py::arg("levels"), py::arg("bu"), py::arg("td"), py::arg("cons"),
           py::arg("slab") = c10::nullopt, py::arg("slab_idx") = 0,
           py::arg("bu0") = c10::nullopt, py::arg("pos") = c10::nullopt);
-    m.def("level_mix_bwd", &level_mix_bwd, "level mix backward");
+    m.def("level_mix_bwd", &level_mix_bwd, "level mix backward",
+          py::arg("dout"), py::arg("lo") = 0, py::arg("want_dtd") = true);
+    m.def("grad_merge", &grad_merge,
+          "cone-aware sum of the four levels-gradient contributions",
+          py::arg("dmix"), py::arg("bu_dl"), py::arg("td_dl"),
+          py::arg("dattn"), py::arg("lo"), py::arg("posz"),
+          py::arg("next"));
+    m.def("db2_cone", &db2_cone, "dB2 of both FF nets from dmix",
+          py::arg("dmix"), py::arg("lo") = 0);
     m.def("glom_step_fwd", &glom_step_fwd, "full GLOM iteration forward",
           py::arg("tokens"), py::arg("levels"), py::arg("pos"),
           py::arg("bw1"), py::arg("bb1"), py::arg("bw2"), py::arg("bb2"),
@@ -1781,7 +1872,8 @@
     m.def("patch_embed_fwd", &patch_embed_fwd,
           "patchify + embed GEMM (K1)");
     m.def("patch_embed_bwd", &patch_embed_bwd, "patch embed backward");
-    m.def("dpos", &dpos, "positional embedding gradient reduction");
+    m.def("dpos", &dpos, "positional embedding gradient reduction",
+          py::arg("dLevels"), py::arg("l0") = 1);
     m.def("colsum", &colsum, "fixed-order column sum (M,C) -> (C,)");
     m.def("fused_adamw", &fused_adamw,
           "fused AdamW + global-norm grad clip (torch semantics)");
diff --git a/glom_pytorch_amd/ops/csrc/native_ops.h b/glom_pytorch_amd/ops/csrc/native_ops.h
--- a/glom_pytorch_amd/ops/csrc/native_ops.h
+++ b/glom_pytorch_amd/ops/csrc/native_ops.h
@@ -14,8 +14,11 @@
                    long M, long C, hipStream_t s);
 void launch_colsum_fin(const float* partials, void* out, int nprob, long C,
                        int RB, hipStream_t s);
+void launch_colsum_cone(const void* in, float* partials, void* out,
+                        void* out2, long M, long C, long C2, long ld,
+                        long c_lo, hipStream_t s);
 void launch_dpos(const void* dlev, void* out, float* partials, int BCH,
-                 int B, int N, int L, int d, hipStream_t s);
+                 int B, int N, int L, int d, hipStream_t s, int l0 = 1);
 void launch_zero_slice(void* out, long BN, int L, int d, int l0,
                        hipStream_t s);
 void launch_zero_slices(void* out, long BN, int L, int d, int l0, int nl,
diff --git a/glom_pytorch_amd/ops/csrc/native_ops.hip b/glom_pytorch_amd/ops/csrc/native_ops.hip
--- a/glom_pytorch_amd/ops/csrc/native_ops.hip
+++ b/glom_pytorch_amd/ops/csrc/native_ops.hip
@@ -172,10 +172,69 @@
                        dim3(CSF_NT), 0, s, partials, (ushort_t*)out, C, RB);
 }
 
+__global__ __launch_bounds__(NT256) void k_colsum_part_cone(
+        const ushort_t* __restrict__ in, float* __restrict__ partials,
+        long M, long C, long ld, long c_lo, int RB) {
+    int rc = blockIdx.y;
+    long chunk = cdivl(M, RB);
+    long r0 = rc * chunk, r1 = min((long)M, r0 + chunk);
+    float* pout = partials + (long)rc * C;
+    long c8 = c_lo + ((long)blockIdx.x * NT256 + threadIdx.x) * 8;
+    if (c8 >= C) return;
+    float acc[8] = {};
+    for (long r = r0; r < r1; r++) {
+        union { uint4v v; ushort_t u[8]; } t;
+        t.v = *(const uint4v*)(in + r * ld + c8);
+#pragma unroll
+        for (int e = 0; e < 8; e++) acc[e] += bf2f(t.u[e]);
+    }
+#pragma unroll
+    for (int e = 0; e < 8; e++) pout[c8 + e] = acc[e];
+}
+
+__global__ __launch_bounds__(CSF_NT) void k_colsum_fin_cone(
+        const float* __restrict__ partials, ushort_t* __restrict__ out,
+        ushort_t* __restrict__ out2, long C, long C2, long c_lo, int RB) {
+    long c = (long)blockIdx.x * CSF_NT + threadIdx.x;
+    if (c >= C) return;
+    ushort_t v = 0;
+    if (c >= c_lo) {
+        const float* base = partials + c;
+        float acc = 0.f;
+        int rc = 0;
+        for (; rc + CSF_UNROLL <= RB; rc += CSF_UNROLL) {
+            float t[CSF_UNROLL];
+#pragma unroll
+            for (int u = 0; u < CSF_UNROLL; u++)
+                t[u] = base[(long)(rc + u) * C];
+#pragma unroll
+            for (int u = 0; u < CSF_UNROLL; u++) acc += t[u];
+        }
+        for (; rc < RB; rc++) acc += base[(long)rc * C];
+        v = f2bf(acc);
+    }
+    out[c] = v;
+    if (out2 && c < C2) out2[c] = v;
+}
+
+void launch_colsum_cone(const void* in, float* partials, void* out,
+                        void* out2, long M, long C, long C2, long ld,
+                        long c_lo, hipStream_t s) {
+    int RB = colsum_rb(M);
+    if (c_lo < C)
+        hipLaunchKernelGGL(k_colsum_part_cone,
+                           dim3(cdivl((C - c_lo) / 8, NT256), RB),
+                           dim3(NT256), 0, s, (const ushort_t*)in, partials,
+                           M, C, ld, c_lo, RB);
+    hipLaunchKernelGGL(k_colsum_fin_cone, dim3(cdivl(C, CSF_NT)),
+                       dim3(CSF_NT), 0, s, partials, (ushort_t*)out,
+                       (ushort_t*)out2, C, C2, c_lo, RB);
+}
+
 
 __global__ __launch_bounds__(NT256) void k_dpos_part(
         const ushort_t* __restrict__ dlev, float* __restrict__ partials,
-        int B, int N, int L, int d, int BCH) {
+        int B, int N, int L, int d, int BCH, int l0) {
     long q8 = ((long)blockIdx.x * NT256 + threadIdx.x) * 8;
     int n = blockIdx.y;
     int bc = blockIdx.z;
@@ -184,10 +243,10 @@
     int b0 = bc * bchunk, b1 = min(B, b0 + bchunk);
     float acc[8] = {};
     const long bstride = (long)N * L * d;
-    const ushort_t* base = dlev + ((long)n * L + 1) * d + q8;
+    const ushort_t* base = dlev + ((long)n * L + l0) * d + q8;
     for (int b = b0; b < b1; b++) {
         const ushort_t* p = base + b * bstride;
-        for (int l = 0; l < L - 1; l++) {
+        for (int l = 0; l < L - l0; l++) {
             union { uint4v v; ushort_t u[8]; } t;
             t.v = *(const uint4v*)(p + (long)l * d);
 #pragma unroll
@@ -211,34 +270,35 @@
 
 __global__ __launch_bounds__(NT256) void k_dpos(
         const ushort_t* __restrict__ dlev, ushort_t* __restrict__ out,
-        int B, int N, int L, int d) {
+        int B, int N, int L, int d, int l0) {
     int q = blockIdx.x * NT256 + threadIdx.x;
     int n = blockIdx.y;
     if (q >= d) return;
     float acc = 0.f;
     const long bstride = (long)N * L * d;
-    const ushort_t* base = dlev + ((long)n * L + 1) * d + q;
+    const ushort_t* base = dlev + ((long)n * L + l0) * d + q;
     for (int b = 0; b < B; b++) {
         const ushort_t* p = base + b * bstride;
-        for (int l = 0; l < L - 1; l++) acc += bf2f(p[(long)l * d]);
+        for (int l = 0; l < L - l0; l++) acc += bf2f(p[(long)l * d]);
     }
     out[(long)n * d + q] = f2bf(acc);
 }
 
 void launch_dpos(const void* dlev, void* out, float* partials, int BCH,
-                 int B, int N, int L, int d, hipStream_t s) {
+                 int B, int N, int L, int d, hipStream_t s, int l0) {
     if (d % 8 == 0 && partials != nullptr && BCH > 0) {
         hipLaunchKernelGGL(k_dpos_part,
                            dim3(cdivl(d / 8, NT256), N, BCH), dim3(NT256),
                            0, s, (const ushort_t*)dlev, partials, B, N, L,
-                           d, BCH);
+                           d, BCH, l0);
         hipLaunchKernelGGL(k_dpos_fin,
                            dim3(cdivl((long)N * d, NT256)), dim3(NT256), 0,
                            s, partials, (ushort_t*)out, (long)N * d, BCH);
         return;
     }
     hipLaunchKernelGGL(k_dpos, dim3(cdivl(d, NT256), N), dim3(NT256), 0, s,
-                       (const ushort_t*)dlev, (ushort_t*)out, B, N, L, d);
+                       (const ushort_t*)dlev, (ushort_t*)out, B, N, L, d,
+                       l0);
 }
 
 
diff --git a/glom_pytorch_amd/ops/functional.py b/glom_pytorch_amd/ops/functional.py
--- a/glom_pytorch_amd/ops/functional.py
+++ b/glom_pytorch_amd/ops/functional.py
@@ -81,6 +81,25 @@
     @staticmethod
     def backward(ctx, dtraj):
         return (None,) + tuple(dtraj[t] for t in range(dtraj.shape[0]))
+
+
+class ConeTrajectoryFn(torch.autograd.Function):
+
+    @staticmethod
+    def forward(ctx, slab, step, t):
+        ctx.t = t
+        return slab
+
+    @staticmethod
+    def backward(ctx, dtraj):
+        return None, dtraj[ctx.t], None
+
+
+def trajectory_at(all_levels, t):
+    steps = getattr(all_levels, "_glom_steps", None)
+    if steps is None:
+        return all_levels[t]
+    return steps[t % len(steps)]
 
 
 class GroupedFFFn(torch.autograd.Function):
@@ -217,10 +236,73 @@
                               bw1t, bw2t, tw1t, tw2t, tdin)
         ctx.attend_self = attend_self
         ctx.cone = cone
+        ctx.bwd = carry.bwd if carry is not None and cone is not None \
+            else None
         return out
 
     @staticmethod
+    def _backward_merged(ctx, dnew):
+        ext = _load_extension()
+        (tokens, levels, pos, bw1, bw2, tw1, tw2, bhp, bha, thp, tha,
+         probs, rnorm, mask, bw1t, bw2t, tw1t, tw2t,
+         tdin) = ctx.saved_tensors
+        L, d = levels.size(2), levels.size(3)
+        lo, t = ctx.cone
+        if lo > 0 and CHECK_LEVEL_CONE:
+            _check_cone(dnew, lo, t)
+        td_live = lo < L - 1
+        cur = torch.cuda.current_stream()
+        s_td, s_at, _ = GlomStepFn._side_streams()
+        dmix = ctx.bwd.take(dnew, lo)
+        if dmix is None:
+            dmix = ext.level_mix_bwd(dnew.contiguous(), lo, False)[0]
+        ev = torch.cuda.Event()
+        ev.record(cur)
+        with torch.cuda.stream(s_at):
+            s_at.wait_event(ev)
+            dAttn = ext.consensus_bwd(dmix, levels, probs, rnorm,
+                                      ctx.attend_self, mask, lo, True)
+            db2_bu, db2_td = ext.db2_cone(dmix, lo)
+        dmix.record_stream(s_at)
+        bu = ext.grouped_ff_bwd(dmix, tokens, levels, None, bw1, bw2,
+                                bhp, bha, 0, bw1t, bw2t, None, lo, 0,
+                                db2_bu, True)
+        if td_live:
+            with torch.cuda.stream(s_td):
+                s_td.wait_event(ev)
+                td = ext.grouped_ff_bwd(dmix, None, levels, pos, tw1, tw2,
+                                        thp, tha, 1, tw1t, tw2t, tdin, lo,
+                                        L * d, db2_td, True)
+                dPos = ext.dpos(td[1], lo + 1)
+            dmix.record_stream(s_td)
+            cur.wait_stream(s_td)
+        else:
+            td = ext.grouped_ff_bwd(dmix, None, levels, pos, tw1, tw2,
+                                    thp, tha, 1, tw1t, tw2t, tdin, lo,
+                                    L * d, db2_td, True)
+            dPos = ext.dpos(td[1], L)
+        cur.wait_stream(s_at)
+        back = [dAttn, db2_bu, db2_td]
+        if td_live:
+            back += list(td) + [dPos]
+        for x in back:
+            if x is not None and x.numel():
+                x.record_stream(cur)
+        want_next = t > 0
+        dLevels, dmix_next = ext.grad_merge(dmix, bu[1], td[1], dAttn, lo,
+                                            ctx.bwd.posz, want_next)
+        if want_next:
+            ctx.bwd.put(dLevels, dmix_next, max(lo - 1, 0))
+        return (bu[0], dLevels, dPos, bu[2], bu[3], bu[4], bu[5],
+                td[2], td[3], td[4], td[5], None, None, None, None,
+                None, None, None, None, None, None)
+
+    @staticmethod
     def backward(ctx, dnew):
+        if (ctx.bwd is not None
+                and os.environ.get("GLOM_NO_BWD_STREAMS", "0") != "1"
+                and os.environ.get("GLOM_BWD_FORK", "3") == "3"):
+            return GlomStepFn._backward_merged(ctx, dnew)
         ext = _load_extension()
         (tokens, levels, pos, bw1, bw2, tw1, tw2, bhp, bha, thp, tha,
          probs, rnorm, mask, bw1t, bw2t, tw1t, tw2t,
@@ -377,6 +459,33 @@
     MIX_FUSION = bool(on)
 
 
+BWD_MERGE = True
+
+
+def set_bwd_merge(on: bool) -> None:
+    global BWD_MERGE
+    BWD_MERGE = bool(on)
+
+
+class _BwdCarry:
+
+    def __init__(self, posz):
+        self.posz = bool(posz)
+        self._pair = None
+
+    def put(self, dlevels, dmix_next, written_from):
+        self._pair = (dlevels, dmix_next, written_from)
+
+    def take(self, dnew, lo):
+        pair, self._pair = self._pair, None
+        if pair is None:
+            return None
+        dl, dm, written_from = pair
+        same = (dnew.data_ptr() == dl.data_ptr() and dnew.dtype == dl.dtype
+                and dnew.shape == dl.shape and dnew.stride() == dl.stride())
+        return dm if same and lo >= written_from else None
+
+
 class _LoopCarry:
 
     def __init__(self, levels):
@@ -390,6 +499,7 @@
         self.td_in = None
         self.rnorm = None
         self.emit = False
+        self.bwd = None
 
     def set_next(self, td_in, rnorm):
         ok = td_in is not None and td_in.numel() > 0
@@ -504,6 +614,14 @@
     n_sync = grad_iters if overlap else iters
 
     carry = _LoopCarry(levels)
+    merge = (loss_level_min is not None and BWD_MERGE
+             and os.environ.get("GLOM_NO_BWD_MERGE", "0") != "1"
+             and os.environ.get("GLOM_NO_BWD_STREAMS", "0") != "1"
+             and os.environ.get("GLOM_BWD_FORK", "3") == "3"
+             and model.dim % 8 == 0 and model.levels >= 2
+             and 0 < grad_iters <= iters and torch.is_grad_enabled())
+    if merge:
+        carry.bwd = _BwdCarry(posz=return_all)
 
     steps = [levels]
     with trace_range(f"glom/iterate x{iters}"):
@@ -558,5 +676,10 @@
                     slab.record_stream(s_tail)
 
     if return_all:
+        if merge:
+            traj = ConeTrajectoryFn.apply(slab, steps[grad_iters],
+                                          grad_iters)
+            traj._glom_steps = steps
+            return traj
         return TrajectoryFn.apply(slab, *steps)
     return levels
diff --git a/glom_pytorch_amd/parallel/trainer.py b/glom_pytorch_amd/parallel/trainer.py
--- a/glom_pytorch_amd/parallel/trainer.py
+++ b/glom_pytorch_amd/parallel/trainer.py
@@ -14,6 +14,7 @@
 
 from glom_pytorch_amd.parallel.ddp import BucketedDDP
 from glom_pytorch_amd.parallel.failure import Heartbeat
+from glom_pytorch_amd.ops.functional import trajectory_at
 
 
 class _DecoderLinear(nn.Linear):
@@ -189,7 +190,7 @@
         all_levels = self.model(noised, iters=iters, return_all=True,
                                 grad_iters=t, overlap_tail=overlap,
                                 loss_level_min=self._loss_level_min())
-        top = all_levels[t, :, :, -1]
+        top = trajectory_at(all_levels, t)[:, :, -1]
         recon = self.decoder(top)
         loss = F.mse_loss(recon.float(), img.float())
         loss.backward()
@@ -235,10 +236,11 @@
         all_levels = self.model(noised, iters=iters, return_all=True,
                                 grad_iters=t, overlap_tail=overlap,
                                 loss_level_min=self._loss_level_min(True))
-        recon = self.decoder(all_levels[t, :, :, -1])
+        at_t = trajectory_at(all_levels, t)
+        recon = self.decoder(at_t[:, :, -1])
         clean = torch.cat((img, img))
         loss = F.mse_loss(recon.float(), clean.float())
-        lvl = all_levels[t, :, :, self.contrast_level]
+        lvl = at_t[:, :, self.contrast_level]
         loss = loss + self.contrast_weight * column_contrastive_loss(
             lvl[:B], lvl[B:], temperature=self.contrast_temperature,
             negatives=self.contrast_negatives)
@@ -275,7 +277,7 @@
         traj = self.model(noised, iters=iters, return_all=True,
                           grad_iters=t, overlap_tail=True,
                           loss_level_min=self._loss_level_min())
-        recon = self.decoder(traj[t, :, :, -1])
+        recon = self.decoder(trajectory_at(traj, t)[:, :, -1])
         return F.mse_loss(recon.float(), half.float()) * scale
 
     def _micro_step(self, img: torch.Tensor, iters: int,
```

After: 2056 images/sec (median of 6 runs). 1.04x the previous value.
